# HPCForge/Bubbleformer

Measured on AMD Instinct MI355X. Metric: train samples/sec, FiLMAViT 16x192x192x4ch, bs=8 per GPU, higher is better.
Workload: dtype bf16; 1 GPU; FiLMAViT-small (E=384, 6 heads, 12 blocks, P=16, 9 fluid params) fwd + relative-L2 loss + bwd + AdamW, 4-field 16x192x192 clips, batch 8 per GPU (BASELINE.json configs[1]); global_batch=8, parallelism=dp1

## Files before the change

bubbleformer_amd/_lib.py:

```python
import ctypes as C
import os
import subprocess

_HERE = os.path.dirname(os.path.abspath(__file__))
LIB_PATH = os.path.join(_HERE, "libbubbleformer_hip.so")
CSRC = os.path.join(_HERE, "csrc")

BF_DTYPE_F32, BF_DTYPE_BF16 = 0, 1
BF_LAY_KC, BF_LAY_XC = 0, 1
BF_PRO_NONE, BF_PRO_AFFINE, BF_PRO_AFFINE_GELU, BF_PRO_GELU = 0, 1, 2, 3
BF_AUX_NONE, BF_AUX_ADD, BF_AUX_DGELU = 0, 1, 2
BF_OUT_STORE, BF_OUT_STORE_F32, BF_OUT_ATOMIC_F32 = 0, 1, 2
BF_MAX_STAGES = 5
BF_LOSS_LIMBS = 5
BF_OPT_CHUNK, BF_OPT_MAX_GROUPS = 64, 64

vp, fp, i32, i64, f32 = C.c_void_p, C.c_void_p, C.c_int32, C.c_int64, C.c_float


class Operand(C.Structure):
    _fields_ = [("p", vp), ("ld", i64), ("layout", i32), ("seglen", i32), ("segstride", i64), ("gw", i32), ("gh", i32),
                ("gc", i32), ("pro", i32), ("sc", fp), ("sh", fp), ("rows_per_frame", i32), ("nch", i32)]


# ... 34 lines not shown


class DebedParams(C.Structure):
    _fields_ = [("conv_w", fp * BF_MAX_STAGES), ("in_w", fp * BF_MAX_STAGES), ("in_b", fp * BF_MAX_STAGES)]


class ConvSrc(C.Structure):
    _fields_ = [("p", vp), ("C", i32), ("nchw", i32), ("f32", i32)]


class ConvGeo(C.Structure):
    _fields_ = [(n, i32) for n in ("F", "Hi", "Wi", "Ho", "Wo", "kh", "kw", "stride", "pad")]


BF_CONV_PRO_NONE, BF_CONV_PRO_AFFINE_GELU, BF_CONV_PRO_GELU = 0, 1, 2


class RolloutStep(C.Structure):
    _fields_ = [("pred", fp), ("frames", fp), ("field_stride", i64), ("total_frames", i64), ("first", vp), ("step", vp), ("field", vp), ("diff", fp),
                ("div", fp)] + [(n, i32) for n in ("nfields", "B", "T", "C", "H", "W", "Ho", "Wo", "steps", "reserved")]


class CensusRows(C.Structure):
    _fields_ = [(n, vp) for n in ("count", "cells", "attached", "area")]


class LinkRows(C.Structure):
    _fields_ = [(n, vp) for n in ("successor", "n_successors", "predecessor", "n_predecessors", "departure_area", "events")]


class ErrorRows(C.Structure):
    _fields_ = [(n, vp) for n in ("rmse", "max_error", "boundary_rmse", "interface_rmse", "interface_cells", "spectral_error", "spectrum_error",
                                  "spectrum_pred", "spectrum_target")]


class EnsembleRows(C.Structure):
    _fields_ = [(n, vp) for n in ("mean_rmse", "spread", "crps", "rank_hist", "mean")]


class OptStep(C.Structure):
    _fields_ = [("p", fp), ("g", fp), ("m", fp), ("v", fp), ("coef_dev", fp), ("avg", fp), ("chunk_group", vp), ("group_lr_scale", fp),
                ("group_weight_decay", fp), ("group_frozen", vp), ("live_dev", vp), ("n", i64), ("step", i32), ("n_groups", i32)] + [
        (n, f32) for n in ("lr", "beta1", "beta2", "eps", "wd", "gscale", "clip_value", "avg_weight")]


class ClipGatherJob(C.Structure):
    _fields_ = [("src", fp), ("idx", vp), ("first_tab", vp), ("in_field", vp), ("in_diff", fp), ("in_div", fp), ("in_out", fp), ("out_field", vp),
                ("out_diff", fp), ("out_div", fp), ("out_out", fp), ("fluid_tab", fp), ("file_tab", vp), ("fluid_out", fp), ("field_stride", i64),
                ("nframes", i64), ("nsamples", i64)] + [(n, i32) for n in ("Cin", "Tin", "Cout", "Tout", "unroll", "P", "B", "H", "W", "Ho", "Wo", "reserved")]


class ClipAugment(C.Structure):
    _fields_ = [("in_odd", vp), ("out_odd", vp), ("seed", i64), ("flip_thr", i64)] + [(n, i32) for n in ("draw", "Hc", "Wc", "crop_y", "eval_view", "reserved")]


class ClipGatherQ16Job(C.Structure):
    _fields_ = [("codes", vp), ("frame_seg", vp), ("seg_lo", fp), ("seg_step", fp), ("idx", vp), ("first_tab", vp), ("in_field", vp), ("in_diff", fp),
                ("in_div", fp), ("in_out", fp), ("out_field", vp), ("out_diff", fp), ("out_div", fp), ("out_out", fp), ("fluid_tab", fp), ("file_tab", vp),
                ("fluid_out", fp), ("field_stride", i64), ("nframes", i64), ("nsamples", i64)] + [
        (n, i32) for n in ("nfiles", "Cin", "Tin", "Cout", "Tout", "unroll", "P", "B", "H", "W", "Ho", "Wo")]


class RenderTile(C.Structure):
    _fields_ = [("a", fp), ("b", fp), ("mask", fp), ("frame_stride", i64), ("slot_stride", i64), ("mask_frame_stride", i64), ("mask_slot_stride", i64),
                ("range", vp), ("kind", i32)]


class RenderGeom(C.Structure):
    _fields_ = [(n, i32) for n in ("H", "W", "scale", "rows", "cols", "ox", "oy", "pitch_x", "pitch_y", "bar_dx", "bar_w", "img_h", "img_w", "stride")] + [
        ("stroke", C.c_double)]


BF_RENDER_SDF, BF_RENDER_TEMP, BF_RENDER_SPEED = 0, 1, 2
BF_RENDER_MAX_TILES = 6

STAGE_DONE_FN = C.CFUNCTYPE(None, C.c_int, C.c_void_p)
P = C.POINTER
SIGNATURES = {
    "bf_last_error": (C.c_char_p, []),
    "bf_abi_version": (C.c_int, []),
    "bf_prof_enable": (None, [C.c_int]),
    "bf_debug_force_generic_attn": (None, [C.c_int]),
    "bf_debug_tokred_fold": (None, [C.c_int]),
    "bf_side_defer": (None, [C.c_int]),
    "bf_prep_stages": (C.c_int, [C.POINTER(Dims), C.c_int, C.POINTER(C.c_int32), C.POINTER(vp), C.POINTER(vp), C.POINTER(vp), vp]),
    "bf_stage_prepared": (None, [C.c_int]),
    "bf_trunk_train_fwd": (C.c_int, [C.POINTER(Dims), C.c_int, C.POINTER(C.c_int32), C.POINTER(vp), C.POINTER(vp), C.POINTER(vp), C.POINTER(vp), vp,
                                     C.POINTER(vp), vp, vp]),
    "bf_trunk_train_bwd": (C.c_int, [C.POINTER(Dims), C.c_int, C.POINTER(C.c_int32), C.POINTER(vp), C.POINTER(vp), C.POINTER(vp), C.POINTER(vp),
                                     C.POINTER(vp), vp, C.POINTER(vp), vp, C.POINTER(vp), vp, vp, vp, vp, vp]),
    "bf_field_stats_ws_doubles": (i64, [C.c_int]),
    "bf_field_stats": (C.c_int, [fp, vp, vp, C.c_int, vp, vp, vp]),
    "bf_stage_chain_next": (C.c_int, [C.POINTER(Dims), C.c_int, vp, vp]),
    "bf_stage_next_scale": (C.c_int, [fp, C.c_int]),
    "bf_gemm_fwd_frames": (C.c_int, [C.c_int, C.c_int, C.c_int, C.c_int, vp, i64, vp, i64, fp, fp, fp, fp, C.c_int, vp, vp, C.c_int,
                                     C.POINTER(FrameNorm), C.POINTER(FrameNorm), vp]),
    "bf_trunk_eval_weights_bytes": (i64, [C.POINTER(Dims), C.c_int, C.POINTER(C.c_int32)]),
    "bf_trunk_eval_prepare": (C.c_int, [C.POINTER(Dims), C.c_int, C.POINTER(C.c_int32), C.POINTER(vp), vp, vp]),
    "bf_trunk_eval_fwd": (C.c_int, [C.POINTER(Dims), C.c_int, C.POINTER(C.c_int32), C.POINTER(vp), vp, vp, vp, vp, vp]),
    "bf_frame_linear": (C.c_int, [C.c_int, C.c_int, C.c_int, C.c_int, C.c_int, vp, i64, vp, i64, fp, fp, fp, fp, fp, vp, i64, C.c_int, fp, fp, fp,
                                  vp, i64, fp, fp, vp, i64, vp]),
    "bf_side_join": (C.c_int, [vp]),
    "bf_prof_report": (C.c_int, [C.c_char_p, C.c_int]),
    "bf_gemm": (C.c_int, [C.c_int, C.c_int, C.c_int, C.c_int, P(Operand), P(Operand), P(Epilogue), C.c_int, vp]),
    "bf_gemm_tokred": (C.c_int, [C.c_int, C.c_int, C.c_int, i64, vp, i64, vp, i64, fp, C.c_int, fp, fp, i64, vp]),
    "bf_gemm_tokred_ws_floats": (i64, [C.c_int, C.c_int, i64]),
    "bf_gemm_inbwd_frames": (C.c_int, [C.c_int, C.c_int, C.c_int, C.c_int, vp, i64, vp, i64, vp, vp, vp, C.c_int, fp, fp, fp, fp, fp, C.c_int, vp]),
    "bf_gemm_inbwd_frames_chain": (C.c_int, [C.c_int, C.c_int, C.c_int, C.c_int, vp, i64, vp, i64, vp, vp, vp, C.c_int, fp, fp, fp, fp, fp, C.c_int,
                                             vp, vp, fp, fp, fp, fp, C.c_int, fp, vp]),
    "bf_in_stats": (C.c_int, [C.c_int, vp, C.c_int, C.c_int, C.c_int, fp, fp, fp, C.c_int, fp, fp, fp, fp, fp, fp, vp]),
    "bf_in_ws_floats": (i64, [C.c_int, C.c_int, C.c_int, C.c_int]),
    "bf_affine_apply": (C.c_int, [C.c_int, vp, vp, fp, fp, vp, i64, C.c_int, C.c_int, vp]),
    "bf_in_bwd": (C.c_int, [C.c_int, vp, vp, vp, vp, C.c_int, C.c_int, C.c_int, fp, fp, fp, fp, fp, C.c_int, C.c_int, fp, fp,
                            fp, fp, fp, vp]),
    "bf_colsum": (C.c_int, [C.c_int, vp, i64, C.c_int, fp, fp, vp]),
    "bf_attn_axial_fwd": (C.c_int, [C.c_int, vp, vp, i64, C.c_int, C.c_int, C.c_int, C.c_int, fp, fp, fp, fp, fp, fp, fp, vp]),
    "bf_attn_axial_norm_fwd": (C.c_int, [C.c_int, vp, vp, vp, i64, C.c_int, C.c_int, C.c_int, C.c_int, fp, fp, fp, fp, fp, fp, fp, fp, fp, fp, fp, fp,
                                         fp, vp]),
    "bf_attn_fwd": (C.c_int, [C.c_int, vp, vp, i64, C.c_int, i64, i64, i64, i64, C.c_int, C.c_int, fp, fp, fp, fp, fp, fp, f32,
                              C.c_int, vp]),
    "bf_attn_bwd": (C.c_int, [C.c_int, vp, vp, vp, i64, C.c_int, i64, i64, i64, i64, C.c_int, C.c_int, fp, fp, fp, fp, fp, fp,
                              fp, fp, fp, fp, fp, fp, f32, C.c_int, fp, i64, vp]),
    "bf_im2col_nchw": (C.c_int, [C.c_int, fp, vp, C.c_int, C.c_int, C.c_int, C.c_int, C.c_int, vp]),
    "bf_col2im_nchw": (C.c_int, [C.c_int, vp, fp, C.c_int, C.c_int, C.c_int, C.c_int, C.c_int, vp]),
    "bf_pm2nchw": (C.c_int, [fp, fp, fp, fp, C.c_int, C.c_int, C.c_int, C.c_int, C.c_int, vp]),
    "bf_debed_last_bwd": (C.c_int, [C.c_int, fp, fp, fp, fp, fp, vp, vp, vp, C.c_int, C.c_int, C.c_int, C.c_int, C.c_int, C.c_int, vp]),
    "bf_debed_last_bwd_norm": (C.c_int, [C.c_int, fp, fp, fp, fp, fp, vp, vp, vp, fp, fp, fp, fp, vp, fp, fp, C.c_int, C.c_int, C.c_int, C.c_int, C.c_int,
                                         C.c_int, fp, C.c_int64, vp]),
    "bf_gather_gemm": (C.c_int, [C.c_int, vp, vp, C.c_int, fp, fp, vp, C.c_int, C.c_int, C.c_int, C.c_int, C.c_int, vp]),
    "bf_scatter_gemm": (C.c_int, [C.c_int, vp, vp, C.c_int, fp, fp, vp, fp, C.c_int, C.c_int, C.c_int, C.c_int, C.c_int, vp]),
    "bf_gather_wgrad_ws_floats": (C.c_int64, [C.c_int, C.c_int, C.c_int]),
    "bf_gather_wgrad": (C.c_int, [C.c_int, vp, vp, fp, fp, fp, fp, fp, C.c_int, C.c_int, C.c_int, C.c_int, C.c_int, C.c_int, fp, C.c_int64, vp]),
    "bf_gather_gemm_rebuilt": (C.c_int, [C.c_int, vp, vp, vp, C.c_int, fp, fp, vp, C.c_int, C.c_int, C.c_int, C.c_int, C.c_int, vp]),
    "bf_gather_wgrad_rebuilt": (C.c_int, [C.c_int, vp, vp, vp, fp, fp, fp, C.c_int, C.c_int, C.c_int, C.c_int, C.c_int, C.c_int, fp, C.c_int64, vp]),
    "bf_stage_chain_head": (C.c_int, [vp, vp, vp]),
    "bf_stage_chain_tail": (C.c_int, [vp, vp, C.c_int]),
    "bf_embed_tail_ws_floats": (C.c_int64, [C.c_int, C.c_int, C.c_int, C.c_int, C.c_int]),
    "bf_embed_tail_bwd": (C.c_int, [C.c_int, vp, vp, vp, vp, vp, fp, fp, fp, fp, fp, fp, fp, fp, C.c_int, C.c_int, C.c_int, C.c_int, C.c_int, C.c_int,
                                    fp, C.c_int64, vp]),
    "bf_embed_first": (C.c_int, [C.c_int, fp, vp, vp, vp, C.c_int, C.c_int, C.c_int, C.c_int, C.c_int, C.c_int, fp, vp]),
    "bf_in_stats_merge_slices": (C.c_int, [C.c_int, C.c_int, C.c_int, C.c_int, C.c_int, fp, fp, fp, C.c_int, fp, fp, fp, fp, fp, fp, vp]),
    "bf_debed_last": (C.c_int, [C.c_int, vp, fp, fp, vp, fp, fp, fp, C.c_int, C.c_int, C.c_int, C.c_int, C.c_int, C.c_int, vp]),
    "bf_lploss_finalize": (C.c_int, [fp, C.c_int, C.c_int, fp, fp, vp]),
    "bf_nchw2pm": (C.c_int, [C.c_int, fp, fp, fp, fp, fp, vp, C.c_int, C.c_int, C.c_int, C.c_int, C.c_int, vp]),
    "bf_wprep": (C.c_int, [C.c_int, C.c_int, fp, vp, C.c_int, C.c_int, C.c_int, vp]),
    "bf_wgrad_unprep": (C.c_int, [C.c_int, fp, fp, C.c_int, C.c_int, C.c_int, C.c_int, vp]),
    "bf_film_net_fwd": (C.c_int, [fp, fp, fp, fp, fp, fp, fp, fp, C.c_int, C.c_int, C.c_int, vp]),
    "bf_film_net_bwd": (C.c_int, [fp, fp, fp, fp, fp, fp, fp, fp, fp, C.c_int, C.c_int, C.c_int, vp]),
    "bf_adamw": (C.c_int, [P(OptStep), vp]),
    "bf_adam": (C.c_int, [P(OptStep), vp]),
    "bf_lion": (C.c_int, [P(OptStep), vp]),
    "bf_grad_norm_ws_doubles": (i64, [i64]),
    "bf_grad_norm": (C.c_int, [fp, i64, f32, f32, fp, vp, i64, vp]),
    "bf_weight_average": (C.c_int, [fp, fp, i64, f32, vp]),
    "bf_swap_buffers": (C.c_int, [fp, fp, i64, vp]),
    "bf_group_sumsq_ws_doubles": (i64, [i64]),
    "bf_group_sumsq": (C.c_int, [fp, i64, vp, C.c_int, vp, vp, i64, vp]),
    "bf_group_clip_coef": (C.c_int, [vp, vp, C.c_int, f32, f32, fp, fp, vp]),
    "bf_step_guard": (C.c_int, [fp, i32, vp, vp]),
    "bf_nonfinite_scan_ws_len": (i64, [i64]),
    "bf_nonfinite_scan": (C.c_int, [fp, i64, vp, vp, i64, vp]),
    "bf_eikonal_sum": (C.c_int, [fp, i64, C.c_int, C.c_int, f32, vp, vp]),
    "bf_eikonal_l1_frames": (C.c_int, [fp, i64, C.c_int, C.c_int, f32, fp, vp]),
    "bf_heatflux_rows": (C.c_int, [fp, fp, i64, i64, C.c_int, f32, f32, f32, f32, fp, vp]),
    "bf_clip_gather": (C.c_int, [fp, i64, vp, vp, C.c_int, fp, fp, fp, C.c_int, C.c_int, C.c_int, C.c_int, C.c_int, C.c_int, C.c_int, vp]),
    "bf_clip_gather_batch": (C.c_int, [fp, i64, vp, i64, vp, vp, fp, fp, C.c_int, C.c_int, fp, vp, fp, fp, C.c_int, C.c_int, fp, fp, vp, C.c_int, fp,
                                       C.c_int, C.c_int, C.c_int, C.c_int, C.c_int, vp]),
    "bf_clip_gather_unroll": (C.c_int, [fp, i64, i64, vp, i64, vp, vp, fp, fp, C.c_int, C.c_int, fp, vp, fp, fp, C.c_int, C.c_int, C.c_int, fp, fp, vp, C.c_int,
                                        fp, C.c_int, C.c_int, C.c_int, C.c_int, C.c_int, vp]),
    "bf_clip_gather_augment": (C.c_int, [P(ClipGatherJob), P(ClipAugment), vp]),
    "bf_clip_encode_q16": (C.c_int, [fp, vp, i64, f32, f32, vp]),
    "bf_clip_decode_q16": (C.c_int, [vp, i64, vp, fp, fp, fp, i64, C.c_int, C.c_int, C.c_int, C.c_int, vp]),
    "bf_clip_gather_q16": (C.c_int, [P(ClipGatherQ16Job), P(ClipAugment), vp]),
    "bf_clip_noise": (C.c_int, [fp, fp, fp, vp, C.c_uint64, C.c_uint32, C.c_uint32, C.c_int, C.c_int, C.c_int, C.c_int, C.c_int, vp]),
    "bf_rollout_score_ws_doubles": (i64, [C.c_int, C.c_int, C.c_int, C.c_int, C.c_int]),
    "bf_rollout_score": (C.c_int, [P(RolloutStep), C.c_int, f32, fp, fp, fp, fp, fp, fp, vp, i64, vp]),
    "bf_rollout_heatflux": (C.c_int, [P(RolloutStep), C.c_int, C.c_int, fp, f32, f32, f32, f32, fp, fp, vp]),
    "bf_kde_kl_ws_doubles": (i64, [C.c_int, i64, i64, C.c_int]),
    "bf_kde_kl": (C.c_int, [vp, vp, C.c_int, i64, i64, C.c_int, C.c_double, vp, vp, vp, vp, vp, i64, vp]),
    "bf_bubble_census_lds_cells": (i64, []),
    "bf_bubble_census_ws_bytes": (i64, [i64, C.c_int, C.c_int, C.c_int]),
    "bf_bubble_census": (C.c_int, [fp, i64, C.c_int, C.c_int, C.c_int, C.c_int, vp, vp, vp, vp, fp, vp, vp, vp, i64, vp]),
    "bf_rollout_bubbles": (C.c_int, [P(RolloutStep), C.c_int, C.c_int, C.c_int, P(CensusRows), P(CensusRows), vp, vp, i64, vp]),
    "bf_redistance_lds_cells": (i64, []),
    "bf_redistance_ws_bytes": (i64, [i64, C.c_int, C.c_int]),
    "bf_redistance": (C.c_int, [fp, i64, C.c_int, C.c_int, f32, f32, C.c_int, fp, vp, fp, vp, i64, vp]),
    "bf_rollout_redistance": (C.c_int, [P(RolloutStep), C.c_int, f32, f32, C.c_int, C.c_int, fp, vp, fp, vp, i64, vp]),
    "bf_bubble_links_lds_entries": (i64, []),
    "bf_bubble_links_ws_bytes": (i64, [i64, C.c_int]),
    "bf_bubble_links": (C.c_int, [vp, P(CensusRows), i64, C.c_int, C.c_int, C.c_int, C.c_int, P(LinkRows), vp, i64, vp]),
    "bf_bubble_track_ids": (C.c_int, [vp, vp, vp, i64, C.c_int, C.c_int, vp, vp, vp]),
    "bf_rollout_bubble_links": (C.c_int, [P(RolloutStep), C.c_int, vp, P(CensusRows), P(CensusRows), P(LinkRows), P(LinkRows), vp, i64, vp]),
# ... 97 lines not shown
```

bubbleformer_amd/csrc/gemm_frame.hip:

```cpp
#include "gemm_common.h"
#include <stdlib.h>
#include <string.h>
#include <type_traits>

int bf_gemm_pair_scaled(int M, int N, int K, const bf_operand* A, const bf_operand* B, const bf_epilogue* E, void* out2, const float* rowfac,
                        int rows_per_group, hipStream_t st);

namespace {
using namespace bfgemm;

constexpr int FM = 144, FN = 128, FK = 64, FNT = 384;
constexpr int A_EL = FM * FK, B_EL = FK * FN, BUF_EL = A_EL + B_EL;
constexpr int XLD = 136;
constexpr int TILE_EL = FM * XLD;
constexpr int RED_OFF = 2 * TILE_EL * 2;
constexpr int LDS_BYTES = RED_OFF + 3 * 2 * FN * 4;
static_assert(2 * BUF_EL * 2 <= RED_OFF, "operand buffers must not reach the exchange area");

struct FrameArgs {
    const bf16* A; long lda; const bf16* B; long ldb; int N, nk, nt;
    const bf16* x; const bf16* add; bf16* out; long ldx;
    const float* mean; const float* rstd; const float* w; float* ws;
    const float* fscale; int fdiv;
};

__global__ void __launch_bounds__(FNT, 3) gemm_inbwd_frames_kernel(FrameArgs a) {
    extern __shared__ __attribute__((aligned(16))) unsigned char smem[];
    bf16* lds = reinterpret_cast<bf16*>(smem);
    const int tid = threadIdx.x, lane = tid & 63, wave = tid >> 6;
    const int wm = wave >> 1, wn = wave & 1;
    const int li = lane & 15, lg = lane >> 4;
    const int seq = xcd_remap(blockIdx.x, gridDim.x);
    const int fidx = seq / a.nt;
    const int m0 = fidx * FM, n0 = (seq - fidx * a.nt) * FN;

    const bf16* ga[3]; int la[3];
    const bf16* gb[3]; int lb[3];
#pragma unroll
    for (int i = 0; i < 3; ++i) {
        const int c = tid + FNT * i;
        const int row = c >> 3, c8 = (c & 7) << 3;
        ga[i] = a.A + (long)(m0 + row) * a.lda + c8;
        la[i] = lds_off<bf16, false, FK>(row, c8);
        const int kr = (c >> 4) & 63, d8 = (c & 15) << 3;
        gb[i] = a.B + (long)kr * a.ldb + n0 + d8;
        lb[i] = A_EL + lds_off<bf16, true, FN>(kr, d8);
    }
    const bool b2 = tid < FK * FN / 8 - 2 * FNT;
    Chunk<bf16> ra[3], rb[3];
    auto issue = [&](int kt) {
        const long ka = (long)kt * FK, kb = (long)kt * FK * a.ldb;
#pragma unroll
        for (int i = 0; i < 3; ++i) ra[i].load(ga[i] + ka);
        rb[0].load(gb[0] + kb);
        rb[1].load(gb[1] + kb);
        if (b2) rb[2].load(gb[2] + kb);
    };
    auto commit = [&](int buf) {
        bf16* base = lds + buf * BUF_EL;
#pragma unroll
        for (int i = 0; i < 3; ++i) ra[i].store(base + la[i]);
        rb[0].store(base + lb[0]);
        rb[1].store(base + lb[1]);
        if (b2) rb[2].store(base + lb[2]);
    };
    f32x4 acc[3][4];
#pragma unroll
    for (int i = 0; i < 3; ++i)
#pragma unroll
        for (int j = 0; j < 4; ++j) acc[i][j] = f32x4{0.f, 0.f, 0.f, 0.f};
    auto mma = [&](int buf) {
        const bf16* cA = lds + buf * BUF_EL;
        const bf16* cB = cA + A_EL;
#pragma unroll
        for (int kk = 0; kk < FK; kk += 32) {
            bf16x8 fa[3], fb[4];
#pragma unroll
            for (int i = 0; i < 3; ++i) fa[i] = frag_bf16<false, FK>(cA, wm * 48 + i * 16, kk, lane);
#pragma unroll
            for (int j = 0; j < 4; ++j) fb[j] = frag_bf16<true, FN>(cB, wn * 64 + j * 16, kk, lane);
#pragma unroll
            for (int i = 0; i < 3; ++i)
#pragma unroll
// ... 455 lines not shown
#pragma unroll
        for (int i = 0; i < 9; ++i) {
            const bf16x8 x8 = xr[i];
            const bf16x8 d8 = __builtin_bit_cast(bf16x8, ad[i]);
            bf16x8 o;
#pragma unroll
            for (int q = 0; q < 8; ++q) {
                const float xh = ((float)x8[q] - mu[q]) * rs[q];
                float t = rs[q] * ww[q] * (v[i][q] - (s1[q] + xh * s2[q]) * invS);
                if (a.add) t += (float)d8[q];
                o[q] = (bf16)t;
            }
            *reinterpret_cast<bf16x8*>(a.out + (row0 + 16 * i) * a.ldx + col0) = o;
            if constexpr (MODE == 5) {
                const float m2 = a.fscale_s[fidx / a.fdiv_s];
                bf16x8 o2;
#pragma unroll
                for (int q = 0; q < 8; ++q) o2[q] = (bf16)((float)o[q] * m2);
                *reinterpret_cast<bf16x8*>(a.out_s + (row0 + 16 * i) * a.ldx + col0) = o2;
            }
        }
        if constexpr (chain) {
            __builtin_amdgcn_sched_barrier(0);
            uint4 zr[9];
            bf16x8 ov[9];
#pragma unroll
            for (int i = 0; i < 9; ++i) {
                zr[i] = *reinterpret_cast<const uint4*>(a.cz + (row0 + 16 * i) * a.ldx + col0);
                ov[i] = *reinterpret_cast<const bf16x8*>(a.out + (row0 + 16 * i) * a.ldx + col0);
            }
            const long cb = (long)fidx * a.N + col0;
            float m3[8], r3[8], k3[8];
            {
                const float4 m0 = *reinterpret_cast<const float4*>(a.cmean + cb), m1 = *reinterpret_cast<const float4*>(a.cmean + cb + 4);
                const float4 r0 = *reinterpret_cast<const float4*>(a.crstd + cb), r1 = *reinterpret_cast<const float4*>(a.crstd + cb + 4);
                const float4 w0 = *reinterpret_cast<const float4*>(a.cw + col0), w1 = *reinterpret_cast<const float4*>(a.cw + col0 + 4);
                m3[0] = m0.x; m3[1] = m0.y; m3[2] = m0.z; m3[3] = m0.w; m3[4] = m1.x; m3[5] = m1.y; m3[6] = m1.z; m3[7] = m1.w;
                r3[0] = r0.x; r3[1] = r0.y; r3[2] = r0.z; r3[3] = r0.w; r3[4] = r1.x; r3[5] = r1.y; r3[6] = r1.z; r3[7] = r1.w;
                k3[0] = w0.x; k3[1] = w0.y; k3[2] = w0.z; k3[3] = w0.w; k3[4] = w1.x; k3[5] = w1.y; k3[6] = w1.z; k3[7] = w1.w;
                if (a.cg) {
                    const long gbase = (long)(fidx / a.cgdiv) * a.N + col0;
                    const float4 g0 = *reinterpret_cast<const float4*>(a.cg + gbase), g1 = *reinterpret_cast<const float4*>(a.cg + gbase + 4);
                    k3[0] *= g0.x; k3[1] *= g0.y; k3[2] *= g0.z; k3[3] *= g0.w; k3[4] *= g1.x; k3[5] *= g1.y; k3[6] *= g1.z; k3[7] *= g1.w;
                }
#pragma unroll
                for (int q = 0; q < 8; ++q) k3[q] *= r3[q];
            }
            float c1[8], c2[8];
#pragma unroll
            for (int q = 0; q < 8; ++q) { c1[q] = 0.f; c2[q] = 0.f; }
#pragma unroll
            for (int i = 0; i < 9; ++i) {
                const bf16x8 z8 = __builtin_bit_cast(bf16x8, zr[i]);
#pragma unroll
                for (int q = 0; q < 8; ++q) {
                    const float dd = (float)ov[i][q], xh = ((float)z8[q] - m3[q]) * r3[q];
                    c1[q] += dd;
                    c2[q] += dd * xh;
                }
            }
#pragma unroll
            for (int q = 0; q < 8; ++q) { c1[q] = row16_sum(c1[q]); c2[q] = row16_sum(c2[q]); }
            if (li == 0 && a.cws) {
                float* wp = a.cws + cb * 2;
#pragma unroll
                for (int q = 0; q < 8; q += 2) *reinterpret_cast<float4*>(wp + 2 * q) = make_float4(c1[q], c2[q], c1[q + 1], c2[q + 1]);
            }
#pragma unroll
            for (int i = 0; i < 9; ++i) {
                const bf16x8 z8 = __builtin_bit_cast(bf16x8, zr[i]);
                bf16x8 o;
#pragma unroll
                for (int q = 0; q < 8; ++q) {
                    const float dd = (float)ov[i][q], xh = ((float)z8[q] - m3[q]) * r3[q];
                    o[q] = (bf16)(k3[q] * (dd - (c1[q] + xh * c2[q]) * (1.f / 144.f)));
                }
                *reinterpret_cast<bf16x8*>(a.cdz + (row0 + 16 * i) * a.ldx + col0) = o;
            }
        }
    }
}

template <int MODE>
__global__ void __launch_bounds__(512) gemm_pair_kernel(PairArgs a) {
    extern __shared__ __attribute__((aligned(16))) unsigned char smem[];
    const int tid = threadIdx.x, lane = tid & 63, wave = __builtin_amdgcn_readfirstlane(tid >> 6);
    const int seq = xcd_remap(blockIdx.x, gridDim.x);
    const int fp = seq / a.nt;
    const int m0 = fp * PM, n0 = (seq - fp * a.nt) * PN;
    const int f0 = ((MODE == 0 || MODE == 2 || MODE == 5) && a.whole) ? fp : 2 * fp;
    if (wave < 4) pair_body<MODE, 0>(a, smem, lane, wave, m0, n0, f0);
    else pair_body<MODE, 1>(a, smem, lane, wave - 4, m0, n0, f0);
}

template <int MODE>
int launch_pair(const PairArgs& a, int M, hipStream_t st) {
    static BfPerDeviceOnce attr_once; bool& attr_done = attr_once.flag();
    if (!attr_done) {
        hipError_t e_ = hipFuncSetAttribute(reinterpret_cast<const void*>(gemm_pair_kernel<MODE>), hipFuncAttributeMaxDynamicSharedMemorySize, PNSLOT * PSLOT_BYTES);
        if (e_ != hipSuccess) return bf_fail(e_, __FILE__, __LINE__);
        attr_done = true;
    }
    hipLaunchKernelGGL(gemm_pair_kernel<MODE>, dim3((unsigned)((M / PM) * a.nt)), dim3(512), PNSLOT * PSLOT_BYTES, st, a);
    BF_CHECK_LAUNCH();
    return 0;
}
bool pair_shape_ok(int M, int N, int K, int64_t lda, int64_t ldb) {
    static const bool off = bf_knob("BF_PAIR", 1) == 0;
    if (off) return false;
    return M > 0 && M % PM == 0 && N > 0 && N % PN == 0 && K >= PK && K % PK == 0 && lda % 8 == 0 && ldb % 8 == 0 &&
           (long)PM * lda * 2 < (1L << 31) && (long)PK * ldb * 2 < (1L << 31);
}

}

struct InbwdChain { const void* z; void* dz; const float *mean, *rstd, *w, *g; int gdiv; float* ws; };
struct InbwdScaled { void* out_s; const float* f; int fdiv; };
static int inbwd_frames_impl2(int dtype, int M, int N, int K, const void* A, int64_t lda, const void* B, int64_t ldb, const void* x,
                              const void* add, void* out, int S, const float* mean, const float* rstd, const float* w, float* ws,
                              const float* fscale, int fdiv, const InbwdChain* ch, const InbwdScaled* sc2, bf_stream_t stream);
static int inbwd_frames_impl(int dtype, int M, int N, int K, const void* A, int64_t lda, const void* B, int64_t ldb, const void* x,
                             const void* add, void* out, int S, const float* mean, const float* rstd, const float* w, float* ws,
                             const float* fscale, int fdiv, const InbwdChain* ch, bf_stream_t stream);
extern "C" int bf_gemm_inbwd_frames(int dtype, int M, int N, int K, const void* A, int64_t lda, const void* B, int64_t ldb, const void* x,
                                    const void* add, void* out, int S, const float* mean, const float* rstd, const float* w, float* ws,
                                    const float* fscale, int fdiv, bf_stream_t stream) {
    return inbwd_frames_impl(dtype, M, N, K, A, lda, B, ldb, x, add, out, S, mean, rstd, w, ws, fscale, fdiv, nullptr, stream);
}
extern "C" int bf_gemm_inbwd_frames_chain(int dtype, int M, int N, int K, const void* A, int64_t lda, const void* B, int64_t ldb, const void* x,
                                          const void* add, void* out, int S, const float* mean, const float* rstd, const float* w, float* ws,
                                          const float* fscale, int fdiv, const void* cz, void* cdz, const float* cmean, const float* crstd,
                                          const float* cw, const float* cg, int cgdiv, float* cws, bf_stream_t stream) {
    BF_REQUIRE(cz && cdz && cmean && crstd && cw, "bf_gemm_inbwd_frames_chain: null pointer");
    const InbwdChain ch{cz, cdz, cmean, crstd, cw, cg, cgdiv > 0 ? cgdiv : 1, cws};
    return inbwd_frames_impl(dtype, M, N, K, A, lda, B, ldb, x, add, out, S, mean, rstd, w, ws, fscale, fdiv, &ch, stream);
}
static int inbwd_frames_impl(int dtype, int M, int N, int K, const void* A, int64_t lda, const void* B, int64_t ldb, const void* x,
                             const void* add, void* out, int S, const float* mean, const float* rstd, const float* w, float* ws,
                             const float* fscale, int fdiv, const InbwdChain* ch, bf_stream_t stream) {
    return inbwd_frames_impl2(dtype, M, N, K, A, lda, B, ldb, x, add, out, S, mean, rstd, w, ws, fscale, fdiv, ch, nullptr, stream);
}
int bf_gemm_inbwd_frames_scaled(int dtype, int M, int N, int K, const void* A, int64_t lda, const void* B, int64_t ldb, const void* x,
                                const void* add, void* out, int S, const float* mean, const float* rstd, const float* w, float* ws,
                                const float* fscale, int fdiv, void* out_s, const float* f_s, int fdiv_s, hipStream_t stream) {
    if (!out_s || !f_s || (((uintptr_t)out_s) & 15)) return 1;
    const InbwdScaled sc2{out_s, f_s, fdiv_s > 0 ? fdiv_s : 1};
    return inbwd_frames_impl2(dtype, M, N, K, A, lda, B, ldb, x, add, out, S, mean, rstd, w, ws, fscale, fdiv, nullptr, &sc2, (bf_stream_t)stream);
}
static int inbwd_frames_impl2(int dtype, int M, int N, int K, const void* A, int64_t lda, const void* B, int64_t ldb, const void* x,
                              const void* add, void* out, int S, const float* mean, const float* rstd, const float* w, float* ws,
                              const float* fscale, int fdiv, const InbwdChain* ch, const InbwdScaled* sc2, bf_stream_t stream) {
    BF_REQUIRE(A && B && x && out && mean && rstd && w, "bf_gemm_inbwd_frames: null pointer");
    static const bool off = bf_knob("BF_FUSE_INBWD", 1) == 0;
    if (off || dtype != BF_DTYPE_BF16 || (S != FM && S != PM) || M <= 0 || M % S || N <= 0 || N % FN || K < FK || K % FK || lda % 8 || ldb % 8) return 1;
    if (pair_shape_ok(M, N, K, lda, ldb) && (((uintptr_t)A | (uintptr_t)B | (uintptr_t)x | (uintptr_t)add | (uintptr_t)out) & 15) == 0) {
        PairArgs a;
        a.whole = S == PM;
        a.A = (const bf16*)A; a.lda = lda; a.B = (const bf16*)B; a.ldb = ldb; a.N = N; a.nk = K / PK; a.nt = N / PN;
        a.x = (const bf16*)x; a.add = (const bf16*)add; a.out = (bf16*)out; a.ldx = N;
        a.mean = mean; a.rstd = rstd; a.w = w; a.ws = ws; a.fscale = fscale; a.fdiv = fdiv > 0 ? fdiv : 1; a.out2 = nullptr;
        a.cz = nullptr; a.cdz = nullptr; a.cmean = a.crstd = a.cw = a.cg = nullptr; a.cgdiv = 1; a.cws = nullptr;
        a.bias = a.cs = a.ch = nullptr; memset(&a.n1, 0, sizeof(a.n1)); memset(&a.n2, 0, sizeof(a.n2));
        a.out_s = nullptr; a.fscale_s = nullptr; a.fdiv_s = 1;
        if (sc2) { a.out_s = (bf16*)sc2->out_s; a.fscale_s = sc2->f; a.fdiv_s = sc2->fdiv; }
        if (ch) {
            if (a.whole || (((uintptr_t)ch->z | (uintptr_t)ch->dz) & 15)) return 1;
            a.cz = (const bf16*)ch->z; a.cdz = (bf16*)ch->dz; a.cmean = ch->mean; a.crstd = ch->rstd; a.cw = ch->w; a.cg = ch->g; a.cgdiv = ch->gdiv; a.cws = ch->ws;
        }
        BfProfScope prof((hipStream_t)stream, ch ? "gemm_pair<inbwd,chain>" : sc2 ? "gemm_pair<inbwd,scaled>" : "gemm_pair<inbwd>", 2.0 * M * N * K,
                         2.0 * ((double)M * K + (double)N * K + (double)M * N * ((add ? 3 : 2) + (ch ? 2 : 0) + (sc2 ? 1 : 0))));
        if (sc2) { if (ch) return 1; return launch_pair<5>(a, M, (hipStream_t)stream); }
        return ch ? launch_pair<2>(a, M, (hipStream_t)stream) : launch_pair<0>(a, M, (hipStream_t)stream);
    }
    if (ch || sc2) return 1;
    if (S != FM) return 1;
    static BfPerDeviceOnce attr_once;
    if (bool& done = attr_once.flag(); !done) {
        const hipError_t attr = hipFuncSetAttribute(reinterpret_cast<const void*>(gemm_inbwd_frames_kernel), hipFuncAttributeMaxDynamicSharedMemorySize, LDS_BYTES);
        if (attr != hipSuccess) return bf_fail(attr, __FILE__, __LINE__);
        done = true;
    }
    hipStream_t st = (hipStream_t)stream;
    FrameArgs a;
    a.A = (const bf16*)A; a.lda = lda; a.B = (const bf16*)B; a.ldb = ldb; a.N = N; a.nk = K / FK; a.nt = N / FN;
    a.x = (const bf16*)x; a.add = (const bf16*)add; a.out = (bf16*)out; a.ldx = N;
    a.mean = mean; a.rstd = rstd; a.w = w; a.ws = ws;
    a.fscale = fscale; a.fdiv = fdiv > 0 ? fdiv : 1;
    BfProfScope prof(st, "gemm_inbwd_frames<bf16>", 2.0 * M * N * K, 2.0 * ((double)M * K + (double)N * K + (double)M * N * (add ? 3 : 2)));
    hipLaunchKernelGGL(gemm_inbwd_frames_kernel, dim3((unsigned)((M / FM) * a.nt)), dim3(FNT), LDS_BYTES, st, a);
    BF_CHECK_LAUNCH();
    return 0;
}

int bf_gemm_pair_try(int M, int N, int K, const bf_operand* A, const bf_operand* B, const bf_epilogue* E, hipStream_t st) {
    return bf_gemm_pair_scaled(M, N, K, A, B, E, nullptr, nullptr, 1, st);
}
int bf_gemm_pair_scaled(int M, int N, int K, const bf_operand* A, const bf_operand* B, const bf_epilogue* E, void* out2, const float* rowfac,
                        int rows_per_group, hipStream_t st) {
    if (A->layout != BF_LAY_KC || B->layout != BF_LAY_XC || A->pro != BF_PRO_NONE || B->pro != BF_PRO_NONE) return 1;
    if (A->gw > 0 || A->seglen > 0 || B->gw > 0 || B->seglen > 0 || E->gw > 0 || E->seglen > 0) return 1;
    if (E->out_mode != BF_OUT_STORE || E->colsum || E->bias || E->colscale || E->rowscale || E->gelu_out) return 1;
    if (E->aux_mode != BF_AUX_NONE && E->aux_mode != BF_AUX_ADD) return 1;
    if (!pair_shape_ok(M, N, K, A->ld, B->ld) || K < 2 * PK || E->ldc != N || (E->aux_mode == BF_AUX_ADD && E->ld_aux != N)) return 1;
    if (((uintptr_t)A->p | (uintptr_t)B->p | (uintptr_t)E->c | (uintptr_t)E->aux) & 15) return 1;
    PairArgs a;
    a.A = (const bf16*)A->p; a.lda = A->ld; a.B = (const bf16*)B->p; a.ldb = B->ld; a.N = N; a.nk = K / PK; a.nt = N / PN;
    a.x = nullptr; a.add = E->aux_mode == BF_AUX_ADD ? (const bf16*)E->aux : nullptr; a.out = (bf16*)E->c; a.ldx = N;
    a.mean = nullptr; a.rstd = nullptr; a.w = nullptr; a.ws = nullptr; a.fscale = rowfac; a.fdiv = rows_per_group > 0 ? rows_per_group : 1;
    a.out2 = rowfac ? (bf16*)out2 : nullptr; a.whole = 0;
    a.cz = nullptr; a.cdz = nullptr; a.cmean = a.crstd = a.cw = a.cg = nullptr; a.cgdiv = 1; a.cws = nullptr;
    a.bias = a.cs = a.ch = nullptr; memset(&a.n1, 0, sizeof(a.n1)); memset(&a.n2, 0, sizeof(a.n2));
    a.out_s = nullptr; a.fscale_s = nullptr; a.fdiv_s = 1;
    if (a.out2 && ((uintptr_t)out2 & 15)) return 1;
    BfProfScope prof(st, a.add ? "gemm_pair<add>" : "gemm_pair<plain>", 2.0 * M * N * K, 2.0 * ((double)M * K + (double)N * K + (double)M * N * (a.add ? 2 : 1)));
    return launch_pair<1>(a, M, st);
}

extern "C" int bf_gemm_fwd_frames(int dtype, int M, int N, int K, const void* A, int64_t lda, const void* Bt, int64_t ldb, const float* bias,
                                  const float* colscale, const float* colshift, const float* fscale, int fdiv, const void* add, void* out, int S,
                                  const bf_frame_norm* n1, const bf_frame_norm* n2, bf_stream_t stream) {
    static const bool off = bf_knob("BF_FUSE_FWD_NORM", 1) == 0;
    if (off || dtype != BF_DTYPE_BF16 || S != FM || !pair_shape_ok(M, N, K, lda, ldb) || K < 2 * PK) return 1;
    BF_REQUIRE(A && Bt && out, "bf_gemm_fwd_frames: null pointer");
    BF_REQUIRE(!colscale == !colshift, "bf_gemm_fwd_frames: column scale and shift come together");
    if (fscale && !colscale) return 1;
    if (((uintptr_t)A | (uintptr_t)Bt | (uintptr_t)add | (uintptr_t)out | (uintptr_t)bias | (uintptr_t)colscale | (uintptr_t)colshift) & 15) return 1;
    PairArgs a;
    memset(&a, 0, sizeof(a));
    a.A = (const bf16*)A; a.lda = lda; a.B = (const bf16*)Bt; a.ldb = ldb; a.N = N; a.nk = K / PK; a.nt = N / PN;
    a.add = (const bf16*)add; a.out = (bf16*)out; a.ldx = N;
    a.fscale = fscale; a.fdiv = fdiv > 0 ? fdiv : 1; a.cgdiv = 1;
    a.bias = bias; a.cs = colscale; a.ch = colshift;
    auto take = [&](const bf_frame_norm* n, FwdNorm& o, bool first) -> int {
        if (!n) return 0;
        BF_REQUIRE(n->w && n->b && n->mean && n->rstd && n->sc && n->sh && n->out, "bf_gemm_fwd_frames: incomplete norm record");
        if (((uintptr_t)n->w | (uintptr_t)n->b | (uintptr_t)n->g | (uintptr_t)n->mean | (uintptr_t)n->rstd | (uintptr_t)n->sc | (uintptr_t)n->sh |
             (uintptr_t)n->resid | (uintptr_t)n->out) & 15) return 1;
        if (!first && (n->g || n->resid)) return 1;
        o.w = n->w; o.b = n->b; o.g = n->g; o.gdiv = n->gdiv > 0 ? n->gdiv : 1; o.mean = n->mean; o.rstd = n->rstd; o.sc = n->sc; o.sh = n->sh;
        o.resid = (const bf16*)n->resid; o.out = (bf16*)n->out;
        return 0;
    };
    if (int rc = take(n1, a.n1, true)) return rc;
    if (int rc = take(n2, a.n2, false)) return rc;
    BfProfScope prof((hipStream_t)stream, n1 ? (n2 ? "gemm_pair<fwd,norm,chain>" : "gemm_pair<fwd,norm>") : (n2 ? "gemm_pair<fwd,chain>" : "gemm_pair<fwd>"),
                     2.0 * M * N * K, 2.0 * ((double)M * K + (double)N * K + (double)M * N * (1 + (add ? 1 : 0) + (n1 ? (n1->resid ? 2 : 1) : 0) + (n2 ? 1 : 0))));
    return n1 ? launch_pair<4>(a, M, (hipStream_t)stream) : launch_pair<3>(a, M, (hipStream_t)stream);
}
```

bubbleformer_amd/csrc/gemm_tokred.hip:

```cpp
#include "gemm_common.h"
#include <stdio.h>
#include <stdlib.h>
#include <algorithm>

namespace {
using namespace bfgemm;

constexpr int PTN = 192;
constexpr int HR = 32;
constexpr int NSB = PTN / 64;
constexpr int SUBB = HR * 64 * 2;
constexpr int NBUF = 4;
template <int NI> struct PPGeom {
    static constexpr int TM = 64 * NI, HALFB = (NI + NSB) * SUBB, TILES = NI * 6, TILE_FLOATS = TM * PTN;
};

__device__ __forceinline__ bf16x8 tr_frag(unsigned addr) {
    return cat(__builtin_amdgcn_ds_read_tr16_b64_v4i16((lds_s16x4)(uintptr_t)addr),
               __builtin_amdgcn_ds_read_tr16_b64_v4i16((lds_s16x4)(uintptr_t)(addr + 512u)));
}

template <int NI, int GRP>
__device__ __forceinline__ void tokred_pp_body(const bf16* __restrict__ A, long lda, const bf16* __restrict__ B, long ldb,
                                               float* __restrict__ slab_tile, float* __restrict__ cslab_row, int nh, bool do_cs,
                                               unsigned ring_lds, int lane, int w4) {
    using Gm = PPGeom<NI>;
    constexpr int HALFB = Gm::HALFB;
    constexpr int PG = NI == 6 ? (GRP == 0 ? 5 : 4) : 3;
    constexpr int NCS = 3;
    const int wm = w4, wn = GRP;
    const int dr = 8 * w4 + (lane >> 3);
    const int dkey = ((dr >> 1) & 1) | (((dr >> 3) & 1) << 1);
    const int dch = (lane & 7) ^ (dkey << 1);
    const bf16* pA = A + (long)dr * lda + 8 * dch;
    const bf16* pB = B + (long)dr * ldb + 8 * dch;
    const long stepA = (long)HR * lda, stepB = (long)HR * ldb;
    auto issue = [&](int buf) {
        const unsigned base = __builtin_amdgcn_readfirstlane(ring_lds + (unsigned)buf * (unsigned)HALFB + (unsigned)w4 * 1024u);
        if constexpr (NI == 6 && GRP == 0) {
            glds16_off<0>(pA, base + 0 * SUBB); glds16_off<128>(pA, base + 1 * SUBB); glds16_off<256>(pA, base + 2 * SUBB);
            glds16_off<384>(pA, base + 3 * SUBB); glds16_off<512>(pA, base + 4 * SUBB);
            pA += stepA;
        } else if constexpr (NI == 6) {
            glds16_off<640>(pA, base + 5 * SUBB);
            glds16_off<0>(pB, base + 6 * SUBB); glds16_off<128>(pB, base + 7 * SUBB); glds16_off<256>(pB, base + 8 * SUBB);
            pA += stepA; pB += stepB;
        } else if constexpr (GRP == 0) {
            glds16_off<0>(pA, base + 0 * SUBB); glds16_off<128>(pA, base + 1 * SUBB); glds16_off<256>(pA, base + 2 * SUBB);
            pA += stepA;
        } else {
            glds16_off<0>(pB, base + 3 * SUBB); glds16_off<128>(pB, base + 4 * SUBB); glds16_off<256>(pB, base + 5 * SUBB);
            pB += stepB;
        }
    };
    const int g = lane >> 4, q = (lane >> 2) & 3, p = lane & 3;
    const int fkey = ((q >> 1) & 1) | ((g & 1) << 1);
    const unsigned rowb = (unsigned)(8 * g + q) * 128u + (unsigned)(p & 1) * 8u;
    const unsigned offA = rowb + (unsigned)(((2 * wm + (p >> 1)) ^ (fkey << 1)) * 16);
    const unsigned offB0 = rowb + (unsigned)(((2 * wn + (p >> 1)) ^ (fkey << 1)) * 16) + (unsigned)(NI * SUBB);
    const unsigned offB1 = rowb + (unsigned)(((2 * wn + 4 + (p >> 1)) ^ (fkey << 1)) * 16) + (unsigned)(NI * SUBB);

    f32x4 acc[NI][6];
#pragma unroll
    for (int i = 0; i < NI; ++i)
#pragma unroll
        for (int j = 0; j < 6; ++j) acc[i][j] = f32x4{0.f, 0.f, 0.f, 0.f};
    f32x4 cs[NCS];
#pragma unroll
    for (int c = 0; c < NCS; ++c) cs[c] = f32x4{0.f, 0.f, 0.f, 0.f};
    bf16x8 ones;
#pragma unroll
    for (int c = 0; c < 8; ++c) ones[c] = (bf16)1.0f;

    issue(0);
    if (nh > 1) issue(1);
    if (nh > 2) issue(2);
    if (nh > 2) wait_vm<2 * PG>(); else if (nh > 1) wait_vm<PG>(); else wait_vm<0>();
    __builtin_amdgcn_s_barrier();
    if constexpr (GRP == 1) __builtin_amdgcn_s_barrier();

    int buf = 0;
    for (int h = 0; h < nh; ++h) {
        const unsigned hb = ring_lds + (unsigned)buf * (unsigned)HALFB;
        bf16x8 fa[NI], fb[6];
#pragma unroll
        for (int i = 0; i < NI; ++i) fa[i] = tr_frag(hb + offA + (unsigned)(i * SUBB));
#pragma unroll
        for (int j = 0; j < 6; ++j) fb[j] = tr_frag(hb + ((j & 1) ? offB1 : offB0) + (unsigned)((j >> 1) * SUBB));
        if (h + 3 < nh) issue((buf + 3) & 3);
        const int younger = min(h + 3, nh - 1) - (h + 1);
        if (younger >= 2) wait_vm<2 * PG>(); else if (younger == 1) wait_vm<PG>(); else wait_vm<0>();
        asm volatile("s_waitcnt lgkmcnt(0)" ::: "memory");
        __builtin_amdgcn_sched_barrier(0);
        __builtin_amdgcn_s_barrier();
#pragma unroll
        for (int i = 0; i < NI; ++i)
#pragma unroll
            for (int j = 0; j < 6; ++j) acc[i][j] = __builtin_amdgcn_mfma_f32_16x16x32_bf16(fb[j], fa[i], acc[i][j], 0, 0, 0);
        if (do_cs) {
#pragma unroll
            for (int c = 0; c < NCS; ++c) {
                if constexpr (NI == 6) cs[c] = __builtin_amdgcn_mfma_f32_16x16x32_bf16(ones, fa[NCS * GRP + c], cs[c], 0, 0, 0);
                else if constexpr (GRP == 0) cs[c] = __builtin_amdgcn_mfma_f32_16x16x32_bf16(ones, fa[c], cs[c], 0, 0, 0);
            }
        }
        __builtin_amdgcn_sched_barrier(0);
        __builtin_amdgcn_s_barrier();
        buf = (buf + 1) & 3;
    }
    if constexpr (GRP == 0) __builtin_amdgcn_s_barrier();

    const int wave = GRP * 4 + w4;
    float* so = slab_tile + ((size_t)wave * Gm::TILES * 64 + lane) * 4;
#pragma unroll
    for (int i = 0; i < NI; ++i)
#pragma unroll
        for (int j = 0; j < 6; ++j)
            *reinterpret_cast<float4*>(so + (size_t)(i * 6 + j) * 256) = make_float4(acc[i][j][0], acc[i][j][1], acc[i][j][2], acc[i][j][3]);
    if (do_cs && lane < 16) {
        if constexpr (NI == 6) {
#pragma unroll
            for (int c = 0; c < NCS; ++c) cslab_row[16 * (wm + 4 * (NCS * GRP + c)) + lane] = cs[c][0];
        } else if constexpr (GRP == 0) {
#pragma unroll
            for (int c = 0; c < NCS; ++c) cslab_row[16 * (wm + 4 * c) + lane] = cs[c][0];
        }
    }
}

struct FoldRed { const float* slab; const float* cslab; int nslice, ntiles, tiles_k, Nout, Kin; float* out; float* colsum; int accumulate; int nwg; };
template <int NI>
__device__ __forceinline__ void fold_reduce(const FoldRed& r, int b) {
    using Gm = PPGeom<NI>;
    constexpr int T4 = Gm::TILE_FLOATS / 4;
    const long total = (long)r.ntiles * T4;
    const size_t sstride = (size_t)r.ntiles * Gm::TILE_FLOATS;
    for (long e = (long)b * 512 + threadIdx.x; e < total; e += (long)r.nwg * 512) {
        const int tile = (int)(e / T4), q = (int)(e - (long)tile * T4);
        const int lane = q & 63, t = q >> 6, wave = t / Gm::TILES, ij = t - wave * Gm::TILES, i = ij / 6, j = ij - i * 6;
        const int wm = wave & 3, wn = wave >> 2;
        const int nout = (tile / r.tiles_k) * Gm::TM + 16 * (wm + 4 * i) + (lane & 15);
        const int kin = (tile % r.tiles_k) * PTN + 16 * (wn + 2 * j) + 4 * (lane >> 4);
        const float* src = r.slab + (size_t)tile * Gm::TILE_FLOATS + (size_t)q * 4;
        float4* dst = reinterpret_cast<float4*>(r.out + (size_t)nout * r.Kin + kin);
        float4 a = r.accumulate ? *dst : make_float4(0.f, 0.f, 0.f, 0.f);
        for (int s0 = 0; s0 < r.nslice; s0 += 8) {
            float4 v[8];
#pragma unroll
            for (int u = 0; u < 8; ++u) v[u] = s0 + u < r.nslice ? *reinterpret_cast<const float4*>(src + (size_t)(s0 + u) * sstride) : make_float4(0.f, 0.f, 0.f, 0.f);
#pragma unroll
            for (int u = 0; u < 8; ++u)
                if (s0 + u < r.nslice) { a.x += v[u].x; a.y += v[u].y; a.z += v[u].z; a.w += v[u].w; }
        }
        *dst = a;
    }
    if (r.colsum)
        for (long m = (long)b * 512 + threadIdx.x; m < r.Nout; m += (long)r.nwg * 512) {
            float a = r.accumulate ? r.colsum[m] : 0.f;
            for (int s2 = 0; s2 < r.nslice; ++s2) a += r.cslab[(size_t)s2 * r.Nout + m];
            r.colsum[m] = a;
        }
}

template <int NI>
__global__ void __launch_bounds__(512) tokred_pp_kernel(const bf16* __restrict__ A, long lda, const bf16* __restrict__ B, long ldb,
                                                      float* __restrict__ slab, float* __restrict__ cslab, int Nout, int halves_total,
                                                      int halves_per, int tiles_k, int ntiles, int main_wgs, FoldRed red) {
    using Gm = PPGeom<NI>;
    extern __shared__ __attribute__((aligned(16))) char smem[];
    if ((int)blockIdx.x >= main_wgs) { fold_reduce<NI>(red, (int)blockIdx.x - main_wgs); return; }
    const int tid = threadIdx.x, lane = tid & 63, wave = __builtin_amdgcn_readfirstlane(tid >> 6);
    const int seq = xcd_remap(blockIdx.x, main_wgs);
    const int slice = seq / ntiles, tile = seq - slice * ntiles;
    const int n0 = (tile / tiles_k) * Gm::TM, c0 = (tile % tiles_k) * PTN;
    const int h_beg = slice * halves_per;
    const int nh = min(halves_per, halves_total - h_beg);
    const bf16* a0 = A + (long)h_beg * HR * lda + n0;
    const bf16* b0 = B + (long)h_beg * HR * ldb + c0;
    float* slab_tile = slab + ((size_t)slice * ntiles + tile) * Gm::TILE_FLOATS;
    const bool do_cs = cslab != nullptr && c0 == 0;
    float* cslab_row = do_cs ? cslab + (size_t)slice * Nout + n0 : nullptr;
    const unsigned ring_lds = lds_addr(smem);
    if (wave < 4) tokred_pp_body<NI, 0>(a0, lda, b0, ldb, slab_tile, cslab_row, nh, do_cs, ring_lds, lane, wave);
    else tokred_pp_body<NI, 1>(a0, lda, b0, ldb, slab_tile, cslab_row, nh, do_cs, ring_lds, lane, wave - 4);
}

template <int NI, int MAXS>
__global__ void __launch_bounds__(256) tokred_pp_reduce_kernel(const float* __restrict__ slab, const float* __restrict__ cslab, int nslice,
                                                               int ntiles, int tiles_k, int Nout, int Kin, float* __restrict__ out,
                                                               float* __restrict__ colsum, int accumulate) {
    using Gm = PPGeom<NI>;
    constexpr int T4 = Gm::TILE_FLOATS / 4;
    const long e = (long)blockIdx.x * 256 + threadIdx.x;
    if (e < (long)ntiles * T4) {
        const int tile = (int)(e / T4), r = (int)(e - (long)tile * T4);
        const int lane = r & 63, t = r >> 6, wave = t / Gm::TILES, ij = t - wave * Gm::TILES, i = ij / 6, j = ij - i * 6;
        const int wm = wave & 3, wn = wave >> 2;
        const int nout = (tile / tiles_k) * Gm::TM + 16 * (wm + 4 * i) + (lane & 15);
        const int kin = (tile % tiles_k) * PTN + 16 * (wn + 2 * j) + 4 * (lane >> 4);
        const size_t sstride = (size_t)ntiles * Gm::TILE_FLOATS;
        const float* src = slab + (size_t)tile * Gm::TILE_FLOATS + (size_t)r * 4;
        float4 v[MAXS];
#pragma unroll
        for (int s = 0; s < MAXS; ++s) v[s] = s < nslice ? *reinterpret_cast<const float4*>(src + s * sstride) : make_float4(0.f, 0.f, 0.f, 0.f);
        float4* dst = reinterpret_cast<float4*>(out + (size_t)nout * Kin + kin);
        float4 a = accumulate ? *dst : make_float4(0.f, 0.f, 0.f, 0.f);
#pragma unroll
        for (int s = 0; s < MAXS; ++s)
            if (s < nslice) { a.x += v[s].x; a.y += v[s].y; a.z += v[s].z; a.w += v[s].w; }
        *dst = a;
    }
    if (colsum && e < Nout) {
        float v[MAXS];
#pragma unroll
        for (int s = 0; s < MAXS; ++s) v[s] = s < nslice ? cslab[(size_t)s * Nout + e] : 0.f;
        float a = accumulate ? colsum[e] : 0.f;
#pragma unroll
        for (int s = 0; s < MAXS; ++s)
            if (s < nslice) a += v[s];
        colsum[e] = a;
    }
}

constexpr int NW_TILE = 32;
template <int CT, bool PRO>
__global__ void __launch_bounds__(256) tokred_narrow_kernel(const bf16* __restrict__ dy, const bf16* __restrict__ x, long tiles_total, float* __restrict__ slab,
                                                          const float* __restrict__ psc, const float* __restrict__ psh, int tiles_per_frame) {
    constexpr int C = 16 * CT, DYB = NW_TILE * C * 2, XB = NW_TILE * 16 * 2, TB_ = DYB + XB;
    extern __shared__ __attribute__((aligned(16))) char smem[];
    const int tid = threadIdx.x, lane = tid & 63, wave = __builtin_amdgcn_readfirstlane(tid >> 6);
    const long nwaves = (long)gridDim.x * 4, w = (long)blockIdx.x * 4 + wave;
    const long t_beg = tiles_total * w / nwaves, t_end = tiles_total * (w + 1) / nwaves;
    char* mine = smem + (size_t)wave * 2 * TB_;
    const unsigned lds0 = lds_addr(mine);
    auto issue = [&](long t, int slot) {
        const char* gd = reinterpret_cast<const char*>(dy) + t * DYB + lane * 16;
        const unsigned dst = __builtin_amdgcn_readfirstlane(lds0 + (unsigned)slot * (unsigned)TB_);
#pragma unroll
        for (int pce = 0; pce < DYB / 1024; ++pce) glds16(gd + pce * 1024, dst + (unsigned)pce * 1024u);
        glds16(reinterpret_cast<const char*>(x) + t * XB + lane * 16, dst + (unsigned)DYB);
    };
    constexpr int PCS = DYB / 1024 + 1;
    f32x4 acc[CT];
#pragma unroll
    for (int i = 0; i < CT; ++i) acc[i] = f32x4{0.f, 0.f, 0.f, 0.f};
    const int g = lane >> 4, q = (lane >> 2) & 3, pp = lane & 3;
    const unsigned offD = (unsigned)((8 * g + q) * (C * 2) + 8 * pp), offX = (unsigned)(DYB + (8 * g + q) * 32 + 8 * pp);
    auto trf = [&](unsigned addr, unsigned hi_off) {
        return cat(__builtin_amdgcn_ds_read_tr16_b64_v4i16((lds_s16x4)(uintptr_t)addr),
                   __builtin_amdgcn_ds_read_tr16_b64_v4i16((lds_s16x4)(uintptr_t)(addr + hi_off)));
    };
    float scv[CT], shv[CT];
    for (long s_beg = t_beg; s_beg < t_end;) {
        long s_end = t_end;
        if constexpr (PRO) {
            const long f = s_beg / tiles_per_frame;
            s_end = min(t_end, (f + 1) * (long)tiles_per_frame);
            wait_vm<0>();
#pragma unroll
            for (int i = 0; i < CT; ++i) { scv[i] = psc[f * C + 16 * i + (lane & 15)]; shv[i] = psh ? psh[f * C + 16 * i + (lane & 15)] : 0.f; }
#pragma unroll
            for (int i = 0; i < CT; ++i) asm volatile("s_waitcnt vmcnt(0)" : "+v"(scv[i]), "+v"(shv[i]) :: "memory");
        }
        issue(s_beg, 0);
        int slot = 0;
        for (long t = s_beg; t < s_end; ++t) {
            if (t + 1 < s_end) { issue(t + 1, slot ^ 1); wait_vm<PCS>(); } else wait_vm<0>();
// ... 103 lines not shown
    bf16x8 ones;
#pragma unroll
    for (int q = 0; q < 8; ++q) ones[q] = (bf16)1.0f;

#pragma unroll
    for (int s = 0; s < NSLOT - 1; ++s)
        if (s < steps) issue(s);

    int cur = 0, nxt = NSLOT - 1;
    for (int s = 0; s < steps; ++s) {
        const int younger = min(NSLOT - 2, steps - 1 - s);
        if (younger == NSLOT - 2) wait_vm<(NSLOT - 2) * G>();
        else wait_vm<0>();
        asm volatile("s_waitcnt lgkmcnt(0)" ::: "memory");
        __builtin_amdgcn_s_barrier();
        if (s + NSLOT - 1 < steps) issue(nxt);
        const bf16* cA = ring + (size_t)cur * SLOT;
        const bf16* cB = cA + CHUNK;
#pragma unroll
        for (int kk = 0; kk < BK; kk += 32) {
            bf16x8 fa[TMI], fb[TNI];
#pragma unroll
            for (int i = 0; i < TMI; ++i) fa[i] = frag_bf16<true, TB>(cA, wm * (16 * TMI) + i * 16, kk, lane);
#pragma unroll
            for (int j = 0; j < TNI; ++j) fb[j] = frag_bf16<true, TB>(cB, wn * (16 * TNI) + j * 16, kk, lane);
#pragma unroll
            for (int i = 0; i < TMI; ++i)
#pragma unroll
                for (int j = 0; j < TNI; ++j) acc[i][j] = __builtin_amdgcn_mfma_f32_16x16x32_bf16(fb[j], fa[i], acc[i][j], 0, 0, 0);
            if (do_cs) {
#pragma unroll
                for (int i = 0; i < TMI; ++i)
                    if (wn == i) cs = __builtin_amdgcn_mfma_f32_16x16x32_bf16(ones, fa[i], cs, 0, 0, 0);
            }
        }
        cur = cur + 1 == NSLOT ? 0 : cur + 1;
        nxt = nxt + 1 == NSLOT ? 0 : nxt + 1;
    }

    const int li = lane & 15, lg = lane >> 4;
    float* so = slab + ((size_t)slice * Nout + n0 + wm * (16 * TMI) + li) * Kin + c0 + wn * (16 * TNI) + 4 * lg;
#pragma unroll
    for (int i = 0; i < TMI; ++i)
#pragma unroll
        for (int j = 0; j < TNI; ++j)
            *reinterpret_cast<float4*>(so + (size_t)(i * 16) * Kin + j * 16) = make_float4(acc[i][j][0], acc[i][j][1], acc[i][j][2], acc[i][j][3]);
    if (do_cs && lg == 0) cslab[(size_t)slice * Nout + n0 + wm * (16 * TMI) + wn * 16 + li] = cs[0];
}

__global__ void __launch_bounds__(256) tokred_reduce_kernel(const float* __restrict__ slab, const float* __restrict__ cslab, int nslice, long n,
                                                            int Nout, float* __restrict__ out, float* __restrict__ colsum, int accumulate) {
    const long n4 = n / 4;
    for (long i = (long)blockIdx.x * 256 + threadIdx.x; i < n4; i += (long)gridDim.x * 256) {
        float4 a = accumulate ? reinterpret_cast<const float4*>(out)[i] : make_float4(0.f, 0.f, 0.f, 0.f);
        for (int s0 = 0; s0 < nslice; s0 += 8) {
            float4 v[8];
#pragma unroll
            for (int q = 0; q < 8; ++q) v[q] = s0 + q < nslice ? reinterpret_cast<const float4*>(slab + (size_t)(s0 + q) * n)[i] : make_float4(0.f, 0.f, 0.f, 0.f);
#pragma unroll
            for (int q = 0; q < 8; ++q)
                if (s0 + q < nslice) { a.x += v[q].x; a.y += v[q].y; a.z += v[q].z; a.w += v[q].w; }
        }
        reinterpret_cast<float4*>(out)[i] = a;
    }
    if (colsum) {
        for (long m = (long)blockIdx.x * 256 + threadIdx.x; m < Nout; m += (long)gridDim.x * 256) {
            float a = accumulate ? colsum[m] : 0.f;
            for (int s = 0; s < nslice; ++s) a += cslab[(size_t)s * Nout + m];
            colsum[m] = a;
        }
    }
}

constexpr int MAX_SLICES = 16;

}

extern "C" int64_t bf_gemm_tokred_ws_floats(int Nout, int Kin, int64_t M) {
    if (Nout <= 0 || Kin <= 0 || M <= 0) return 0;
    return (int64_t)MAX_SLICES * ((int64_t)Nout * Kin + Nout);
}

namespace {
struct PendingRed { bool on = false; FoldRed r{}; int NI = 0; hipStream_t st = nullptr; bool half = false; hipEvent_t handoff = nullptr; };
PendingRed g_pending[64];
PendingRed& pending_slot() { int dev = 0; (void)hipGetDevice(&dev); return g_pending[(dev >= 0 && dev < 64) ? dev : 0]; }
constexpr int FOLD_WGS = 40;
}
static int tokred_impl(int dtype, int Nout, int Kin, int64_t M, const void* dy, int64_t ldy, const void* x, int64_t ldx, float* out,
                       int accumulate, float* colsum, float* ws, int64_t ws_floats, bool defer, bf_stream_t stream);
static int flush_pending(PendingRed& p, hipStream_t caller) {
    if (!p.on) return 0;
    p.on = false;
    hipStream_t st = p.st;
    const FoldRed& r = p.r;
    const long n = (long)r.Nout * r.Kin;
    const unsigned rblocks = (unsigned)bf_cdiv(std::max<long>(n / 4, r.Nout), 256);
    BfProfScope prof(st, "tokred_reduce_kernel", 0.0, (double)(r.nslice + 1 + (r.accumulate ? 1 : 0)) * n * 4.0);
    if (p.NI == 6) {
        if (r.nslice <= 8) hipLaunchKernelGGL((tokred_pp_reduce_kernel<6, 8>), dim3(rblocks), dim3(256), 0, st, r.slab, r.cslab, r.nslice, r.ntiles, r.tiles_k, r.Nout, r.Kin, r.out, r.colsum, r.accumulate);
        else hipLaunchKernelGGL((tokred_pp_reduce_kernel<6, MAX_SLICES>), dim3(rblocks), dim3(256), 0, st, r.slab, r.cslab, r.nslice, r.ntiles, r.tiles_k, r.Nout, r.Kin, r.out, r.colsum, r.accumulate);
    } else {
        if (r.nslice <= 8) hipLaunchKernelGGL((tokred_pp_reduce_kernel<3, 8>), dim3(rblocks), dim3(256), 0, st, r.slab, r.cslab, r.nslice, r.ntiles, r.tiles_k, r.Nout, r.Kin, r.out, r.colsum, r.accumulate);
        else hipLaunchKernelGGL((tokred_pp_reduce_kernel<3, MAX_SLICES>), dim3(rblocks), dim3(256), 0, st, r.slab, r.cslab, r.nslice, r.ntiles, r.tiles_k, r.Nout, r.Kin, r.out, r.colsum, r.accumulate);
    }
    BF_CHECK_LAUNCH();
    if (caller == st) return 0;
    hipError_t e = p.handoff ? hipSuccess : hipEventCreateWithFlags(&p.handoff, hipEventDisableTiming);
    if (e == hipSuccess) e = hipEventRecord(p.handoff, st);
    if (e == hipSuccess) e = hipStreamWaitEvent(caller, p.handoff, 0);
    return e == hipSuccess ? 0 : bf_fail(e, __FILE__, __LINE__);
}
int bf_gemm_tokred_flush(hipStream_t st) { return flush_pending(pending_slot(), st); }
namespace { bool g_fold_off = false; }
extern "C" void bf_debug_tokred_fold(int on) { g_fold_off = on == 0; }
bool bf_gemm_tokred_pending() { return pending_slot().on; }
const float* bf_gemm_tokred_pending_out() { const PendingRed& p = pending_slot(); return p.on ? p.r.out : nullptr; }
int bf_gemm_tokred_deferred(int dtype, int Nout, int Kin, int64_t M, const void* dy, int64_t ldy, const void* x, int64_t ldx, float* out,
                            int accumulate, float* colsum, float* ws, int64_t ws_floats, hipStream_t stream) {
    return tokred_impl(dtype, Nout, Kin, M, dy, ldy, x, ldx, out, accumulate, colsum, ws, ws_floats, true, (bf_stream_t)stream);
}
extern "C" int bf_gemm_tokred(int dtype, int Nout, int Kin, int64_t M, const void* dy, int64_t ldy, const void* x, int64_t ldx, float* out,
                              int accumulate, float* colsum, float* ws, int64_t ws_floats, bf_stream_t stream) {
    return tokred_impl(dtype, Nout, Kin, M, dy, ldy, x, ldx, out, accumulate, colsum, ws, ws_floats, false, stream);
}
static int tokred_impl(int dtype, int Nout, int Kin, int64_t M, const void* dy, int64_t ldy, const void* x, int64_t ldx, float* out,
                       int accumulate, float* colsum, float* ws, int64_t ws_floats, bool defer, bf_stream_t stream) {
    if (dtype != BF_DTYPE_BF16) return 1;
    static const int skip_env = bf_knob("BF_TOKRED_SKIP", 0);
    if (skip_env) return 0;
    const bool pp = Nout % 192 == 0 && Kin % PTN == 0 && M % HR == 0 && M >= 4 * HR;
    if (!pp && (Nout % TB || Kin % TB || M % BK || M < BK)) return 1;
    if (ldy % 8 || ldx % 8) return 1;
    BF_REQUIRE(dy && x && out && ws, "bf_gemm_tokred: null pointer");
    BF_REQUIRE(((uintptr_t)dy & 15) == 0 && ((uintptr_t)x & 15) == 0 && ((uintptr_t)out & 15) == 0 && ((uintptr_t)ws & 15) == 0,
               "bf_gemm_tokred: operands must be 16-byte aligned");
    BF_REQUIRE(ldy >= Nout && ldx >= Kin, "bf_gemm_tokred: leading dimensions smaller than the row length");
    hipStream_t st = (hipStream_t)stream;
    const long n = (long)Nout * Kin;
    static const int slices_env = bf_knob("BF_TOKRED_SLICES", 0);
    static const int tile_env = bf_knob("BF_TOKRED_TILE", 0);
    static const int wgs_env = bf_knob("BF_TOKRED_WGS", 128);
    if (pp) {
        const long halves = M / HR;
        const int tiles_k0 = Kin / PTN;
        const bool big = Nout % 384 == 0 && tile_env == 384;
        const int tm = big ? 384 : 192;
        int nslice = slices_env > 0 ? slices_env : std::max(1, wgs_env / ((Nout / tm) * tiles_k0));
        nslice = (int)std::max<long>(1, std::min<long>({(long)nslice, (long)MAX_SLICES, halves / 4}));
        const int halves_per = bf_cdiv(halves, nslice);
        const int ns = bf_cdiv(halves, halves_per);
        BF_REQUIRE(ws_floats >= (int64_t)ns * (n + Nout), "bf_gemm_tokred: workspace too small (bf_gemm_tokred_ws_floats)");
        const int tiles_k = Kin / PTN, ntiles = (Nout / tm) * tiles_k;
        static const bool fold_on = bf_knob("BF_TOKRED_FOLD", 1) != 0;
        const int64_t half_floats = (ws_floats / 2) & ~(int64_t)3;
        const bool fold = defer && fold_on && !g_fold_off && (int64_t)ns * (n + Nout) <= half_floats;
        PendingRed& pend = pending_slot();
        if (pend.on && (!fold || pend.NI != (big ? 6 : 3) || pend.st != st)) { const int frc = flush_pending(pend, st); if (frc) return frc; }
        float* region = ws;
        if (fold) { region = ws + (pend.half ? half_floats : 0); pend.half = !pend.half; }
        float* slab = region;
        float* cslab = colsum ? region + (size_t)ns * n : nullptr;
        const unsigned rblocks = (unsigned)bf_cdiv(std::max<long>(n / 4, Nout), 256);
        FoldRed red{};
        static const int fold_wgs = bf_knob("BF_TOKRED_FOLD_WGS", FOLD_WGS);
        if (fold && pend.on) { red = pend.r; red.nwg = fold_wgs; }
        const unsigned extra = red.nwg > 0 ? (unsigned)red.nwg : 0u;
#define BF_PP_GO(NIV)                                                                                                                     \
        do {                                                                                                                              \
            {                                                                                                                             \
                BfProfScope prof(st, NIV == 6 ? "tokred_pp_kernel<384x192,h32,ring4>" : "tokred_pp_kernel<192x192,h32,ring4>",           \
                                 2.0 * Nout * Kin * (double)M, (double)M * (Nout + Kin) * 2.0 + (double)n * 4.0);                         \
                static BfPerDeviceOnce attr_once; bool& attr_done = attr_once.flag();                                                                                            \
                constexpr int lds_bytes = NBUF * PPGeom<NIV>::HALFB;                                                                      \
                if (!attr_done) {                                                                                                         \
                    hipError_t e_ = hipFuncSetAttribute((const void*)tokred_pp_kernel<NIV>, hipFuncAttributeMaxDynamicSharedMemorySize, lds_bytes); \
                    if (e_ != hipSuccess) return bf_fail(e_, __FILE__, __LINE__);                                                         \
                    attr_done = true;                                                                                                     \
                }                                                                                                                         \
                hipLaunchKernelGGL(tokred_pp_kernel<NIV>, dim3((unsigned)(ns * ntiles) + extra), dim3(512), lds_bytes, st, (const bf16*)dy, (long)ldy, \
                                   (const bf16*)x, (long)ldx, slab, cslab, Nout, (int)halves, halves_per, tiles_k, ntiles, ns * ntiles, red); \
                BF_CHECK_LAUNCH();                                                                                                        \
            }                                                                                                                             \
            if (fold) {                                                                                                                   \
                pend.on = true; pend.NI = NIV; pend.st = st;                                                                              \
                pend.r = FoldRed{slab, cslab, ns, ntiles, tiles_k, Nout, Kin, out, colsum, accumulate, 0};                                \
                break;                                                                                                                    \
            }                                                                                                                             \
            BfProfScope prof(st, "tokred_reduce_kernel", 0.0, (double)(ns + 1 + (accumulate ? 1 : 0)) * n * 4.0);                         \
            if (ns <= 8) hipLaunchKernelGGL((tokred_pp_reduce_kernel<NIV, 8>), dim3(rblocks), dim3(256), 0, st, slab, cslab, ns, ntiles, tiles_k, Nout, Kin, out, colsum, accumulate); \
            else hipLaunchKernelGGL((tokred_pp_reduce_kernel<NIV, MAX_SLICES>), dim3(rblocks), dim3(256), 0, st, slab, cslab, ns, ntiles, tiles_k, Nout, Kin, out, colsum, accumulate); \
            BF_CHECK_LAUNCH();                                                                                                            \
        } while (0)
        if (big) BF_PP_GO(6); else BF_PP_GO(3);
#undef BF_PP_GO
        return 0;
    }
    { const int frc = flush_pending(pending_slot(), st); if (frc) return frc; }
    const long steps = M / BK;
    int nslice = slices_env > 0 ? slices_env : 8;
    nslice = (int)std::max<long>(1, std::min<long>({(long)nslice, (long)MAX_SLICES, steps}));
    BF_REQUIRE(ws_floats >= (int64_t)nslice * (n + Nout), "bf_gemm_tokred: workspace too small (bf_gemm_tokred_ws_floats)");
    const int steps_per = bf_cdiv(steps, nslice);
    const int ns = bf_cdiv(steps, steps_per);
    const int tiles_k = Kin / TB, ntiles = (Nout / TB) * tiles_k;
    float* slab = ws;
    float* cslab = colsum ? ws + (size_t)ns * n : nullptr;
    {
        BfProfScope prof(st, "tokred_kernel<128x128,bk64,slots3>", 2.0 * Nout * Kin * (double)M, (double)M * (Nout + Kin) * 2.0 + (double)n * 4.0);
        static BfPerDeviceOnce attr_once; bool& attr_done = attr_once.flag();
        constexpr int lds_bytes = NSLOT * 2 * BK * TB * 2;
        if (!attr_done) {
            hipError_t e_ = hipFuncSetAttribute((const void*)tokred_kernel, hipFuncAttributeMaxDynamicSharedMemorySize, lds_bytes);
            if (e_ != hipSuccess) return bf_fail(e_, __FILE__, __LINE__);
            attr_done = true;
        }
        hipLaunchKernelGGL(tokred_kernel, dim3((unsigned)(ns * ntiles)), dim3(512), lds_bytes, st, (const bf16*)dy, (long)ldy, (const bf16*)x,
                           (long)ldx, slab, cslab, Nout, Kin, (int)steps, steps_per, tiles_k, ntiles);
        BF_CHECK_LAUNCH();
    }
    {
        BfProfScope prof(st, "tokred_reduce_kernel", 0.0, (double)(ns + 1 + (accumulate ? 1 : 0)) * n * 4.0);
        const int blocks = (int)std::min<long>(512, (n / 4 + 255) / 256);
        hipLaunchKernelGGL(tokred_reduce_kernel, dim3(blocks), dim3(256), 0, st, slab, cslab, ns, n, Nout, out, colsum, accumulate);
        BF_CHECK_LAUNCH();
    }
    return 0;
}

int bf_tokred_narrow(int dtype, int C, int64_t P, const void* wide, const void* narrow, float* out, int ldo, int accumulate, int transposed,
                     const float* sc, const float* sh, int64_t rows_per_frame, float* ws, int64_t ws_floats, hipStream_t st) {
    static const bool off = bf_knob("BF_TOKRED_NARROW", 1) == 0;
    if (off || dtype != BF_DTYPE_BF16 || (C != 96 && C != 64 && C != 32) || P <= 0 || P % NW_TILE || ldo < (transposed ? C : 16)) return 1;
    if (((uintptr_t)wide | (uintptr_t)narrow | (uintptr_t)ws) & 15) return 1;
    if (sc && (rows_per_frame <= 0 || rows_per_frame % NW_TILE)) return 1;
    const int wgs = sc ? 512 : 256;
    if (ws_floats < (int64_t)wgs * C * 16) return 1;
    const long tiles = P / NW_TILE;
    const int tpf = sc ? (int)(rows_per_frame / NW_TILE) : 1;
    BfProfScope prof(st, sc ? "tokred_narrow_kernel<gelu>" : "tokred_narrow_kernel", 2.0 * C * 16 * (double)P, (double)P * (C + 16) * 2.0);
#define BF_NARROW_GO(CTV)                                                                                                               \
    do {                                                                                                                                \
        constexpr int lds_bytes = 4 * 2 * (NW_TILE * 16 * CTV * 2 + NW_TILE * 16 * 2);                                                  \
        static_assert(lds_bytes >= 4 * 16 * CTV * 16 * 4, "the reduction buffer aliases the tile rings");                               \
        if (sc) hipLaunchKernelGGL((tokred_narrow_kernel<CTV, true>), dim3(wgs), dim3(256), lds_bytes, st, (const bf16*)wide, (const bf16*)narrow, tiles, ws, sc, sh, tpf); \
        else hipLaunchKernelGGL((tokred_narrow_kernel<CTV, false>), dim3(wgs), dim3(256), lds_bytes, st, (const bf16*)wide, (const bf16*)narrow, tiles, ws, sc, sh, tpf); \
    } while (0)
    if (C == 96) BF_NARROW_GO(6); else if (C == 64) BF_NARROW_GO(4); else BF_NARROW_GO(2);
#undef BF_NARROW_GO
    BF_CHECK_LAUNCH();
    hipLaunchKernelGGL(tokred_narrow_reduce_kernel, dim3(bf_cdiv(C * 16, 256)), dim3(256), 0, st, ws, wgs, C, out, ldo, accumulate, transposed);
    BF_CHECK_LAUNCH();
    return 0;
}
```

bubbleformer_amd/csrc/model.hip:

```cpp
#include "model_common.h"

bool bf_attn_raw_modes(int dtype, int d);
int bf_gemm_tokred_deferred(int dtype, int Nout, int Kin, int64_t M, const void* dy, int64_t ldy, const void* x, int64_t ldx, float* out,
                            int accumulate, float* colsum, float* ws, int64_t ws_floats, hipStream_t stream);
const float* bf_gemm_tokred_pending_out();
int bf_gemm_inbwd_frames_scaled(int dtype, int M, int N, int K, const void* A, int64_t lda, const void* B, int64_t ldb, const void* x,
                                const void* add, void* out, int S, const float* mean, const float* rstd, const float* w, float* ws,
                                const float* fscale, int fdiv, void* out_s, const float* f_s, int fdiv_s, hipStream_t stream);

using namespace bfm;

namespace {

bool g_side_defer = false;

BfPerDevice<TrunkLinks> g_links;

int launch_reduce_jobs(ReduceJobs& J, hipStream_t st);
__global__ void __launch_bounds__(256) stage_prep_multi_kernel(PrepBatch b);

}

bool bfm::side_defer() { return g_side_defer; }
TrunkLinks& bfm::links() { return g_links.get(); }
int bfm::flush_pending_reduce(TrunkLinks& L, hipStream_t st) {
    if (!L.reduce.on) return 0;
    L.reduce.on = false;
    TRY(launch_reduce_jobs(L.reduce.jobs, L.reduce.st));
    return L.hand_over(L.reduce.st, st);
}
int bfm::side_join_pending(TrunkLinks& L, hipStream_t main, int set) {
    if (set < 0) TRY(flush_pending_reduce(L, main));
    SideStream* s = L.side_stream();
    if (set < 0 && bf_gemm_tokred_pending()) {
        hipStream_t ws_st = s ? s->st : main;
        TRY(bf_gemm_tokred_flush(ws_st));
        if (s) { HIP_TRY(hipEventRecord(s->join, s->st)); HIP_TRY(hipStreamWaitEvent(main, s->join, 0)); }
    }
    if (!s) return 0;
    for (int i = 0; i < 2; ++i)
        if ((set < 0 || set == i) && s->pending[i]) {
            HIP_TRY(hipStreamWaitEvent(main, s->tail[i], 0));
            s->pending[i] = false;
        }
    return 0;
}
int bfm::launch_stage_prep(const D& d, const PrepBatch& b, int m, int planes, hipStream_t st) {
    hipLaunchKernelGGL(stage_prep_multi_kernel, dim3(std::max(64, d.E), planes, m), dim3(256), 0, st, b);
    BF_CHECK_LAUNCH();
    return 0;
}

namespace {

int launch_with_pending(TrunkLinks& L, ReduceJobs& J, hipStream_t st) {
    if (L.reduce.on && L.reduce.st == st && J.fits(L.reduce.jobs)) {
        L.reduce.on = false;
        const ReduceJobs& P = L.reduce.jobs;
        for (int i = 0; i < P.n_in; ++i) TRY(J.push(P.in[i]));
        for (int i = 0; i < P.n_attn; ++i) TRY(J.push(P.at[i]));
    }
    TRY(flush_pending_reduce(L, st));
    return launch_reduce_jobs(J, st);
}

__device__ __forceinline__ void outproj_prep_row(const float* __restrict__ W, const float* __restrict__ bias, const float* __restrict__ nb,
                                                 const float* __restrict__ gamma, const float* __restrict__ lo, const float* __restrict__ hi,
                                                 float* __restrict__ alpha, float* __restrict__ beta, float* __restrict__ mc, int E, int n,
                                                 void* __restrict__ wscaled, int dtype) {
    __shared__ float red[4];
    __shared__ float s_alpha;
    float acc = 0.f;
    if (lo) for (int k = threadIdx.x; k < E; k += blockDim.x) acc += W[(long)n * E + k] * nb[k];
    acc = wave_sum(acc);
    if ((threadIdx.x & 63) == 0) red[threadIdx.x >> 6] = acc;
    __syncthreads();
    if (threadIdx.x == 0) {
        float m = bias[n];
        for (int i = 0; i < (int)(blockDim.x >> 6); ++i) m += red[i];
        const float l = lo ? lo[n] : 0.f, h = hi ? hi[n] : 0.f, g = gamma[n];
        alpha[n] = g * (1.f + h);
        beta[n] = g * (bias[n] * (1.f + h) + (lo ? m * (l - h) : 0.f));
        mc[n] = m;
        s_alpha = g * (1.f + h);
    }
    if (wscaled) {
        __syncthreads();
        const float al = s_alpha;
// ... 216 lines not shown
        const InReduceJob& j = J.in[z];
        if ((int)blockIdx.x < (j.C + 63) / 64 && (int)blockIdx.y < (j.frames + j.rdiv() - 1) / j.rdiv()) in_reduce_block(j, blockIdx.x, blockIdx.y, red);
    } else {
        int a = z - J.n_in;
        if (J.at_follows[a]) return;
        for (;; ++a) {
            const AttnReduceJob& j = J.at[a];
            const int nvals = 4 * j.D + 32 * j.heads + j.heads;
            if ((int)blockIdx.x < (nvals + 63) / 64 && blockIdx.y == 0) attn_reduce_block(j, blockIdx.x, 0, 1, red);
            if (a + 1 >= J.n_attn || !J.at_follows[a + 1]) break;
            __syncthreads();
        }
    }
}
int launch_reduce_jobs(ReduceJobs& J, hipStream_t st) {
    int k = 0;
    for (int i = 0; i < J.n_attn; ++i) if (J.at[i].rows > 0) J.at[k++] = J.at[i];
    J.n_attn = k;
    for (int i = 0; i < J.n_attn; ++i)
        J.at_follows[i] = i > 0 && J.at[i].D == J.at[i - 1].D && J.at[i].heads == J.at[i - 1].heads &&
                          ((J.at[i].dqw && J.at[i].dqw == J.at[i - 1].dqw) || (J.at[i].demb && J.at[i].demb == J.at[i - 1].demb));
    if (J.n_in + J.n_attn == 0) return 0;
    int gx = 1, gy = 1;
    for (int i = 0; i < J.n_in; ++i) { gx = std::max(gx, bf_cdiv(J.in[i].C, 64)); gy = std::max(gy, bf_cdiv(J.in[i].frames, J.in[i].rdiv())); }
    for (int i = 0; i < J.n_attn; ++i) { gx = std::max(gx, bf_cdiv(4 * J.at[i].D + 33 * J.at[i].heads, 64)); }
    hipLaunchKernelGGL(stage_param_reduce_kernel, dim3(gx, gy, J.n_in + J.n_attn), dim3(64 * BF_RED_FL), 0, st, J);
    BF_CHECK_LAUNCH();
    return 0;
}

int qkv_gemm(const D& d, const void* xn, const void* w_c, const float* bias, void* qkv, hipStream_t st) {
    bf_operand A = op_plain(xn, d.E, BF_LAY_KC);
    bf_operand Bo = op_plain(w_c, d.E, BF_LAY_KC);
    bf_epilogue e = epi_store(qkv, 3L * d.E);
    e.bias = bias;
    return bf_gemm(d.dtype, (int)d.N, 3 * d.E, d.E, &A, &Bo, &e, 1, st);
}
int outproj_gemm(const D& d, const void* on, const void* w_c, const float* alpha, const float* beta,
                 const void* resid, void* out, const float* drop, long rows_per_group, hipStream_t st) {
    bf_operand A = op_plain(on, d.E, BF_LAY_KC);
    bf_operand Bo = op_plain(w_c, d.E, BF_LAY_KC);
    bf_epilogue e = epi_store(out, d.E);
    e.colscale = alpha; e.colshift = beta; e.aux_mode = BF_AUX_ADD; e.aux = resid; e.ld_aux = d.E;
    e.rowscale = drop; e.rows_per_group = (int)rows_per_group;
    return bf_gemm(d.dtype, (int)d.N, d.E, d.E, &A, &Bo, &e, 1, st);
}
void* bwd_scratch(TrunkLinks& L, const D& d, void* scratch) {
    if (!g_side_defer || !L.side_stream()) return scratch;
    L.scratch_parity ^= 1;
    return (char*)scratch + (size_t)L.scratch_parity * Scratch(d, nullptr).bytes;
}
struct TailNorm { const void* z; void* dz; const float *mean, *rstd, *w, *g; int gdiv; float* ws; bool* done; };
struct InFuse { const void* x; const void* add; void* dx; const float* mean; const float* rstd; const float* w; const float* b; float* ws;
                const float* fscale = nullptr; int fdiv = 1;
                const TailNorm* tail = nullptr;
                void* scaled_out = nullptr; const float* scaled_f = nullptr; int scaled_fdiv = 1; bool* scaled_done = nullptr; };
int dgrad_inbwd(const D& d, const void* dy, int Kdim, const void* w_xc, int Nout, void* tmp, const InFuse& f, hipStream_t st) {
    if (f.tail) {
        const TailNorm& t = *f.tail;
        const int crc = bf_gemm_inbwd_frames_chain(d.dtype, (int)d.N, Nout, Kdim, dy, Kdim, w_xc, Nout, f.x, f.add, f.dx, (int)d.S, f.mean, f.rstd, f.w, f.ws,
                                                   f.fscale, f.fdiv, t.z, t.dz, t.mean, t.rstd, t.w, t.g, t.gdiv, t.ws, st);
        if (crc < 0) return crc;
        if (crc == 0) { *t.done = true; return 0; }
    }
    if (f.scaled_out) {
        const int src = bf_gemm_inbwd_frames_scaled(d.dtype, (int)d.N, Nout, Kdim, dy, Kdim, w_xc, Nout, f.x, f.add, f.dx, (int)d.S, f.mean, f.rstd, f.w, f.ws,
                                                    f.fscale, f.fdiv, f.scaled_out, f.scaled_f, f.scaled_fdiv, st);
        if (src < 0) return src;
        if (src == 0) { *f.scaled_done = true; return 0; }
    }
    const int rc = bf_gemm_inbwd_frames(d.dtype, (int)d.N, Nout, Kdim, dy, Kdim, w_xc, Nout, f.x, f.add, f.dx, (int)d.S, f.mean, f.rstd, f.w, f.ws,
                                        f.fscale, f.fdiv, st);
    if (rc <= 0) return rc;
    bf_operand A = op_plain(dy, Kdim, BF_LAY_KC);
    bf_operand Bo = op_plain(w_xc, Nout, BF_LAY_XC);
    bf_epilogue e = epi_store(tmp, Nout);
    if (f.fscale) { e.rowscale = f.fscale; e.rows_per_group = (int)(d.S * f.fdiv); }
    TRY(bf_gemm(d.dtype, (int)d.N, Nout, Kdim, &A, &Bo, &e, 1, st));
    return bf_in_bwd_partials(d.dtype, tmp, f.x, f.add, f.dx, (int)d.F, (int)d.S, Nout, f.mean, f.rstd, f.w, f.b, nullptr, 1, 0, f.ws, st);
}
int outproj_bwd(const D& d, const Scratch& sc, const void* dout, const void* on, const void* w_s,
                const float* W, const float* bias, const float* nb, const float* gamma, const float* lo, const float* hi,
                const float* alpha, const float* mc, float* dW, float* dbias, float* dnb, float* dgamma, float* dlo, float* dhi,
                void* don, hipStream_t st, Fork& fk, const InFuse* fu = nullptr) {
    TRY(fk.run([=](hipStream_t ss) -> int {
        const void* dsrc = dout;
        const int trc = bf_gemm_tokred_deferred(d.dtype, d.E, d.E, d.N, dsrc, d.E, on, d.E, sc.G, 0, sc.csum, sc.tokred_ws, sc.tokred_floats, ss);
        if (trc < 0) return trc;
        if (trc == 1) {
            ZERO_ON(ss, sc.G, (size_t)((char*)sc.csum - (char*)sc.G) + (size_t)d.E * 4);
            bf_operand A = op_plain(dsrc, d.E, BF_LAY_XC);
            bf_operand Bo = op_plain(on, d.E, BF_LAY_XC);
            bf_epilogue e = epi_atomic(sc.G, d.E);
            e.colsum = sc.csum;
            TRY(bf_gemm(d.dtype, d.E, d.E, (int)d.N, &A, &Bo, &e, splitk_for(d.E, d.E, d.N), ss));
        }
        return 0;
    }));
    fk.run_late([=](hipStream_t ss) -> int {
        if (bf_gemm_tokred_pending_out() == sc.G) TRY(bf_gemm_tokred_flush(ss));
        hipLaunchKernelGGL(outproj_finalize_kernel, dim3(d.E + (lo ? bf_cdiv(d.E, 16) : 0)), dim3(256), 0, ss, sc.G, sc.csum, W, bias, nb, gamma, lo, hi, mc,
                           dW, dbias, dnb, dgamma, dlo, dhi, d.E);
        BF_CHECK_LAUNCH();
        return 0;
    });
    if (fu) return dgrad_inbwd(d, dout, d.E, w_s, d.E, don, *fu, st);
    {
        bf_operand A = op_plain(dout, d.E, BF_LAY_KC);
        bf_operand Bo = op_plain(w_s, d.E, BF_LAY_XC);
        bf_epilogue e = epi_store(don, d.E);
        TRY(bf_gemm(d.dtype, (int)d.N, d.E, d.E, &A, &Bo, &e, 1, st));
    }
    return 0;
}
int linear_bwd(const D& d, const Scratch& sc, const void* dy, int Nout, const void* x, int Kin, int xpro, const float* xsc, const float* xsh,
               const void* w_c, float* dW, float* db, void* dxn, const bf_epilogue* dx_epi, hipStream_t st, Fork& fk, const InFuse* fu = nullptr,
               bool last = false, const void* w_t = nullptr, void* scaled_out = nullptr, const float* rowfac = nullptr, int rpg = 1,
               bool* scaled_done = nullptr) {
    TRY(fk.run([=](hipStream_t ss) -> int {
        const void* xo = x;
        int pro = xpro;
        bf_operand A = op_plain(dy, Nout, BF_LAY_XC);
        if (pro == BF_PRO_AFFINE) {
            TRY(bf_affine_apply(d.dtype, x, nullptr, xsc, xsh, sc.s1, d.N, (int)d.S, Kin, ss));
            xo = sc.s1;
            pro = BF_PRO_NONE;
        }
        bf_operand Bo = op_plain(xo, Kin, BF_LAY_XC);
        if (pro == BF_PRO_NONE) {
            const int trc = bf_gemm_tokred_deferred(d.dtype, Nout, Kin, d.N, dy, Nout, xo, Kin, dW, 1, db, sc.tokred_ws, sc.tokred_floats, ss);
            if (trc <= 0) return trc;
        }
        if (pro != BF_PRO_NONE) op_affine(Bo, pro, xsc, xsh, d.S, Kin);
        bf_epilogue e = epi_atomic(dW, Kin);
        e.colsum = db;
        return bf_gemm(d.dtype, Nout, Kin, (int)d.N, &A, &Bo, &e, splitk_for(Nout, Kin, d.N), ss);
    }));
    if (last) TRY(fk.flush());
    if (fu) return dgrad_inbwd(d, dy, Nout, w_c, Kin, dxn, *fu, st);
    {
        bf_operand A = op_plain(dy, Nout, BF_LAY_KC);
        bf_operand Bo = w_t ? op_plain(w_t, Nout, BF_LAY_KC) : op_plain(w_c, Kin, BF_LAY_XC);
        bf_epilogue e = dx_epi ? *dx_epi : epi_store(dxn, Kin);
        e.c = dxn; e.ldc = Kin;
        if (scaled_out && rowfac && d.dtype == BF_DTYPE_BF16) {
            const int rc = bf_gemm_pair_scaled((int)d.N, Kin, Nout, &A, &Bo, &e, scaled_out, rowfac, rpg, st);
            if (rc < 0) return rc;
            if (rc == 0) { if (scaled_done) *scaled_done = true; return 0; }
        }
        TRY(bf_gemm(d.dtype, (int)d.N, Kin, Nout, &A, &Bo, &e, 1, st));
    }
    return 0;
}

}

extern "C" int64_t bf_temporal_saved_bytes(const bf_dims* s) { D d; if (get_dims(s, &d)) return -1; return (int64_t)TemporalSaved(d, nullptr).bytes; }
extern "C" int64_t bf_spatial_saved_bytes(const bf_dims* s) { D d; if (get_dims(s, &d)) return -1; return (int64_t)SpatialSaved(d, nullptr).bytes; }
static size_t dbr_bytes(const D& d) { return (((size_t)d.N * d.E * d.es) + 255) & ~(size_t)255; }
extern "C" int64_t bf_scratch_bytes(const bf_dims* s) { D d; if (get_dims(s, &d)) return -1; return 2 * (int64_t)Scratch(d, nullptr).bytes + 2 * (int64_t)dbr_bytes(d); }

extern "C" void bf_side_defer(int on) { g_side_defer = on != 0; }
extern "C" int bf_side_join(bf_stream_t s) { return side_join_pending(g_links.get(), (hipStream_t)s); }

extern "C" void bf_stage_prepared(int on) { g_links.get().hints.prepared = on != 0; }
extern "C" int bf_stage_chain_tail(const bf_spatial_params* prev_p, const void* prev_saved, int has_drop_mlp) {
    g_links.get().hints.tail = NextTail{prev_p && prev_saved, prev_p, prev_saved, has_drop_mlp != 0};
    return 0;
}
extern "C" int bf_stage_next_scale(const float* factors, int fdiv) { g_links.get().hints.scale = NextScale{factors, fdiv > 0 ? fdiv : 1}; return 0; }
static NextHead next_head(const D& d, int kind, const void* params, void* saved) {
    auto of = [&](auto* np, const auto& sv) { return NextHead{true, np->norm1_w, np->norm1_b, sv.mean1, sv.rstd1, sv.sc1, sv.sh1, sv.xn, saved}; };
    return kind == 0 ? of((const bf_temporal_params*)params, TemporalSaved(d, saved)) : of((const bf_spatial_params*)params, SpatialSaved(d, saved));
}
extern "C" int bf_stage_chain_next(const bf_dims* dims, int next_kind, const void* next_params, void* next_saved) {
    NextHead& h = g_links.get().hints.head;
    h = NextHead{};
    if (!dims || !next_params || !next_saved) return 0;
    BF_REQUIRE(next_kind == 0 || next_kind == 1, "bf_stage_chain_next: kind must be 0 (temporal) or 1 (spatial)");
    D d; TRY(get_dims(dims, &d));
    h = next_head(d, next_kind, next_params, next_saved);
    return 0;
}
extern "C" int bf_stage_chain_head(const bf_dims* dims, const bf_temporal_params* next_p, void* next_saved) {
    return bf_stage_chain_next(dims, 0, next_p, next_saved);
}

static int temporal_fwd(TrunkLinks& L, const StageHints& H, const bf_dims* dims, const bf_temporal_params* p, const void* x, void* out, void* saved,
                        void* scratch, const float* drop, bf_stream_t s) {
    D d; TRY(get_dims(dims, &d));
    BF_REQUIRE(p && x && out && saved && scratch, "bf_temporal_fwd: null pointer");
    hipStream_t st = (hipStream_t)s;
    const bool head_done = L.take_head_done(saved, st);
    TRY(side_join_pending(L, st));
    TemporalSaved sv(d, saved);
    Scratch sc(d, scratch);
    const void* wv[4];
    TRY(wviews(d, stage_prep(d, 0, p, sv.prep_dst(), nullptr), H.prepared, wv, st));
    const void *win_c = wv[0], *wout_c = wv[1];
    if (!head_done)
        TRY(bf_in_stats_apply(d.dtype, x, (int)d.F, (int)d.S, d.E, p->norm1_w, p->norm1_b, nullptr, 1, nullptr, sv.mean1, sv.rstd1, sv.sc1, sv.sh1, sc.in_ws,
                              nullptr, sv.xn, st));
    TRY(qkv_gemm(d, sv.xn, win_c, p->input_head_b, sv.qkv, st));
    TRY(bf_attn_fwd(d.dtype, sv.qkv, sv.o, (long)d.B * d.S, d.T, d.S, (long)d.T * d.S, 1, d.S, d.heads, d.d, p->qnorm_w, p->qnorm_b,
                    p->knorm_w, p->knorm_b, p->rel_pos_emb, d.attn_scale ? p->attn_scale_factor : nullptr, 1.f, 0, st));
    TRY(bf_in_stats_apply(d.dtype, sv.o, (int)d.F, (int)d.S, d.E, p->norm2_w, p->norm2_b, nullptr, 1, nullptr, sv.mean2, sv.rstd2, sv.sc2, sv.sh2, sc.in_ws,
                          nullptr, sv.on, st));
    if (H.head.armed) {
        const NextHead& h = H.head;
        const bf_frame_norm n2{h.w, h.b, nullptr, 1, h.mean, h.rstd, h.sc, h.sh, nullptr, h.xn};
        const int rc = bf_gemm_fwd_frames(d.dtype, (int)d.N, d.E, d.E, sv.on, d.E, sv.wout_t, d.E, nullptr, sv.alpha, sv.beta, drop, d.T, x, out, (int)d.S,
                                          nullptr, &n2, s);
        if (rc < 0) return rc;
        if (rc == 0) { L.head_done = {h.saved, st}; return 0; }
    }
    TRY(outproj_gemm(d, sv.on, wout_c, sv.alpha, sv.beta, x, out, drop, (long)d.T * d.S, st));
    return 0;
}

static int temporal_bwd(TrunkLinks& L, const StageHints& H, const bf_dims* dims, const bf_temporal_params* p, const bf_temporal_params* g, const void* x,
                        const void* dout, void* dx, void* saved, void* scratch, const float* drop, bf_stream_t s) {
    D d; TRY(get_dims(dims, &d));
    BF_REQUIRE(p && g && x && dout && dx && saved && scratch, "bf_temporal_bwd: null pointer");
    hipStream_t st = (hipStream_t)s;
    TemporalSaved sv(d, saved);
    Scratch sc(d, bwd_scratch(L, d, scratch));
    const void* win_c = d.dtype == BF_DTYPE_F32 ? (const void*)p->input_head_w : sv.win_c;
    Fork fk(L, st, true, L.scratch_parity);
    if (fk.deferred) TRY(side_join_pending(L, st, fk.set));
    void* don = sc.t1;
    void* dO = sc.t1b;
    void* dqkv = sc.t3;
    const void* dbr = dout;
    if (drop) {
        const TrunkLinks::DbrReady& r = L.dbr_ready;
        if (r.dx == dout && r.f == drop && r.buf && r.st == st) dbr = r.buf;
        else {
            TRY(bf_frame_scale(d.dtype, dout, drop, d.T, sc.t4, d.N, (int)d.S, d.E, st));
            dbr = sc.t4;
        }
    }
    L.dbr_ready = TrunkLinks::DbrReady{};
    const InFuse fu2{sv.o, nullptr, dO, sv.mean2, sv.rstd2, p->norm2_w, p->norm2_b, sc.in_ws2};
    TRY(outproj_bwd(d, sc, dbr, sv.on, sv.wout_s, p->output_head_w, p->output_head_b, p->norm2_b, p->gamma, nullptr, nullptr,
                    sv.alpha, sv.mc, g->output_head_w, g->output_head_b, nullptr, g->gamma, nullptr, nullptr, don, st, fk, &fu2));
    ReduceJobs jobs;
    TRY(jobs.push(InReduceJob{sc.in_ws2, (int)d.F, d.E, p->norm2_w, p->norm2_b, nullptr, 1, g->norm2_w, g->norm2_b, nullptr, nullptr, nullptr, nullptr}));
    {
        int rows = 0;
        TRY(bf_attn_bwd_partials(d.dtype, sv.qkv, dO, dqkv, (long)d.B * d.S, d.T, d.S, (long)d.T * d.S, 1, d.S, d.heads, d.d, p->qnorm_w, p->qnorm_b,
                                 p->knorm_w, p->knorm_b, p->rel_pos_emb, d.attn_scale ? p->attn_scale_factor : nullptr, g->qnorm_w, g->qnorm_b,
                                 g->knorm_w, g->knorm_b, g->rel_pos_emb, d.attn_scale ? g->attn_scale_factor : nullptr, 1.f, 0, sc.attn_ws,
                                 Scratch::ATTN_WS_FLOATS, &rows, st));
        TRY(jobs.push(AttnReduceJob{sc.attn_ws, rows, d.d, d.heads, g->qnorm_w, g->qnorm_b, g->knorm_w, g->knorm_b, g->rel_pos_emb,
                                    d.attn_scale ? g->attn_scale_factor : nullptr}));
    }
    void* dxn = sc.t1;
    InFuse fu1{x, dout, dx, sv.mean1, sv.rstd1, p->norm1_w, p->norm1_b, sc.in_ws};
    TailNorm tn;
    bool tail_done = false;
    static const bool chain_on = bf_knob("BF_BWD_CHAIN", 1) != 0;
    if (H.tail.armed && chain_on && fk.deferred && d.dtype == BF_DTYPE_BF16 && d.S == 144 && d.F % 2 == 0) {
        const NextTail& h = H.tail;
        const int oset = L.scratch_parity ^ 1;
        TRY(side_join_pending(L, st, oset));
        Scratch so(d, (char*)scratch + (size_t)oset * Scratch(d, nullptr).bytes);
        SpatialSaved ps(d, const_cast<void*>(h.saved));
        tn = TailNorm{ps.z, so.t1, ps.mean3, ps.rstd3, h.p->mlp_norm_w, h.drop ? ps.gtab : h.p->gamma_mlp, h.drop ? 1 : (int)d.F, L.tail_ws_flip ? so.in_ws5 : so.in_ws4, &tail_done};
        L.tail_ws_flip = !L.tail_ws_flip;
        fu1.tail = &tn;
    }
    if (H.tail.armed) L.tail_done = TrunkLinks::TailDone{};
    TRY(linear_bwd(d, sc, dqkv, 3 * d.E, sv.xn, d.E, BF_PRO_NONE, nullptr, nullptr, win_c, g->input_head_w, g->input_head_b, dxn, nullptr, st, fk, &fu1, true));
    if (tail_done) L.tail_done = {H.tail.saved, dx, tn.ws, st};
    TRY(jobs.push(InReduceJob{sc.in_ws, (int)d.F, d.E, p->norm1_w, p->norm1_b, nullptr, 1, g->norm1_w, g->norm1_b, nullptr, nullptr, nullptr, nullptr}));
    TRY(launch_with_pending(L, jobs, st));
    return fk.join();
}
extern "C" int bf_temporal_fwd(const bf_dims* dims, const bf_temporal_params* p, const void* x, void* out, void* saved, void* scratch,
                               const float* drop, bf_stream_t s) {
    TrunkLinks& L = g_links.get();
    return temporal_fwd(L, L.take_hints(), dims, p, x, out, saved, scratch, drop, s);
}
extern "C" int bf_temporal_bwd(const bf_dims* dims, const bf_temporal_params* p, const bf_temporal_params* g, const void* x, const void* dout,
                               void* dx, void* saved, void* scratch, const float* drop, bf_stream_t s) {
    TrunkLinks& L = g_links.get();
    return temporal_bwd(L, L.take_hints(), dims, p, g, x, dout, dx, saved, scratch, drop, s);
}

static int prep_stages(TrunkLinks& L, const bf_dims* dims, int n, const int32_t* kinds, const void* const* params, void* const* saved,
                       const float* const* drop_mlp, bf_stream_t s) {
    D d; TRY(get_dims(dims, &d));
    BF_REQUIRE(n >= 1 && kinds && params && saved, "bf_prep_stages: bad arguments");
    if (d.dtype != BF_DTYPE_BF16) return 1;
    hipStream_t st = (hipStream_t)s;
    TRY(side_join_pending(L, st));
    for (int i0 = 0; i0 < n; i0 += PREP_BATCH) {
        PrepBatch b;
        memset(&b, 0, sizeof(b));
        const int m = std::min(PREP_BATCH, n - i0);
        for (int i = 0; i < m; ++i) {
            const int k = i0 + i;
            BF_REQUIRE(params[k] && saved[k] && (kinds[k] == 0 || kinds[k] == 1), "bf_prep_stages: bad stage entry");
            b.s[i] = kinds[k] == 0 ? stage_prep(d, 0, params[k], TemporalSaved(d, saved[k]).prep_dst(), nullptr)
                                   : stage_prep(d, 1, params[k], SpatialSaved(d, saved[k]).prep_dst(), drop_mlp ? drop_mlp[k] : nullptr);
        }
        TRY(launch_stage_prep(d, b, m, 7, st));
    }
    return 0;
}
extern "C" int bf_prep_stages(const bf_dims* dims, int n, const int32_t* kinds, const void* const* params, void* const* saved,
                              const float* const* drop_mlp, bf_stream_t s) {
    return prep_stages(g_links.get(), dims, n, kinds, params, saved, drop_mlp, s);
}

static int spatial_fwd(TrunkLinks& L, const StageHints& H, const bf_dims* dims, const bf_spatial_params* p, const void* x, void* out, void* saved,
                       void* scratch, const float* drop_att, const float* drop_mlp, bf_stream_t s) {
    D d; TRY(get_dims(dims, &d));
    BF_REQUIRE(p && x && out && saved && scratch, "bf_spatial_fwd: null pointer");
    hipStream_t st = (hipStream_t)s;
    const bool head_done = L.take_head_done(saved, st);
    TRY(side_join_pending(L, st));
    SpatialSaved sv(d, saved);
    Scratch sc(d, scratch);
    const void* wv[4];
    TRY(wviews(d, stage_prep(d, 1, p, sv.prep_dst(), drop_mlp), H.prepared, wv, st));
    const void *win_c = wv[0], *wout_c = wv[1], *w1_c = wv[2], *w2_c = wv[3];
    if (!head_done)
// ... 38 lines not shown
        const int rc = bf_gemm_fwd_frames(d.dtype, (int)d.N, d.E, 4 * d.E, sv.hid, 4L * d.E, sv.w2t_c, d.E, p->fc2_b, nullptr, nullptr, nullptr, 1, nullptr, sv.z,
                                          (int)d.S, &n1, h.armed ? &n2 : nullptr, s);
        if (rc < 0) return rc;
        if (rc == 0) {
            if (h.armed) L.head_done = {h.saved, st};
            return 0;
        }
    }
    {
        bf_operand A = op_plain(sv.hid, 4L * d.E, BF_LAY_KC);
        bf_operand Bo = op_plain(w2_c, 4L * d.E, BF_LAY_KC);
        bf_epilogue e = epi_store(sv.z, d.E);
        e.bias = p->fc2_b;
        TRY(bf_gemm(d.dtype, (int)d.N, d.E, 4 * d.E, &A, &Bo, &e, 1, st));
    }
    if (H.head.armed) {
        const NextHead& h = H.head;
        bool chained = false;
        TRY(bf_in_stats_apply_chain(d.dtype, sv.z, (int)d.F, (int)d.S, d.E, p->mlp_norm_w, p->mlp_norm_b, g3, g3div, nullptr, sv.mean3, sv.rstd3, sv.sc3, sv.sh3,
                                    sc.in_ws, sv.x1, out, h.w, h.b, h.mean, h.rstd, h.sc, h.sh, h.xn, &chained, st));
        if (chained) L.head_done = {h.saved, st};
        return 0;
    }
    TRY(bf_in_stats_apply(d.dtype, sv.z, (int)d.F, (int)d.S, d.E, p->mlp_norm_w, p->mlp_norm_b, g3, g3div, nullptr, sv.mean3, sv.rstd3,
                          sv.sc3, sv.sh3, sc.in_ws, sv.x1, out, st));
    return 0;
}

static int spatial_bwd(TrunkLinks& L, const StageHints& H, const bf_dims* dims, const bf_spatial_params* p, const bf_spatial_params* g, const void* x,
                       const void* dout, void* dx, void* saved, void* scratch, const float* drop_att, const float* drop_mlp, bf_stream_t s) {
    D d; TRY(get_dims(dims, &d));
    BF_REQUIRE(p && g && x && dout && dx && saved && scratch, "bf_spatial_bwd: null pointer");
    hipStream_t st = (hipStream_t)s;
    SpatialSaved sv(d, saved);
    Scratch sc(d, bwd_scratch(L, d, scratch));
    const bool f32 = d.dtype == BF_DTYPE_F32;
    const void* win_c = f32 ? (const void*)p->input_head_w : sv.win_c;
    const void* w1_c = f32 ? (const void*)p->fc1_w : sv.w1_c;
    const void* w2_c = f32 ? (const void*)p->fc2_w : sv.w2_c;
    TRY(flush_pending_reduce(L, st));
    Fork fk(L, st, true, L.scratch_parity);
    if (fk.deferred) TRY(side_join_pending(L, st, fk.set));
    void* dz = sc.t1;
    ReduceJobs jobs;
    const TrunkLinks::TailDone td = L.tail_done;
    L.tail_done = TrunkLinks::TailDone{};
    const bool tail_done = td.saved == saved && td.dx == dout && td.st == st;
    {
        const float* gsc = drop_mlp ? sv.gtab : p->gamma_mlp;
        const int gdiv = drop_mlp ? 1 : (int)d.F;
        if (!tail_done)
            TRY(bf_in_bwd_partials(d.dtype, dout, sv.z, nullptr, dz, (int)d.F, (int)d.S, d.E, sv.mean3, sv.rstd3, p->mlp_norm_w, p->mlp_norm_b, gsc, gdiv, 0, sc.in_ws3, st));
        TRY(jobs.push(InReduceJob{tail_done ? td.ws : sc.in_ws3, (int)d.F, d.E, p->mlp_norm_w, p->mlp_norm_b, gsc, gdiv, g->mlp_norm_w, g->mlp_norm_b,
                                  drop_mlp ? nullptr : g->gamma_mlp, nullptr, drop_mlp, drop_mlp ? g->gamma_mlp : nullptr}));
    }
    void* dpre = sc.t4;
    {
        bf_epilogue e; memset(&e, 0, sizeof(e));
        e.aux_mode = BF_AUX_DGELU; e.aux = sv.pre; e.ld_aux = 4L * d.E; e.out_mode = BF_OUT_STORE;
        static const bool use_t = bf_knob("BF_FC2_DGRAD_T", 1) != 0;
        TRY(linear_bwd(d, sc, dz, d.E, sv.hid, 4 * d.E, BF_PRO_NONE, nullptr, nullptr, w2_c, g->fc2_w, g->fc2_b, dpre, &e, st, fk, nullptr, false,
                       (!f32 && use_t) ? sv.w2t_c : nullptr));
    }
    void* dx1 = sc.t1b;
    bool dbr_done = false;
    {
        bf_epilogue e; memset(&e, 0, sizeof(e));
        e.aux_mode = BF_AUX_ADD; e.aux = dout; e.ld_aux = d.E; e.out_mode = BF_OUT_STORE;
        TRY(linear_bwd(d, sc, dpre, 4 * d.E, sv.x1, d.E, BF_PRO_NONE, nullptr, nullptr, w1_c, g->fc1_w, g->fc1_b, dx1, &e, st, fk, nullptr, false, nullptr,
                       drop_att ? sc.e5 : nullptr, drop_att, (int)d.S, &dbr_done));
    }
    void* don = sc.e6;
    const void* dbr = dx1;
    if (dbr_done) dbr = sc.e5;
    else if (drop_att) {
        TRY(bf_frame_scale(d.dtype, dx1, drop_att, 1, sc.e5, d.N, (int)d.S, d.E, st));
        dbr = sc.e5;
    }
    void* dO = sc.e7;
    const InFuse fu2{sv.o, nullptr, dO, sv.mean2, sv.rstd2, p->norm2_w, p->norm2_b, sc.in_ws2};
    TRY(outproj_bwd(d, sc, dbr, sv.on, sv.wout_s, p->output_head_w, p->output_head_b, p->norm2_b, p->gamma_att,
                    d.feat_scale ? p->low_freq_scalar : nullptr, d.feat_scale ? p->high_freq_scalar : nullptr, sv.alpha, sv.mc,
                    g->output_head_w, g->output_head_b, g->norm2_b, g->gamma_att, d.feat_scale ? g->low_freq_scalar : nullptr,
                    d.feat_scale ? g->high_freq_scalar : nullptr, don, st, fk, &fu2));
    TRY(jobs.push(InReduceJob{sc.in_ws2, (int)d.F, d.E, p->norm2_w, p->norm2_b, nullptr, 1, g->norm2_w, g->norm2_b, nullptr, nullptr, nullptr, nullptr}));
    void* dqkv = sc.t3;
    {
        int rows = 0;
        static const bool raw_on = bf_knob("BF_ATTN_RAW", 1) != 0;
        const bool rawm = raw_on && bf_attn_raw_modes(d.dtype, d.d);
        TRY(bf_attn_bwd_partials(d.dtype, sv.qkv, dO, dqkv, d.F * d.h, d.w, 1, d.w, 0, 1, d.heads, d.d, p->qnorm_w, p->qnorm_b, p->knorm_w, p->knorm_b,
                                 p->rel_pos_emb, d.attn_scale ? p->attn_scale_factor_x : nullptr, g->qnorm_w, g->qnorm_b, g->knorm_w, g->knorm_b,
                                 g->rel_pos_emb, d.attn_scale ? g->attn_scale_factor_x : nullptr, 0.5f, rawm ? 2 : 0, sc.attn_ws, Scratch::ATTN_WS_FLOATS, &rows, st));
        TRY(jobs.push(AttnReduceJob{sc.attn_ws, rows, d.d, d.heads, g->qnorm_w, g->qnorm_b, g->knorm_w, g->knorm_b, g->rel_pos_emb,
                                    d.attn_scale ? g->attn_scale_factor_x : nullptr}));
        TRY(bf_attn_bwd_partials(d.dtype, sv.qkv, dO, dqkv, d.F * d.w, d.h, d.w, d.S, 1, d.w, d.heads, d.d, p->qnorm_w, p->qnorm_b, p->knorm_w, p->knorm_b,
                                 p->rel_pos_emb, d.attn_scale ? p->attn_scale_factor_y : nullptr, g->qnorm_w, g->qnorm_b, g->knorm_w, g->knorm_b,
                                 g->rel_pos_emb, d.attn_scale ? g->attn_scale_factor_y : nullptr, 0.5f, rawm ? 5 : 1, sc.attn_ws2, Scratch::ATTN_WS_FLOATS, &rows, st));
        TRY(jobs.push(AttnReduceJob{sc.attn_ws2, rows, d.d, d.heads, g->qnorm_w, g->qnorm_b, g->knorm_w, g->knorm_b, g->rel_pos_emb,
                                    d.attn_scale ? g->attn_scale_factor_y : nullptr}));
    }
    void* dxn = sc.e6;
    InFuse fu1{x, dx1, dx, sv.mean1, sv.rstd1, p->norm1_w, p->norm1_b, sc.in_ws};
    bool scaled_done = false;
    const NextScale& ns = H.scale;
    L.dbr_ready = TrunkLinks::DbrReady{};
    static const bool scaled_on = bf_knob("BF_BWD_SCALED_COPY", 1) != 0;
    if (ns.f && scaled_on && fk.deferred && d.dtype == BF_DTYPE_BF16) {
        fu1.scaled_out = (char*)scratch + 2 * Scratch(d, nullptr).bytes + (L.dbr_flip ? dbr_bytes(d) : 0);
        fu1.scaled_f = ns.f; fu1.scaled_fdiv = ns.fdiv; fu1.scaled_done = &scaled_done;
    }
    TRY(linear_bwd(d, sc, dqkv, 3 * d.E, sv.xn, d.E, BF_PRO_NONE, nullptr, nullptr, win_c, g->input_head_w, g->input_head_b, dxn, nullptr, st, fk, &fu1, true));
    if (scaled_done) { L.dbr_ready = {dx, ns.f, fu1.scaled_out, st}; L.dbr_flip = !L.dbr_flip; }
    TRY(jobs.push(InReduceJob{sc.in_ws, (int)d.F, d.E, p->norm1_w, p->norm1_b, nullptr, 1, g->norm1_w, g->norm1_b, nullptr, nullptr, nullptr, nullptr}));
    static const bool merge_on = bf_knob("BF_REDUCE_MERGE", 1) != 0;
    if (fk.deferred && merge_on) { L.reduce.jobs = jobs; L.reduce.on = true; L.reduce.st = st; }
    else TRY(launch_reduce_jobs(jobs, st));
    return fk.join();
}
extern "C" int bf_spatial_fwd(const bf_dims* dims, const bf_spatial_params* p, const void* x, void* out, void* saved, void* scratch,
                              const float* drop_att, const float* drop_mlp, bf_stream_t s) {
    TrunkLinks& L = g_links.get();
    return spatial_fwd(L, L.take_hints(), dims, p, x, out, saved, scratch, drop_att, drop_mlp, s);
}
extern "C" int bf_spatial_bwd(const bf_dims* dims, const bf_spatial_params* p, const bf_spatial_params* g, const void* x, const void* dout,
                              void* dx, void* saved, void* scratch, const float* drop_att, const float* drop_mlp, bf_stream_t s) {
    TrunkLinks& L = g_links.get();
    return spatial_bwd(L, L.take_hints(), dims, p, g, x, dout, dx, saved, scratch, drop_att, drop_mlp, s);
}

extern "C" int bf_trunk_train_fwd(const bf_dims* dims, int n, const int32_t* kinds, const void* const* params, void* const* saved,
                                  const float* const* drop_a, const float* const* drop_b, const void* x, void* const* acts, void* scratch,
                                  bf_stream_t s) {
    D d; TRY(get_dims(dims, &d));
    BF_REQUIRE(n >= 1 && kinds && params && saved && x && acts && scratch, "bf_trunk_train_fwd: bad arguments");
    for (int i = 0; i < n; ++i)
        BF_REQUIRE(params[i] && saved[i] && acts[i] && (kinds[i] == 0 || kinds[i] == 1), "bf_trunk_train_fwd: bad stage entry");
    TrunkLinks& L = g_links.get();
    (void)L.take_hints();
    const bool b16 = d.dtype == BF_DTYPE_BF16;
    if (b16) {
        const int rc = prep_stages(L, dims, n, kinds, params, saved, drop_b, s);
        if (rc < 0) return rc;
    }
    for (int i = 0; i < n; ++i) {
        const void* in = i ? acts[i - 1] : x;
        StageHints H;
        H.prepared = b16;
        if (b16 && i + 1 < n && kinds[i + 1] != kinds[i]) H.head = next_head(d, kinds[i + 1], params[i + 1], saved[i + 1]);
        TRY(kinds[i] == 0
            ? temporal_fwd(L, H, dims, (const bf_temporal_params*)params[i], in, acts[i], saved[i], scratch, drop_a ? drop_a[i] : nullptr, s)
            : spatial_fwd(L, H, dims, (const bf_spatial_params*)params[i], in, acts[i], saved[i], scratch, drop_a ? drop_a[i] : nullptr,
                          drop_b ? drop_b[i] : nullptr, s));
    }
    return 0;
}

extern "C" int bf_trunk_train_bwd(const bf_dims* dims, int n, const int32_t* kinds, const void* const* params, const void* const* grads,
                                  void* const* saved, const float* const* drop_a, const float* const* drop_b, const void* x, void* const* acts,
                                  const void* dout, void* const* gbuf3, void* dx, void* scratch, bf_stage_done_fn stage_done, void* user,
                                  bf_stream_t s) {
    D d; TRY(get_dims(dims, &d));
    BF_REQUIRE(n >= 1 && kinds && params && grads && saved && x && acts && dout && gbuf3 && dx && scratch, "bf_trunk_train_bwd: bad arguments");
    BF_REQUIRE(gbuf3[0] && gbuf3[1] && gbuf3[2], "bf_trunk_train_bwd: three gradient buffers are needed");
    TrunkLinks& L = g_links.get();
    (void)L.take_hints();
    const void* cur = dout;
    int rot = 0;
    for (int i = n - 1; i >= 0; --i) {
        BF_REQUIRE(params[i] && grads[i] && saved[i] && (kinds[i] == 0 || kinds[i] == 1), "bf_trunk_train_bwd: bad stage entry");
        const void* in = i ? acts[i - 1] : x;
        void* gout = i ? gbuf3[rot] : dx;
        rot = (rot + 1) % 3;
        StageHints H;
        if (kinds[i] == 0) {
            if (i > 0 && kinds[i - 1] == 1) H.tail = NextTail{true, (const bf_spatial_params*)params[i - 1], saved[i - 1], drop_b && drop_b[i - 1]};
            TRY(temporal_bwd(L, H, dims, (const bf_temporal_params*)params[i], (const bf_temporal_params*)grads[i], in, cur, gout, saved[i], scratch,
                             drop_a ? drop_a[i] : nullptr, s));
        } else {
            if (i > 0 && kinds[i - 1] == 0 && drop_a && drop_a[i - 1]) H.scale = NextScale{drop_a[i - 1], d.T};
            TRY(spatial_bwd(L, H, dims, (const bf_spatial_params*)params[i], (const bf_spatial_params*)grads[i], in, cur, gout, saved[i], scratch,
                            drop_a ? drop_a[i] : nullptr, drop_b ? drop_b[i] : nullptr, s));
        }
        if (stage_done) stage_done(i, user);
        cur = gout;
    }
    return 0;
}
```

bubbleformer_amd/csrc/model_common.h:

```cpp
#pragma once
#include <algorithm>
#include <functional>
#include <vector>
#include "bf_common.h"
#include "param_reduce.h"
#include <stdlib.h>
#include <string.h>

int bf_gemm_tokred_flush(hipStream_t st);
bool bf_gemm_tokred_pending();

namespace bfm __attribute__((visibility("hidden"))) {

struct D {
    int dtype, B, T, h, w, E, heads, attn_scale, feat_scale, patch, cin, cout, nfluid;
    long N, F, S;
    int d, nst;
    size_t es;
};
inline int get_dims(const bf_dims* s, D* o) {
    if (!s) return bf_fail_msg("dims: null", __FILE__, __LINE__);
    o->dtype = s->dtype; o->B = s->B; o->T = s->T; o->h = s->h; o->w = s->w; o->E = s->E; o->heads = s->heads;
    o->attn_scale = s->attn_scale; o->feat_scale = s->feat_scale; o->patch = s->patch; o->cin = s->cin; o->cout = s->cout;
    o->nfluid = s->nfluid;
    if (o->B < 1 || o->T < 1 || o->h < 1 || o->w < 1 || o->E < 8 || o->E > 1024 || o->heads < 1 || o->E % o->heads)
        return bf_fail_msg("dims: bad sizes", __FILE__, __LINE__);
    if (o->dtype != BF_DTYPE_F32 && o->dtype != BF_DTYPE_BF16) return bf_fail_msg("dims: bad dtype", __FILE__, __LINE__);
    o->F = (long)o->B * o->T; o->S = (long)o->h * o->w; o->N = o->F * o->S; o->d = o->E / o->heads;
    o->es = bf_esize(o->dtype);
    const int ch = o->dtype == BF_DTYPE_BF16 ? 8 : 4;
    if (o->E % ch || o->d % ch) return bf_fail_msg("dims: E and head dim must be multiples of the 16-byte chunk", __FILE__, __LINE__);
    if (o->T > 128 || o->h > 128 || o->w > 128) return bf_fail_msg("dims: attention axes are limited to 128 tokens", __FILE__, __LINE__);
    o->nst = 0;
    if (o->patch > 0) {
        int p = o->patch;
        while (p > 1) { if (p & 1) return bf_fail_msg("dims: patch must be a power of two", __FILE__, __LINE__); p >>= 1; o->nst++; }
        if (o->nst < 1 || o->nst > BF_MAX_STAGES) return bf_fail_msg("dims: patch size out of range", __FILE__, __LINE__);
        if (o->nst > 1 && (o->E / 4) % ch) return bf_fail_msg("dims: E/4 must be a multiple of the 16-byte chunk", __FILE__, __LINE__);
    }
    return 0;
}

struct Arena {
    char* base; size_t off;
    explicit Arena(void* p) : base((char*)p), off(0) {}
    void* take(size_t bytes) { void* r = base ? base + off : nullptr; off += (bytes + 255) & ~(size_t)255; return r; }
    float* f32(size_t n) { return (float*)take(n * 4); }
};

inline bf_operand op_plain(const void* p, long ld, int layout) {
    bf_operand o; memset(&o, 0, sizeof(o)); o.p = p; o.ld = ld; o.layout = layout; return o;
}
inline void op_affine(bf_operand& o, int pro, const float* sc, const float* sh, long rpf, int nch) {
    o.pro = pro; o.sc = sc; o.sh = sh; o.rows_per_frame = (int)rpf; o.nch = nch;
}
inline void op_gather(bf_operand& o, int gw, int gh, int C) { o.gw = gw; o.gh = gh; o.gc = C; o.seglen = 2 * C; o.segstride = 2L * gw * C; }
inline bf_epilogue epi_store(void* c, long ldc) { bf_epilogue e; memset(&e, 0, sizeof(e)); e.c = c; e.ldc = ldc; e.out_mode = BF_OUT_STORE; return e; }
inline bf_epilogue epi_atomic(float* c, long ldc) { bf_epilogue e = epi_store(c, ldc); e.out_mode = BF_OUT_ATOMIC_F32; return e; }
inline void epi_scatter(bf_epilogue& e, int gw, int gh, int C) { e.gw = gw; e.gh = gh; e.gc = C; e.seglen = 2 * C; e.segstride = 2L * gw * C; }

inline int splitk_for(int M, int N, long K) {
    const long tiles = (long)bf_cdiv(M, 128) * bf_cdiv(N, 128);
    static const long target = bf_knob("BF_SPLITK_TARGET", 256);
    long s = (target + tiles / 2) / tiles;
    const long kt = (K + 63) / 64;
    if (s > kt / 4) s = kt / 4;
    if (s < 1) s = 1;
    return (int)s;
}

#define TRY(x) do { int rc__ = (x); if (rc__) return rc__; } while (0)
#define ZERO(ptr, bytes) do { hipError_t e__ = hipMemsetAsync((ptr), 0, (bytes), st); if (e__ != hipSuccess) return bf_fail(e__, __FILE__, __LINE__); } while (0)
#define ZERO_ON(stream, ptr, bytes) do { hipError_t e__ = hipMemsetAsync((ptr), 0, (bytes), (stream)); if (e__ != hipSuccess) return bf_fail(e__, __FILE__, __LINE__); } while (0)
#define HIP_TRY(x) do { hipError_t e__ = (x); if (e__ != hipSuccess) return bf_fail(e__, __FILE__, __LINE__); } while (0)

struct SideStream { hipStream_t st = nullptr; hipEvent_t fork = nullptr, join = nullptr, tail[2] = {nullptr, nullptr}; bool failed = false; bool pending[2] = {false, false}; };
bool side_defer();

struct NextHead { bool armed = false; const float *w = nullptr, *b = nullptr; float *mean = nullptr, *rstd = nullptr, *sc = nullptr, *sh = nullptr; void* xn = nullptr; const void* saved = nullptr; };
struct NextTail { bool armed = false; const bf_spatial_params* p = nullptr; const void* saved = nullptr; bool drop = false; };
struct NextScale { const float* f = nullptr; int fdiv = 1; };
struct StageHints { bool prepared = false; NextHead head; NextTail tail; NextScale scale; };

struct ReduceJobs {
    static constexpr int IN_CAP = 6, ATTN_CAP = 4;
    int n_in = 0, n_attn = 0; InReduceJob in[IN_CAP]; AttnReduceJob at[ATTN_CAP];
    bool at_follows[ATTN_CAP] = {};
    bool fits(const ReduceJobs& o) const { return n_in + o.n_in <= IN_CAP && n_attn + o.n_attn <= ATTN_CAP; }
    int push(const InReduceJob& j) { BF_REQUIRE(n_in < IN_CAP, "ReduceJobs: more InstanceNorm reductions than one launch holds"); in[n_in++] = j; return 0; }
    int push(const AttnReduceJob& j) { BF_REQUIRE(n_attn < ATTN_CAP, "ReduceJobs: more attention reductions than one launch holds"); at[n_attn++] = j; return 0; }
};

struct TrunkLinks {
    StageHints hints;
    StageHints take_hints() { const StageHints h = hints; hints = StageHints{}; return h; }
    struct HeadDone { const void* saved = nullptr; hipStream_t st = nullptr; } head_done;
    struct TailDone { const void* saved = nullptr; const void* dx = nullptr; float* ws = nullptr; hipStream_t st = nullptr; } tail_done;
    struct DbrReady { const void* dx = nullptr; const float* f = nullptr; void* buf = nullptr; hipStream_t st = nullptr; } dbr_ready;
    int scratch_parity = 0; bool tail_ws_flip = false, dbr_flip = false;
    bool take_head_done(const void* saved, hipStream_t st) { const bool hit = head_done.saved == saved && head_done.st == st; head_done = HeadDone{}; return hit; }
    struct { ReduceJobs jobs; bool on = false; hipStream_t st = nullptr; } reduce;
    hipEvent_t handoff = nullptr;
    SideStream side;
    std::vector<const void*> embed_lean;

    SideStream* side_stream() {
        static const bool enabled = bf_knob("BF_SIDE_STREAM", 1) != 0;
        if (!enabled) return nullptr;
        SideStream& s = side;
        if (!s.st && !s.failed) {
            int lo = 0, hi = 0;
            (void)hipDeviceGetStreamPriorityRange(&lo, &hi);
            const unsigned ef = hipEventDisableTiming | hipEventDisableSystemFence;
            if (hipStreamCreateWithPriority(&s.st, hipStreamNonBlocking, lo) != hipSuccess || hipEventCreateWithFlags(&s.fork, ef) != hipSuccess ||
                hipEventCreateWithFlags(&s.join, ef) != hipSuccess || hipEventCreateWithFlags(&s.tail[0], ef) != hipSuccess ||
                hipEventCreateWithFlags(&s.tail[1], ef) != hipSuccess) { s.failed = true; s.st = nullptr; }
        }
        return s.st ? &s : nullptr;
    }
    int hand_over(hipStream_t from, hipStream_t to) {
        if (from == to) return 0;
        if (!handoff) HIP_TRY(hipEventCreateWithFlags(&handoff, hipEventDisableTiming));
        HIP_TRY(hipEventRecord(handoff, from));
        HIP_TRY(hipStreamWaitEvent(to, handoff, 0));
        return 0;
    }
    void clear(bool forward_side) {
        if (forward_side) { hints.prepared = false; hints.head = NextHead{}; head_done = HeadDone{}; }
        hints.tail = NextTail{}; hints.scale = NextScale{}; tail_done = TailDone{}; dbr_ready = DbrReady{};
    }
    bool embed_lean_get(const void* saved) const { return std::find(embed_lean.begin(), embed_lean.end(), saved) != embed_lean.end(); }
    void embed_lean_set(const void* saved, bool lean) {
        const auto it = std::find(embed_lean.begin(), embed_lean.end(), saved);
        if (it == embed_lean.end()) { if (lean) embed_lean.push_back(saved); }
        else if (!lean) { *it = embed_lean.back(); embed_lean.pop_back(); }
    }
};
TrunkLinks& links();
int flush_pending_reduce(TrunkLinks& L, hipStream_t st);
int side_join_pending(TrunkLinks& L, hipStream_t main, int set = -1);

struct Fork {
    hipStream_t main; SideStream* s; bool used = false; bool deferred; int set;
    std::vector<std::function<int(hipStream_t)>> jobs;
    std::vector<std::function<int(hipStream_t)>> late;
    hipStream_t last_side = nullptr;
    explicit Fork(TrunkLinks& L, hipStream_t m, bool may_defer = false, int scratch_set = 0) : main(m), s(L.side_stream()), set(scratch_set) {
        deferred = may_defer && side_defer() && s != nullptr;
    }
    int begin(hipStream_t* out) {
        *out = main;
        if (!s) return 0;
        HIP_TRY(hipEventRecord(s->fork, main));
        HIP_TRY(hipStreamWaitEvent(s->st, s->fork, 0));
        used = true;
        *out = s->st;
        return 0;
    }
    template <class F> int run(F&& job) {
        hipStream_t ss;
        const int rc = begin(&ss);
        last_side = ss;
        return rc ? rc : job(ss);
    }
    template <class F> void run_late(F&& job) { late.push_back(job); }
    int drain_late() {
        if (late.empty()) return 0;
        hipStream_t ss = last_side ? last_side : main;
        for (auto& j : late) TRY(j(ss));
        late.clear();
        return 0;
    }
    int flush() {
        if (!deferred || jobs.empty()) return 0;
        hipStream_t ss;
        TRY(begin(&ss));
        for (auto& j : jobs) TRY(j(ss));
        jobs.clear();
        return 0;
    }
    int join() {
        if (deferred) {
            TRY(flush());
            TRY(drain_late());
            if (used) { HIP_TRY(hipEventRecord(s->tail[set], s->st)); s->pending[set] = true; used = false; }
            return 0;
        }
        TRY(drain_late());
        if (bf_gemm_tokred_pending()) TRY(bf_gemm_tokred_flush(last_side ? last_side : main));
        if (!s || !used) return 0;
        HIP_TRY(hipEventRecord(s->join, s->st));
        HIP_TRY(hipStreamWaitEvent(main, s->join, 0));
        used = false;
        return 0;
    }
};

struct Scratch {
    float *G, *csum, *zeros, *ones, *wg, *attn_ws, *attn_ws2, *in_ws, *in_ws2, *in_ws3, *in_ws4, *in_ws5;
    float* tokred_ws; int64_t tokred_floats;
    static constexpr long ATTN_WS_FLOATS = 1024L * (4 * 128 + 32 * 16 + 16);
    void *t1, *t3, *t4, *t1b; int64_t t1b_floats;
    void *s1, *e5, *e6, *e7;
    size_t bytes;
    Scratch(const D& d, void* base) {
        Arena a(base);
        const int cm = d.nst > 1 ? d.E / 4 : d.E;
        size_t wgn = (size_t)d.E * d.E;
        wgn = std::max(wgn, (size_t)4 * cm * d.E);
        wgn = std::max(wgn, (size_t)d.E * 64);
        G = a.f32((size_t)d.E * d.E);
        csum = a.f32((size_t)4 * d.E);
        zeros = a.f32((size_t)4 * d.E);
        ones = a.f32((size_t)4 * d.E);
        wg = a.f32(wgn);
        tokred_floats = bf_gemm_tokred_ws_floats(4 * d.E, d.E, d.N);
        tokred_ws = a.f32((size_t)tokred_floats);
        attn_ws = a.f32(ATTN_WS_FLOATS);
        attn_ws2 = a.f32(ATTN_WS_FLOATS);
        {
            int64_t n = bf_in_ws_floats(d.dtype, (int)d.F, (int)d.S, d.E);
            long Si = d.S;
            for (int i = 1; i < d.nst; ++i) { Si *= 4; n = std::max(n, bf_in_ws_floats(d.dtype, (int)d.F, (int)Si, cm)); }
            in_ws = a.f32((size_t)n);
            const size_t nt = (size_t)bf_in_ws_floats(d.dtype, (int)d.F, (int)d.S, d.E);
            in_ws2 = a.f32(nt); in_ws3 = a.f32(nt); in_ws4 = a.f32(nt); in_ws5 = a.f32(nt);
        }
        size_t tok = (size_t)d.N * d.E;
        size_t big = tok * 4;
        if (d.patch > 1) {
            const size_t P0 = (size_t)d.N * (d.patch / 2) * (d.patch / 2);
            const int kp = ((4 * std::max(d.cin, d.cout) + 7) / 8) * 8;
            big = std::max(big, P0 * (size_t)std::max(cm, kp) * 2);
        }
        t4 = a.take(big * d.es);
        t3 = a.take(std::max(tok * 3, big / 2) * d.es);
        t1 = a.take(std::max(tok, big / 2) * d.es);
        t1b = a.take(std::max(tok, big / 2) * d.es);
        t1b_floats = (int64_t)(std::max(tok, big / 2) * d.es / 4);
        s1 = a.take(tok * d.es); e5 = a.take(tok * d.es); e6 = a.take(tok * d.es); e7 = a.take(tok * d.es);
        bytes = a.off;
    }
};

struct PrepArgs { const float *W, *bias, *nb, *gamma, *lo, *hi; float *alpha, *beta, *mc; int E;
                  void* wscaled; int dtype;
                  const float *tab_m, *tab_v; float* tab_out; int tab_F;
                  const float* tr_src; void* tr_dst; int tr_R, tr_C; };
struct Cast4 { const float* src[4]; bf16* dst[4]; long n[4]; };
struct StagePrep { Cast4 j; int cnt; PrepArgs a; };
constexpr int PREP_BATCH = 12;
struct PrepBatch { StagePrep s[PREP_BATCH]; };
struct PrepDst { void *win_c, *wout_c, *w1_c, *w2_c; float *alpha, *beta, *mc; void *wout_s, *wt; float* gtab; };

inline StagePrep stage_prep(const D& d, int kind, const void* params, const PrepDst& o, const float* drop_mlp) {
    const long EE = (long)d.E * d.E;
    StagePrep r;
    memset(&r, 0, sizeof(r));
    auto cast = [&r](const float* src, void* dst, long n) { r.j.src[r.cnt] = src; r.j.dst[r.cnt] = (bf16*)dst; r.j.n[r.cnt] = n; ++r.cnt; };
    const float *W, *bias, *nb, *gamma, *lo = nullptr, *hi = nullptr, *tab_v = nullptr, *tr_src;
    int tr_C;
    if (kind == 0) {
        const bf_temporal_params* p = (const bf_temporal_params*)params;
        cast(p->input_head_w, o.win_c, 3 * EE); cast(p->output_head_w, o.wout_c, EE);
        for (int q = 2; q < 4; ++q) { r.j.src[q] = r.j.src[0]; r.j.dst[q] = r.j.dst[0]; }
        W = p->output_head_w; bias = p->output_head_b; nb = p->norm2_b; gamma = p->gamma;
        tr_src = p->output_head_w; tr_C = d.E;
    } else {
        const bf_spatial_params* p = (const bf_spatial_params*)params;
        cast(p->input_head_w, o.win_c, 3 * EE); cast(p->output_head_w, o.wout_c, EE); cast(p->fc1_w, o.w1_c, 4 * EE); cast(p->fc2_w, o.w2_c, 4 * EE);
        W = p->output_head_w; bias = p->output_head_b; nb = p->norm2_b; gamma = p->gamma_att;
        if (d.feat_scale) { lo = p->low_freq_scalar; hi = p->high_freq_scalar; }
        tab_v = p->gamma_mlp;
        tr_src = p->fc2_w; tr_C = 4 * d.E;
    }
    const bool tab = drop_mlp && tab_v && o.gtab && d.dtype != BF_DTYPE_F32;
    const bool tr = o.wt && d.dtype == BF_DTYPE_BF16;
    r.a = PrepArgs{W, bias, nb, gamma, lo, hi, o.alpha, o.beta, o.mc, d.E, o.wout_s, d.dtype,
                   tab ? drop_mlp : nullptr, tab ? tab_v : nullptr, tab ? o.gtab : nullptr, tab ? (int)d.F : 0,
                   tr ? tr_src : nullptr, tr ? o.wt : nullptr, tr ? d.E : 0, tr ? tr_C : 0};
    return r;
}
int launch_stage_prep(const D& d, const PrepBatch& b, int m, int planes, hipStream_t st);

}
```

include/bubbleformer_hip.h:

```cpp
#ifndef BUBBLEFORMER_HIP_H
#define BUBBLEFORMER_HIP_H

#include <stdint.h>

#ifdef __cplusplus
extern "C" {
#endif

typedef void* bf_stream_t;

enum { BF_DTYPE_F32 = 0, BF_DTYPE_BF16 = 1 };

enum { BF_LAY_KC = 0,
       BF_LAY_XC = 1   };
enum { BF_PRO_NONE = 0, BF_PRO_AFFINE = 1, BF_PRO_AFFINE_GELU = 2, BF_PRO_GELU = 3 };
enum { BF_AUX_NONE = 0, BF_AUX_ADD = 1 , BF_AUX_DGELU = 2  };
enum { BF_OUT_STORE = 0 , BF_OUT_ATOMIC_F32 = 2 ,
       BF_OUT_STORE_F32 = 1  };

typedef struct bf_operand {
    const void* p;
    int64_t ld;
    int32_t layout;
    int32_t seglen;
    int64_t segstride;
    int32_t gw, gh, gc;
    int32_t pro;
    const float* sc;
    const float* sh;
    int32_t rows_per_frame;
    int32_t nch;
} bf_operand;

typedef struct bf_epilogue {
    const float* bias;
    const float* colscale;
    const float* colshift;
    int32_t aux_mode;
    const void* aux;
    int64_t ld_aux;
    int32_t out_mode;
    void* c;
    int64_t ldc;
    int32_t seglen;
    int64_t segstride;
    int32_t gw, gh, gc;
    void* gelu_out;
    float* colsum;
    const float* rowscale;
    int32_t rows_per_group;
} bf_epilogue;

int bf_gemm(int dtype, int M, int N, int K, const bf_operand* A, const bf_operand* B, const bf_epilogue* E,
            int splitk, bf_stream_t stream);

int bf_gemm_inbwd_frames(int dtype, int M, int N, int K, const void* A, int64_t lda, const void* B, int64_t ldb, const void* x,
                         const void* add, void* out, int S, const float* mean, const float* rstd, const float* w, float* ws,
                         const float* fscale , int fdiv,
                         bf_stream_t stream);
int bf_gemm_inbwd_frames_chain(int dtype, int M, int N, int K, const void* A, int64_t lda, const void* B, int64_t ldb, const void* x,
                               const void* add, void* out, int S, const float* mean, const float* rstd, const float* w, float* ws,
                               const float* fscale, int fdiv, const void* cz, void* cdz, const float* cmean, const float* crstd,
                               const float* cw, const float* cg, int cgdiv, float* cws, bf_stream_t stream);

typedef struct bf_frame_norm {
    const float *w, *b;
    const float* g; int32_t gdiv;
    float *mean, *rstd, *sc, *sh;
    const void* resid;
    void* out;
} bf_frame_norm;
int bf_gemm_fwd_frames(int dtype, int M, int N, int K, const void* A, int64_t lda, const void* Bt, int64_t ldb, const float* bias,
                       const float* colscale, const float* colshift, const float* fscale, int fdiv, const void* add, void* out, int S,
                       const bf_frame_norm* n1, const bf_frame_norm* n2, bf_stream_t stream);

int bf_gemm_tokred(int dtype, int Nout, int Kin, int64_t M, const void* dy, int64_t ldy, const void* x, int64_t ldx, float* out,
                   int accumulate, float* colsum, float* ws, int64_t ws_floats, bf_stream_t stream);
int64_t bf_gemm_tokred_ws_floats(int Nout, int Kin, int64_t M);

int bf_frame_linear(int dtype, int frames, int S, int K, int N, const void* A, int64_t lda, const void* W, int64_t ldw,
                    const float* norm_w, const float* norm_b, const float* bias, const float* colscale, const float* colshift,
                    const void* resid, int64_t ldr, int gelu, const float* en_w, const float* en_b, const float* en_g,
                    void* out, int64_t ldo,
                    const float* next_w, const float* next_b, void* out_n, int64_t ldn,
                    bf_stream_t stream);


int bf_in_stats(int dtype, const void* x, int frames, int S, int C, const float* w, const float* b, const float* g, int gdiv,
                const float* gb, float* mean, float* rstd, float* sc, float* sh,
                float* ws ,
                bf_stream_t stream);
int64_t bf_in_ws_floats(int dtype, int frames, int S, int C);
int bf_affine_apply(int dtype, const void* z, const void* resid, const float* sc, const float* sh, void* out, int64_t nrows,
                    int S, int C, bf_stream_t stream);
int bf_in_bwd(int dtype, const void* dy, const void* x, const void* add, void* dx, int frames, int S, int C, const float* mean,
              const float* rstd, const float* w, const float* b, const float* g, int gdiv, int gelu, float* dw, float* db,
              float* dg, float* dgb, float* ws ,
              bf_stream_t stream);
int bf_colsum(int dtype, const void* x, int64_t nrows, int C, const float* scale, float* out, bf_stream_t stream);

int bf_attn_fwd(int dtype, const void* qkv, void* out, int64_t nseq, int L, int64_t inner, int64_t outer_stride,
                int64_t inner_stride, int64_t tok_stride, int heads, int d, const float* qw, const float* qb, const float* kw,
                const float* kb, const float* emb, const float* hscale, float out_scale, int accumulate, bf_stream_t stream);
int bf_attn_axial_fwd(int dtype, const void* qkv, void* out, int64_t frames, int h, int w, int heads, int d, const float* qw,
                      const float* qb, const float* kw, const float* kb, const float* emb, const float* hscale_x,
                      const float* hscale_y, bf_stream_t stream);
int bf_attn_axial_norm_fwd(int dtype, const void* qkv, void* out, void* out_n, int64_t frames, int h, int w, int heads, int d,
                           const float* qw, const float* qb, const float* kw, const float* kb, const float* emb, const float* hscale_x,
                           const float* hscale_y, const float* norm_w, const float* norm_b, float* mean, float* rstd, float* sc,
                           float* sh, bf_stream_t stream);
int bf_attn_bwd(int dtype, const void* qkv, const void* dout, void* dqkv, int64_t nseq, int L, int64_t inner,
                int64_t outer_stride, int64_t inner_stride, int64_t tok_stride, int heads, int d, const float* qw,
                const float* qb, const float* kw, const float* kb, const float* emb, const float* hscale, float* dqw,
                float* dqb, float* dkw, float* dkb, float* demb, float* dhscale, float out_scale, int accumulate,
                float* ws, int64_t ws_floats,
                bf_stream_t stream);

void bf_side_defer(int on);
int bf_side_join(bf_stream_t stream);
void bf_debug_force_generic_attn(int on);
void bf_debug_tokred_fold(int on);

int bf_im2col_nchw(int dtype, const float* x, void* out, int frames, int C, int H, int W, int Kp, bf_stream_t stream);
int bf_col2im_nchw(int dtype, const void* g, float* dx, int frames, int C, int H, int W, int Kp, bf_stream_t stream);
#define BF_LOSS_LIMBS 5
int bf_pm2nchw(const float* pm, float* pred, const float* y, float* lossbuf, int frames, int Co, int h, int w, int Np,
               bf_stream_t stream);
int bf_debed_last(int dtype, const void* act, const float* sc, const float* sh, const void* wc, float* pred, const float* y,
                  float* lossbuf, int frames, int Ci, int Co, int h, int w, int Np, bf_stream_t stream);
int bf_debed_last_bwd(int dtype, const float* dpred, const float* pred, const float* y, const float* coef, const float* gscale,
                      const void* wc, void* dpm, void* dact, int frames, int Ci, int Co, int h, int w, int Np, bf_stream_t stream);
int bf_debed_last_bwd_norm(int dtype, const float* dpred, const float* pred, const float* y, const float* coef, const float* gscale,
                           const void* wc, void* dpm, const void* ymap, const float* mean, const float* rstd, const float* in_w,
                           const float* in_b, void* dx, float* d_in_w, float* d_in_b, int frames, int Ci, int Co, int h, int w, int Np,
                           float* ws, int64_t ws_floats, bf_stream_t stream);
int bf_embed_first(int dtype, const float* x, const void* wc, void* patches, void* y0, int frames, int C0, int cin, int h2, int w2,
                   int Kp, float* stat_part, bf_stream_t stream);
int bf_in_stats_merge_slices(int dtype, int frames, int S, int C, int rows, const float* w, const float* b, const float* g, int gdiv,
                             const float* gb, float* mean, float* rstd, float* sc, float* sh, float* ws, bf_stream_t stream);
int bf_gather_gemm(int dtype, const void* map, const void* w, int w_kn, const float* sc, const float* sh, void* out, int frames, int gh,
                   int gw, int C0, int N, bf_stream_t stream);
int bf_scatter_gemm(int dtype, const void* a, const void* w, int w_kn, const float* sc, const float* sh, void* map, float* stat_part, int frames,
                    int gh, int gw, int K, int C0, bf_stream_t stream);
int64_t bf_gather_wgrad_ws_floats(int frames, int gh, int gw);
int bf_gather_wgrad(int dtype, const void* fine, const void* coarse, const float* fsc, const float* fsh, const float* csc, const float* csh,
                    float* out, int transposed, int frames, int gh, int gw, int C0, int Kc, float* ws, int64_t ws_floats, bf_stream_t stream);
int bf_gather_gemm_rebuilt(int dtype, const void* patches, const void* w0c, const void* w, int w_kn, const float* sc, const float* sh, void* out,
                           int frames, int gh, int gw, int C0, int N, bf_stream_t stream);
int bf_gather_wgrad_rebuilt(int dtype, const void* patches, const void* w0c, const void* coarse, const float* fsc, const float* fsh, float* out,
                            int transposed, int frames, int gh, int gw, int C0, int Kc, float* ws, int64_t ws_floats, bf_stream_t stream);
int64_t bf_embed_tail_ws_floats(int frames, int gh1, int gw1, int C0, int Kp);
int bf_embed_tail_bwd(int dtype, const void* dy1, const void* w1c, const void* y0, const void* patches, const void* w0c, const float* sc,
                      const float* sh, const float* mean, const float* rstd, const float* in_w, float* dwprep, float* d_in_w, float* d_in_b,
                      int frames, int gh1, int gw1, int C1, int C0, int Kp, float* ws, int64_t ws_floats, bf_stream_t stream);
int bf_lploss_finalize(const float* lossbuf, int frames, int Co, float* loss, float* coef, bf_stream_t stream);
int bf_nchw2pm(int dtype, const float* dpred, const float* pred, const float* y, const float* coef, const float* gscale,
               void* dpm, int frames, int Co, int h, int w, int Np, bf_stream_t stream);
int bf_wprep(int dtype, int mode, const float* src, void* dst, int R, int K, int Kp, bf_stream_t stream);
int bf_wgrad_unprep(int mode, const float* gsrc, float* gdst, int R, int K, int Kp, int transposed, bf_stream_t stream);
int bf_film_net_fwd(const float* cond, const float* lnw, const float* lnb, const float* W, const float* bias, float* gb,
                    float* chat, float* crstd, int B, int P, int E2, bf_stream_t stream);
int bf_film_net_bwd(const float* dgb, const float* chat, const float* lnw, const float* lnb, const float* W, float* dW,
                    float* dbias, float* dlnw, float* dlnb, int B, int P, int E2, bf_stream_t stream);
int bf_clip_gather(const float* src, int64_t field_stride, const int32_t* field, const int64_t* first, int t0, const float* diff,
                   const float* div, float* out, int B, int T, int C, int H, int W, int Ho, int Wo, bf_stream_t stream);
int bf_clip_gather_batch(const float* src, int64_t field_stride, const int64_t* idx, int64_t nsamples, const int64_t* first_tab, const int32_t* in_field,
                         const float* in_diff, const float* in_div, int Cin, int Tin, float* in_out, const int32_t* out_field,
                         const float* out_diff, const float* out_div, int Cout, int Tout, float* out_out, const float* fluid_tab,
                         const int64_t* file_tab, int P, float* fluid_out, int B, int H, int W, int Ho, int Wo, bf_stream_t stream);
int bf_clip_gather_unroll(const float* src, int64_t field_stride, int64_t nframes, const int64_t* idx, int64_t nsamples, const int64_t* first_tab,
                          const int32_t* in_field, const float* in_diff, const float* in_div, int Cin, int Tin, float* in_out,
                          const int32_t* out_field, const float* out_diff, const float* out_div, int Cout, int Tout, int unroll, float* out_out,
                          const float* fluid_tab, const int64_t* file_tab, int P, float* fluid_out, int B, int H, int W, int Ho, int Wo,
                          bf_stream_t stream);
typedef struct bf_clip_gather_job {
    const float* src; const int64_t *idx, *first_tab;
    const int32_t* in_field; const float *in_diff, *in_div; float* in_out;
    const int32_t* out_field; const float *out_diff, *out_div; float* out_out;
    const float* fluid_tab; const int64_t* file_tab; float* fluid_out;
    int64_t field_stride, nframes, nsamples;
    int32_t Cin, Tin, Cout, Tout, unroll, P, B, H, W, Ho, Wo, reserved;
} bf_clip_gather_job;
typedef struct bf_clip_augment {
    const int32_t *in_odd, *out_odd;
    int64_t seed, flip_thr;
    int32_t draw, Hc, Wc, crop_y, eval_view, reserved;
} bf_clip_augment;
int bf_clip_gather_augment(const bf_clip_gather_job* job, const bf_clip_augment* augment, bf_stream_t stream);
typedef struct bf_clip_gather_q16_job {
    const uint16_t* codes; const int32_t* frame_seg; const float *seg_lo, *seg_step;
    const int64_t *idx, *first_tab;
    const int32_t* in_field; const float *in_diff, *in_div; float* in_out;
    const int32_t* out_field; const float *out_diff, *out_div; float* out_out;
    const float* fluid_tab; const int64_t* file_tab; float* fluid_out;
    int64_t field_stride, nframes, nsamples;
    int32_t nfiles, Cin, Tin, Cout, Tout, unroll, P, B, H, W, Ho, Wo;
} bf_clip_gather_q16_job;
int bf_clip_encode_q16(const float* src, uint16_t* dst, int64_t n, float lo, float inv, bf_stream_t stream);
int bf_clip_decode_q16(const uint16_t* codes, int64_t field_stride, const int32_t* frame_seg, const float* seg_lo, const float* seg_step, float* dst,
                       int64_t nframes, int nfields, int nfiles, int H, int W, bf_stream_t stream);
int bf_clip_gather_q16(const bf_clip_gather_q16_job* job, const bf_clip_augment* augment, bf_stream_t stream);
int bf_clip_noise(const float* src, float* dst, const float* sigma, const int64_t* sample_ids, uint64_t seed, uint32_t draw, uint32_t pass,
                  int B, int T, int C, int H, int W, bf_stream_t stream);
int64_t bf_field_stats_ws_doubles(int nseg);
// ... 247 lines not shown
```

Before: 816.1 samples/s.

## Co-schedule weight-gradient tokred cells as riders inside the inbwd pair GEMM launch

Moves the token-reduction ping-pong body into a shared header. It adds a ride kernel variant of the pair GEMM that launches extra workgroups to compute weight-gradient token-reduction cells alongside the input-backward GEMM, followed by a commit step. The aim is to fill idle CUs during the input-backward GEMM and drop a separate wgrad launch. It raises dynamic LDS to the larger of the two footprints and adds a planning and commit path. Whether it runs depends on callers and a debug toggle, and the Python caller is not shown.

Result: slower. 803.9 samples/s (-1.5%).

```diff
diff --git a/bubbleformer_amd/_lib.py b/bubbleformer_amd/_lib.py
--- a/bubbleformer_amd/_lib.py
+++ b/bubbleformer_amd/_lib.py
@@ -140,6 +140,7 @@
     "bf_prof_enable": (None, [C.c_int]),
     "bf_debug_force_generic_attn": (None, [C.c_int]),
     "bf_debug_tokred_fold": (None, [C.c_int]),
+    "bf_debug_wgrad_ride": (None, [C.c_int]),
     "bf_side_defer": (None, [C.c_int]),
     "bf_prep_stages": (C.c_int, [C.POINTER(Dims), C.c_int, C.POINTER(C.c_int32), C.POINTER(vp), C.POINTER(vp), C.POINTER(vp), vp]),
     "bf_stage_prepared": (None, [C.c_int]),
@@ -166,6 +167,8 @@
     "bf_gemm_inbwd_frames": (C.c_int, [C.c_int, C.c_int, C.c_int, C.c_int, vp, i64, vp, i64, vp, vp, vp, C.c_int, fp, fp, fp, fp, fp, C.c_int, vp]),
     "bf_gemm_inbwd_frames_chain": (C.c_int, [C.c_int, C.c_int, C.c_int, C.c_int, vp, i64, vp, i64, vp, vp, vp, C.c_int, fp, fp, fp, fp, fp, C.c_int,
                                              vp, vp, fp, fp, fp, fp, C.c_int, fp, vp]),
+    "bf_gemm_inbwd_frames_ride_wgrad": (C.c_int, [C.c_int, C.c_int, C.c_int, C.c_int, vp, i64, vp, i64, vp, vp, vp, C.c_int, fp, fp, fp, fp, fp, C.c_int,
+                                                  C.c_int, C.c_int, vp, i64, vp, i64, fp, C.c_int, fp, fp, i64, C.c_int, vp]),
     "bf_in_stats": (C.c_int, [C.c_int, vp, C.c_int, C.c_int, C.c_int, fp, fp, fp, C.c_int, fp, fp, fp, fp, fp, fp, vp]),
     "bf_in_ws_floats": (i64, [C.c_int, C.c_int, C.c_int, C.c_int]),
     "bf_affine_apply": (C.c_int, [C.c_int, vp, vp, fp, fp, vp, i64, C.c_int, C.c_int, vp]),
diff --git a/bubbleformer_amd/csrc/gemm_frame.hip b/bubbleformer_amd/csrc/gemm_frame.hip
--- a/bubbleformer_amd/csrc/gemm_frame.hip
+++ b/bubbleformer_amd/csrc/gemm_frame.hip
@@ -1,4 +1,5 @@
 #include "gemm_common.h"
+#include "tokred_pp.h"
 #include <stdlib.h>
 #include <string.h>
 #include <type_traits>
@@ -620,15 +621,29 @@
 }
 
 template <int MODE>
-__global__ void __launch_bounds__(512) gemm_pair_kernel(PairArgs a) {
-    extern __shared__ __attribute__((aligned(16))) unsigned char smem[];
+__device__ __forceinline__ void pair_wg(const PairArgs& a, unsigned char* smem, int bid, int nwg) {
     const int tid = threadIdx.x, lane = tid & 63, wave = __builtin_amdgcn_readfirstlane(tid >> 6);
-    const int seq = xcd_remap(blockIdx.x, gridDim.x);
+    const int seq = xcd_remap(bid, nwg);
     const int fp = seq / a.nt;
     const int m0 = fp * PM, n0 = (seq - fp * a.nt) * PN;
     const int f0 = ((MODE == 0 || MODE == 2 || MODE == 5) && a.whole) ? fp : 2 * fp;
     if (wave < 4) pair_body<MODE, 0>(a, smem, lane, wave, m0, n0, f0);
     else pair_body<MODE, 1>(a, smem, lane, wave - 4, m0, n0, f0);
+}
+template <int MODE>
+__global__ void __launch_bounds__(512) gemm_pair_kernel(PairArgs a) {
+    extern __shared__ __attribute__((aligned(16))) unsigned char smem[];
+    pair_wg<MODE>(a, smem, blockIdx.x, gridDim.x);
+}
+template <int MODE>
+__global__ void __launch_bounds__(512) gemm_pair_ride_kernel(PairArgs a, int host_wgs, tokpp::Riders r) {
+    extern __shared__ __attribute__((aligned(16))) unsigned char smem[];
+    if ((int)blockIdx.x >= host_wgs) {
+        const int tid = threadIdx.x, wave = __builtin_amdgcn_readfirstlane(tid >> 6);
+        tokpp::tokred_pp_cell<3>(r.c, xcd_remap((int)blockIdx.x - host_wgs, r.n), reinterpret_cast<char*>(smem), tid & 63, wave);
+        __builtin_amdgcn_endpgm();
+    }
+    pair_wg<MODE>(a, smem, blockIdx.x, host_wgs);
 }
 
 template <int MODE>
@@ -643,6 +658,20 @@
     BF_CHECK_LAUNCH();
     return 0;
 }
+template <int MODE>
+int launch_pair_ride(const PairArgs& a, int M, const tokpp::Riders& r, hipStream_t st) {
+    constexpr int lds_bytes = PNSLOT * PSLOT_BYTES > tokpp::RIDER_LDS_BYTES ? PNSLOT * PSLOT_BYTES : tokpp::RIDER_LDS_BYTES;
+    static BfPerDeviceOnce attr_once; bool& attr_done = attr_once.flag();
+    if (!attr_done) {
+        hipError_t e_ = hipFuncSetAttribute(reinterpret_cast<const void*>(gemm_pair_ride_kernel<MODE>), hipFuncAttributeMaxDynamicSharedMemorySize, lds_bytes);
+        if (e_ != hipSuccess) return bf_fail(e_, __FILE__, __LINE__);
+        attr_done = true;
+    }
+    const int host_wgs = (M / PM) * a.nt;
+    hipLaunchKernelGGL(gemm_pair_ride_kernel<MODE>, dim3((unsigned)(host_wgs + r.n)), dim3(512), lds_bytes, st, a, host_wgs, r);
+    BF_CHECK_LAUNCH();
+    return 0;
+}
 bool pair_shape_ok(int M, int N, int K, int64_t lda, int64_t ldb) {
     static const bool off = bf_knob("BF_PAIR", 1) == 0;
     if (off) return false;
@@ -656,7 +685,7 @@
 struct InbwdScaled { void* out_s; const float* f; int fdiv; };
 static int inbwd_frames_impl2(int dtype, int M, int N, int K, const void* A, int64_t lda, const void* B, int64_t ldb, const void* x,
                               const void* add, void* out, int S, const float* mean, const float* rstd, const float* w, float* ws,
-                              const float* fscale, int fdiv, const InbwdChain* ch, const InbwdScaled* sc2, bf_stream_t stream);
+                              const float* fscale, int fdiv, const InbwdChain* ch, const InbwdScaled* sc2, const bfgemm::tokpp::Riders* ride, bf_stream_t stream);
 static int inbwd_frames_impl(int dtype, int M, int N, int K, const void* A, int64_t lda, const void* B, int64_t ldb, const void* x,
                              const void* add, void* out, int S, const float* mean, const float* rstd, const float* w, float* ws,
                              const float* fscale, int fdiv, const InbwdChain* ch, bf_stream_t stream);
@@ -676,18 +705,40 @@
 static int inbwd_frames_impl(int dtype, int M, int N, int K, const void* A, int64_t lda, const void* B, int64_t ldb, const void* x,
                              const void* add, void* out, int S, const float* mean, const float* rstd, const float* w, float* ws,
                              const float* fscale, int fdiv, const InbwdChain* ch, bf_stream_t stream) {
-    return inbwd_frames_impl2(dtype, M, N, K, A, lda, B, ldb, x, add, out, S, mean, rstd, w, ws, fscale, fdiv, ch, nullptr, stream);
+    return inbwd_frames_impl2(dtype, M, N, K, A, lda, B, ldb, x, add, out, S, mean, rstd, w, ws, fscale, fdiv, ch, nullptr, nullptr, stream);
 }
 int bf_gemm_inbwd_frames_scaled(int dtype, int M, int N, int K, const void* A, int64_t lda, const void* B, int64_t ldb, const void* x,
                                 const void* add, void* out, int S, const float* mean, const float* rstd, const float* w, float* ws,
                                 const float* fscale, int fdiv, void* out_s, const float* f_s, int fdiv_s, hipStream_t stream) {
     if (!out_s || !f_s || (((uintptr_t)out_s) & 15)) return 1;
     const InbwdScaled sc2{out_s, f_s, fdiv_s > 0 ? fdiv_s : 1};
-    return inbwd_frames_impl2(dtype, M, N, K, A, lda, B, ldb, x, add, out, S, mean, rstd, w, ws, fscale, fdiv, nullptr, &sc2, (bf_stream_t)stream);
+    return inbwd_frames_impl2(dtype, M, N, K, A, lda, B, ldb, x, add, out, S, mean, rstd, w, ws, fscale, fdiv, nullptr, &sc2, nullptr, (bf_stream_t)stream);
+}
+int bf_gemm_inbwd_frames_ride(int dtype, int M, int N, int K, const void* A, int64_t lda, const void* B, int64_t ldb, const void* x,
+                              const void* add, void* out, int S, const float* mean, const float* rstd, const float* w, float* ws,
+                              const float* fscale, int fdiv, const TokredRidePlan& plan, hipStream_t stream) {
+    if (plan.ride.n <= 0) return 1;
+    return inbwd_frames_impl2(dtype, M, N, K, A, lda, B, ldb, x, add, out, S, mean, rstd, w, ws, fscale, fdiv, nullptr, nullptr, &plan.ride, (bf_stream_t)stream);
+}
+extern "C" int bf_gemm_inbwd_frames_ride_wgrad(int dtype, int M, int N, int K, const void* A, int64_t lda, const void* B, int64_t ldb, const void* x,
+                                               const void* add, void* out, int S, const float* mean, const float* rstd, const float* w, float* ws,
+                                               const float* fscale, int fdiv, int Nout, int Kin, const void* dy, int64_t ldy, const void* tx,
+                                               int64_t ldtx, float* dW, int accumulate, float* colsum, float* tws, int64_t tws_floats, int riders,
+                                               bf_stream_t stream) {
+    BF_REQUIRE(A && B && x && out && mean && rstd && w && dy && tx && dW && tws, "bf_gemm_inbwd_frames_ride_wgrad: null pointer");
+    if (dtype != BF_DTYPE_BF16 || S != FM || !pair_shape_ok(M, N, K, lda, ldb) || K < FK) return 1;
+    if (((uintptr_t)A | (uintptr_t)B | (uintptr_t)x | (uintptr_t)add | (uintptr_t)out | (uintptr_t)dW) & 15) return 1;
+    TokredRidePlan plan;
+    if (const int rc = bf_tokred_ride_plan(dtype, Nout, Kin, M, dy, ldy, tx, ldtx, colsum, tws, tws_floats, riders, &plan)) return rc;
+    const int rc = plan.ride.n > 0
+        ? bf_gemm_inbwd_frames_ride(dtype, M, N, K, A, lda, B, ldb, x, add, out, S, mean, rstd, w, ws, fscale, fdiv, plan, (hipStream_t)stream)
+        : bf_gemm_inbwd_frames(dtype, M, N, K, A, lda, B, ldb, x, add, out, S, mean, rstd, w, ws, fscale, fdiv, stream);
+    if (rc) return rc;
+    return bf_tokred_ride_commit(plan, dW, accumulate, false, (hipStream_t)stream);
 }
 static int inbwd_frames_impl2(int dtype, int M, int N, int K, const void* A, int64_t lda, const void* B, int64_t ldb, const void* x,
                               const void* add, void* out, int S, const float* mean, const float* rstd, const float* w, float* ws,
-                              const float* fscale, int fdiv, const InbwdChain* ch, const InbwdScaled* sc2, bf_stream_t stream) {
+                              const float* fscale, int fdiv, const InbwdChain* ch, const InbwdScaled* sc2, const bfgemm::tokpp::Riders* ride, bf_stream_t stream) {
     BF_REQUIRE(A && B && x && out && mean && rstd && w, "bf_gemm_inbwd_frames: null pointer");
     static const bool off = bf_knob("BF_FUSE_INBWD", 1) == 0;
     if (off || dtype != BF_DTYPE_BF16 || (S != FM && S != PM) || M <= 0 || M % S || N <= 0 || N % FN || K < FK || K % FK || lda % 8 || ldb % 8) return 1;
@@ -705,12 +756,14 @@
             if (a.whole || (((uintptr_t)ch->z | (uintptr_t)ch->dz) & 15)) return 1;
             a.cz = (const bf16*)ch->z; a.cdz = (bf16*)ch->dz; a.cmean = ch->mean; a.crstd = ch->rstd; a.cw = ch->w; a.cg = ch->g; a.cgdiv = ch->gdiv; a.cws = ch->ws;
         }
-        BfProfScope prof((hipStream_t)stream, ch ? "gemm_pair<inbwd,chain>" : sc2 ? "gemm_pair<inbwd,scaled>" : "gemm_pair<inbwd>", 2.0 * M * N * K,
+        if (ride && (ch || sc2)) return 1;
+        BfProfScope prof((hipStream_t)stream, ch ? "gemm_pair<inbwd,chain>" : sc2 ? "gemm_pair<inbwd,scaled>" : ride ? "gemm_pair<inbwd,ride>" : "gemm_pair<inbwd>", 2.0 * M * N * K,
                          2.0 * ((double)M * K + (double)N * K + (double)M * N * ((add ? 3 : 2) + (ch ? 2 : 0) + (sc2 ? 1 : 0))));
         if (sc2) { if (ch) return 1; return launch_pair<5>(a, M, (hipStream_t)stream); }
+        if (ride && ride->n > 0) return launch_pair_ride<0>(a, M, *ride, (hipStream_t)stream);
         return ch ? launch_pair<2>(a, M, (hipStream_t)stream) : launch_pair<0>(a, M, (hipStream_t)stream);
     }
-    if (ch || sc2) return 1;
+    if (ch || sc2 || ride) return 1;
     if (S != FM) return 1;
     static BfPerDeviceOnce attr_once;
     if (bool& done = attr_once.flag(); !done) {
diff --git a/bubbleformer_amd/csrc/gemm_tokred.hip b/bubbleformer_amd/csrc/gemm_tokred.hip
--- a/bubbleformer_amd/csrc/gemm_tokred.hip
+++ b/bubbleformer_amd/csrc/gemm_tokred.hip
@@ -1,132 +1,12 @@
 #include "gemm_common.h"
+#include "tokred_pp.h"
 #include <stdio.h>
 #include <stdlib.h>
 #include <algorithm>
 
 namespace {
 using namespace bfgemm;
-
-constexpr int PTN = 192;
-constexpr int HR = 32;
-constexpr int NSB = PTN / 64;
-constexpr int SUBB = HR * 64 * 2;
-constexpr int NBUF = 4;
-template <int NI> struct PPGeom {
-    static constexpr int TM = 64 * NI, HALFB = (NI + NSB) * SUBB, TILES = NI * 6, TILE_FLOATS = TM * PTN;
-};
-
-__device__ __forceinline__ bf16x8 tr_frag(unsigned addr) {
-    return cat(__builtin_amdgcn_ds_read_tr16_b64_v4i16((lds_s16x4)(uintptr_t)addr),
-               __builtin_amdgcn_ds_read_tr16_b64_v4i16((lds_s16x4)(uintptr_t)(addr + 512u)));
-}
-
-template <int NI, int GRP>
-__device__ __forceinline__ void tokred_pp_body(const bf16* __restrict__ A, long lda, const bf16* __restrict__ B, long ldb,
-                                               float* __restrict__ slab_tile, float* __restrict__ cslab_row, int nh, bool do_cs,
-                                               unsigned ring_lds, int lane, int w4) {
-    using Gm = PPGeom<NI>;
-    constexpr int HALFB = Gm::HALFB;
-    constexpr int PG = NI == 6 ? (GRP == 0 ? 5 : 4) : 3;
-    constexpr int NCS = 3;
-    const int wm = w4, wn = GRP;
-    const int dr = 8 * w4 + (lane >> 3);
-    const int dkey = ((dr >> 1) & 1) | (((dr >> 3) & 1) << 1);
-    const int dch = (lane & 7) ^ (dkey << 1);
-    const bf16* pA = A + (long)dr * lda + 8 * dch;
-    const bf16* pB = B + (long)dr * ldb + 8 * dch;
-    const long stepA = (long)HR * lda, stepB = (long)HR * ldb;
-    auto issue = [&](int buf) {
-        const unsigned base = __builtin_amdgcn_readfirstlane(ring_lds + (unsigned)buf * (unsigned)HALFB + (unsigned)w4 * 1024u);
-        if constexpr (NI == 6 && GRP == 0) {
-            glds16_off<0>(pA, base + 0 * SUBB); glds16_off<128>(pA, base + 1 * SUBB); glds16_off<256>(pA, base + 2 * SUBB);
-            glds16_off<384>(pA, base + 3 * SUBB); glds16_off<512>(pA, base + 4 * SUBB);
-            pA += stepA;
-        } else if constexpr (NI == 6) {
-            glds16_off<640>(pA, base + 5 * SUBB);
-            glds16_off<0>(pB, base + 6 * SUBB); glds16_off<128>(pB, base + 7 * SUBB); glds16_off<256>(pB, base + 8 * SUBB);
-            pA += stepA; pB += stepB;
-        } else if constexpr (GRP == 0) {
-            glds16_off<0>(pA, base + 0 * SUBB); glds16_off<128>(pA, base + 1 * SUBB); glds16_off<256>(pA, base + 2 * SUBB);
-            pA += stepA;
-        } else {
-            glds16_off<0>(pB, base + 3 * SUBB); glds16_off<128>(pB, base + 4 * SUBB); glds16_off<256>(pB, base + 5 * SUBB);
-            pB += stepB;
-        }
-    };
-    const int g = lane >> 4, q = (lane >> 2) & 3, p = lane & 3;
-    const int fkey = ((q >> 1) & 1) | ((g & 1) << 1);
-    const unsigned rowb = (unsigned)(8 * g + q) * 128u + (unsigned)(p & 1) * 8u;
-    const unsigned offA = rowb + (unsigned)(((2 * wm + (p >> 1)) ^ (fkey << 1)) * 16);
-    const unsigned offB0 = rowb + (unsigned)(((2 * wn + (p >> 1)) ^ (fkey << 1)) * 16) + (unsigned)(NI * SUBB);
-    const unsigned offB1 = rowb + (unsigned)(((2 * wn + 4 + (p >> 1)) ^ (fkey << 1)) * 16) + (unsigned)(NI * SUBB);
-
-    f32x4 acc[NI][6];
-#pragma unroll
-    for (int i = 0; i < NI; ++i)
-#pragma unroll
-        for (int j = 0; j < 6; ++j) acc[i][j] = f32x4{0.f, 0.f, 0.f, 0.f};
-    f32x4 cs[NCS];
-#pragma unroll
-    for (int c = 0; c < NCS; ++c) cs[c] = f32x4{0.f, 0.f, 0.f, 0.f};
-    bf16x8 ones;
-#pragma unroll
-    for (int c = 0; c < 8; ++c) ones[c] = (bf16)1.0f;
-
-    issue(0);
-    if (nh > 1) issue(1);
-    if (nh > 2) issue(2);
-    if (nh > 2) wait_vm<2 * PG>(); else if (nh > 1) wait_vm<PG>(); else wait_vm<0>();
-    __builtin_amdgcn_s_barrier();
-    if constexpr (GRP == 1) __builtin_amdgcn_s_barrier();
-
-    int buf = 0;
-    for (int h = 0; h < nh; ++h) {
-        const unsigned hb = ring_lds + (unsigned)buf * (unsigned)HALFB;
-        bf16x8 fa[NI], fb[6];
-#pragma unroll
-        for (int i = 0; i < NI; ++i) fa[i] = tr_frag(hb + offA + (unsigned)(i * SUBB));
-#pragma unroll
-        for (int j = 0; j < 6; ++j) fb[j] = tr_frag(hb + ((j & 1) ? offB1 : offB0) + (unsigned)((j >> 1) * SUBB));
-        if (h + 3 < nh) issue((buf + 3) & 3);
-        const int younger = min(h + 3, nh - 1) - (h + 1);
-        if (younger >= 2) wait_vm<2 * PG>(); else if (younger == 1) wait_vm<PG>(); else wait_vm<0>();
-        asm volatile("s_waitcnt lgkmcnt(0)" ::: "memory");
-        __builtin_amdgcn_sched_barrier(0);
-        __builtin_amdgcn_s_barrier();
-#pragma unroll
-        for (int i = 0; i < NI; ++i)
-#pragma unroll
-            for (int j = 0; j < 6; ++j) acc[i][j] = __builtin_amdgcn_mfma_f32_16x16x32_bf16(fb[j], fa[i], acc[i][j], 0, 0, 0);
-        if (do_cs) {
-#pragma unroll
-            for (int c = 0; c < NCS; ++c) {
-                if constexpr (NI == 6) cs[c] = __builtin_amdgcn_mfma_f32_16x16x32_bf16(ones, fa[NCS * GRP + c], cs[c], 0, 0, 0);
-                else if constexpr (GRP == 0) cs[c] = __builtin_amdgcn_mfma_f32_16x16x32_bf16(ones, fa[c], cs[c], 0, 0, 0);
-            }
-        }
-        __builtin_amdgcn_sched_barrier(0);
-        __builtin_amdgcn_s_barrier();
-        buf = (buf + 1) & 3;
-    }
-    if constexpr (GRP == 0) __builtin_amdgcn_s_barrier();
-
-    const int wave = GRP * 4 + w4;
-    float* so = slab_tile + ((size_t)wave * Gm::TILES * 64 + lane) * 4;
-#pragma unroll
-    for (int i = 0; i < NI; ++i)
-#pragma unroll
-        for (int j = 0; j < 6; ++j)
-            *reinterpret_cast<float4*>(so + (size_t)(i * 6 + j) * 256) = make_float4(acc[i][j][0], acc[i][j][1], acc[i][j][2], acc[i][j][3]);
-    if (do_cs && lane < 16) {
-        if constexpr (NI == 6) {
-#pragma unroll
-            for (int c = 0; c < NCS; ++c) cslab_row[16 * (wm + 4 * (NCS * GRP + c)) + lane] = cs[c][0];
-        } else if constexpr (GRP == 0) {
-#pragma unroll
-            for (int c = 0; c < NCS; ++c) cslab_row[16 * (wm + 4 * c) + lane] = cs[c][0];
-        }
-    }
-}
+using namespace bfgemm::tokpp;
 
 struct FoldRed { const float* slab; const float* cslab; int nslice, ntiles, tiles_k, Nout, Kin; float* out; float* colsum; int accumulate; int nwg; };
 template <int NI>
@@ -163,26 +43,15 @@
 }
 
 template <int NI>
-__global__ void __launch_bounds__(512) tokred_pp_kernel(const bf16* __restrict__ A, long lda, const bf16* __restrict__ B, long ldb,
-                                                      float* __restrict__ slab, float* __restrict__ cslab, int Nout, int halves_total,
-                                                      int halves_per, int tiles_k, int ntiles, int main_wgs, FoldRed red) {
-    using Gm = PPGeom<NI>;
+__global__ void __launch_bounds__(512) tokred_pp_kernel(Cells c, int cell0, int main_wgs, FoldRed red, FoldRed red2) {
     extern __shared__ __attribute__((aligned(16))) char smem[];
-    if ((int)blockIdx.x >= main_wgs) { fold_reduce<NI>(red, (int)blockIdx.x - main_wgs); return; }
+    if ((int)blockIdx.x >= main_wgs) {
+        const int fb = (int)blockIdx.x - main_wgs;
+        if (fb < red.nwg) fold_reduce<NI>(red, fb); else fold_reduce<NI>(red2, fb - red.nwg);
+        return;
+    }
     const int tid = threadIdx.x, lane = tid & 63, wave = __builtin_amdgcn_readfirstlane(tid >> 6);
-    const int seq = xcd_remap(blockIdx.x, main_wgs);
-    const int slice = seq / ntiles, tile = seq - slice * ntiles;
-    const int n0 = (tile / tiles_k) * Gm::TM, c0 = (tile % tiles_k) * PTN;
-    const int h_beg = slice * halves_per;
-    const int nh = min(halves_per, halves_total - h_beg);
-    const bf16* a0 = A + (long)h_beg * HR * lda + n0;
-    const bf16* b0 = B + (long)h_beg * HR * ldb + c0;
-    float* slab_tile = slab + ((size_t)slice * ntiles + tile) * Gm::TILE_FLOATS;
-    const bool do_cs = cslab != nullptr && c0 == 0;
-    float* cslab_row = do_cs ? cslab + (size_t)slice * Nout + n0 : nullptr;
-    const unsigned ring_lds = lds_addr(smem);
-    if (wave < 4) tokred_pp_body<NI, 0>(a0, lda, b0, ldb, slab_tile, cslab_row, nh, do_cs, ring_lds, lane, wave);
-    else tokred_pp_body<NI, 1>(a0, lda, b0, ldb, slab_tile, cslab_row, nh, do_cs, ring_lds, lane, wave - 4);
+    tokred_pp_cell<NI>(c, cell0 + xcd_remap(blockIdx.x, main_wgs), smem, lane, wave);
 }
 
 template <int NI, int MAXS>
@@ -452,22 +321,50 @@
 }
 
 namespace {
-struct PendingRed { bool on = false; FoldRed r{}; int NI = 0; hipStream_t st = nullptr; bool half = false; hipEvent_t handoff = nullptr; };
+struct PendingSum { bool on = false; FoldRed r{}; int NI = 0; hipStream_t st = nullptr; };
+struct PendingRed { PendingSum own, ride; bool half = false; hipEvent_t handoff = nullptr, ride_ready = nullptr; };
 PendingRed g_pending[64];
 PendingRed& pending_slot() { int dev = 0; (void)hipGetDevice(&dev); return g_pending[(dev >= 0 && dev < 64) ? dev : 0]; }
 constexpr int FOLD_WGS = 40;
 }
 static int tokred_impl(int dtype, int Nout, int Kin, int64_t M, const void* dy, int64_t ldy, const void* x, int64_t ldx, float* out,
                        int accumulate, float* colsum, float* ws, int64_t ws_floats, bool defer, bf_stream_t stream);
-static int flush_pending(PendingRed& p, hipStream_t caller) {
-    if (!p.on) return 0;
-    p.on = false;
-    hipStream_t st = p.st;
-    const FoldRed& r = p.r;
+namespace {
+bool g_fold_off = false, g_ride_off = false;
+bool fold_allowed() { static const bool fold_on = bf_knob("BF_TOKRED_FOLD", 1) != 0; return fold_on && !g_fold_off; }
+struct PPSplit { bool big; int ns, halves_per, tiles_k, ntiles; };
+PPSplit pp_split(int Nout, int Kin, int64_t M) {
+    static const int slices_env = bf_knob("BF_TOKRED_SLICES", 0);
+    static const int tile_env = bf_knob("BF_TOKRED_TILE", 0);
+    static const int wgs_env = bf_knob("BF_TOKRED_WGS", 128);
+    const long halves = M / HR;
+    const int tiles_k = Kin / PTN;
+    const bool big = Nout % 384 == 0 && tile_env == 384;
+    const int tm = big ? 384 : 192;
+    int nslice = slices_env > 0 ? slices_env : std::max(1, wgs_env / ((Nout / tm) * tiles_k));
+    nslice = (int)std::max<long>(1, std::min<long>({(long)nslice, (long)MAX_SLICES, halves / 4}));
+    const int halves_per = bf_cdiv(halves, nslice);
+    return PPSplit{big, bf_cdiv(halves, halves_per), halves_per, tiles_k, (Nout / tm) * tiles_k};
+}
+template <int NI>
+int launch_pp(const Cells& c, int cell0, int main_wgs, const FoldRed& red, const FoldRed& red2, hipStream_t st) {
+    static BfPerDeviceOnce attr_once; bool& attr_done = attr_once.flag();
+    constexpr int lds_bytes = NBUF * PPGeom<NI>::HALFB;
+    if (!attr_done) {
+        hipError_t e_ = hipFuncSetAttribute((const void*)tokred_pp_kernel<NI>, hipFuncAttributeMaxDynamicSharedMemorySize, lds_bytes);
+        if (e_ != hipSuccess) return bf_fail(e_, __FILE__, __LINE__);
+        attr_done = true;
+    }
+    const unsigned extra = (unsigned)(std::max(red.nwg, 0) + std::max(red2.nwg, 0));
+    hipLaunchKernelGGL(tokred_pp_kernel<NI>, dim3((unsigned)main_wgs + extra), dim3(512), lds_bytes, st, c, cell0, main_wgs, red, red2);
+    BF_CHECK_LAUNCH();
+    return 0;
+}
+int launch_sum(const FoldRed& r, int NI, hipStream_t st) {
     const long n = (long)r.Nout * r.Kin;
     const unsigned rblocks = (unsigned)bf_cdiv(std::max<long>(n / 4, r.Nout), 256);
     BfProfScope prof(st, "tokred_reduce_kernel", 0.0, (double)(r.nslice + 1 + (r.accumulate ? 1 : 0)) * n * 4.0);
-    if (p.NI == 6) {
+    if (NI == 6) {
         if (r.nslice <= 8) hipLaunchKernelGGL((tokred_pp_reduce_kernel<6, 8>), dim3(rblocks), dim3(256), 0, st, r.slab, r.cslab, r.nslice, r.ntiles, r.tiles_k, r.Nout, r.Kin, r.out, r.colsum, r.accumulate);
         else hipLaunchKernelGGL((tokred_pp_reduce_kernel<6, MAX_SLICES>), dim3(rblocks), dim3(256), 0, st, r.slab, r.cslab, r.nslice, r.ntiles, r.tiles_k, r.Nout, r.Kin, r.out, r.colsum, r.accumulate);
     } else {
@@ -475,17 +372,33 @@
         else hipLaunchKernelGGL((tokred_pp_reduce_kernel<3, MAX_SLICES>), dim3(rblocks), dim3(256), 0, st, r.slab, r.cslab, r.nslice, r.ntiles, r.tiles_k, r.Nout, r.Kin, r.out, r.colsum, r.accumulate);
     }
     BF_CHECK_LAUNCH();
+    return 0;
+}
+}
+static int flush_one(PendingRed& pr, PendingSum& p, hipStream_t caller) {
+    if (!p.on) return 0;
+    p.on = false;
+    hipStream_t st = p.st;
+    if (const int rc = launch_sum(p.r, p.NI, st)) return rc;
     if (caller == st) return 0;
-    hipError_t e = p.handoff ? hipSuccess : hipEventCreateWithFlags(&p.handoff, hipEventDisableTiming);
-    if (e == hipSuccess) e = hipEventRecord(p.handoff, st);
-    if (e == hipSuccess) e = hipStreamWaitEvent(caller, p.handoff, 0);
+    hipError_t e = pr.handoff ? hipSuccess : hipEventCreateWithFlags(&pr.handoff, hipEventDisableTiming);
+    if (e == hipSuccess) e = hipEventRecord(pr.handoff, st);
+    if (e == hipSuccess) e = hipStreamWaitEvent(caller, pr.handoff, 0);
     return e == hipSuccess ? 0 : bf_fail(e, __FILE__, __LINE__);
 }
+static int flush_pending(PendingRed& p, hipStream_t caller) {
+    if (const int rc = flush_one(p, p.own, caller)) return rc;
+    return flush_one(p, p.ride, caller);
+}
 int bf_gemm_tokred_flush(hipStream_t st) { return flush_pending(pending_slot(), st); }
-namespace { bool g_fold_off = false; }
 extern "C" void bf_debug_tokred_fold(int on) { g_fold_off = on == 0; }
-bool bf_gemm_tokred_pending() { return pending_slot().on; }
-const float* bf_gemm_tokred_pending_out() { const PendingRed& p = pending_slot(); return p.on ? p.r.out : nullptr; }
+extern "C" void bf_debug_wgrad_ride(int on) { g_ride_off = on == 0; }
+bool bf_wgrad_ride_on() { static const bool knob = bf_knob("BF_WGRAD_RIDE", 1) != 0; return knob && !g_ride_off; }
+bool bf_gemm_tokred_pending() { const PendingRed& p = pending_slot(); return p.own.on || p.ride.on; }
+bool bf_gemm_tokred_pending_for(const float* out) {
+    const PendingRed& p = pending_slot();
+    return (p.own.on && p.own.r.out == out) || (p.ride.on && p.ride.r.out == out);
+}
 int bf_gemm_tokred_deferred(int dtype, int Nout, int Kin, int64_t M, const void* dy, int64_t ldy, const void* x, int64_t ldx, float* out,
                             int accumulate, float* colsum, float* ws, int64_t ws_floats, hipStream_t stream) {
     return tokred_impl(dtype, Nout, Kin, M, dy, ldy, x, ldx, out, accumulate, colsum, ws, ws_floats, true, (bf_stream_t)stream);
@@ -509,62 +422,37 @@
     hipStream_t st = (hipStream_t)stream;
     const long n = (long)Nout * Kin;
     static const int slices_env = bf_knob("BF_TOKRED_SLICES", 0);
-    static const int tile_env = bf_knob("BF_TOKRED_TILE", 0);
-    static const int wgs_env = bf_knob("BF_TOKRED_WGS", 128);
     if (pp) {
-        const long halves = M / HR;
-        const int tiles_k0 = Kin / PTN;
-        const bool big = Nout % 384 == 0 && tile_env == 384;
-        const int tm = big ? 384 : 192;
-        int nslice = slices_env > 0 ? slices_env : std::max(1, wgs_env / ((Nout / tm) * tiles_k0));
-        nslice = (int)std::max<long>(1, std::min<long>({(long)nslice, (long)MAX_SLICES, halves / 4}));
-        const int halves_per = bf_cdiv(halves, nslice);
-        const int ns = bf_cdiv(halves, halves_per);
+        const PPSplit sp = pp_split(Nout, Kin, M);
+        const bool big = sp.big;
+        const int ns = sp.ns, ntiles = sp.ntiles;
         BF_REQUIRE(ws_floats >= (int64_t)ns * (n + Nout), "bf_gemm_tokred: workspace too small (bf_gemm_tokred_ws_floats)");
-        const int tiles_k = Kin / PTN, ntiles = (Nout / tm) * tiles_k;
-        static const bool fold_on = bf_knob("BF_TOKRED_FOLD", 1) != 0;
         const int64_t half_floats = (ws_floats / 2) & ~(int64_t)3;
-        const bool fold = defer && fold_on && !g_fold_off && (int64_t)ns * (n + Nout) <= half_floats;
+        const bool fold = defer && fold_allowed() && (int64_t)ns * (n + Nout) <= half_floats;
         PendingRed& pend = pending_slot();
-        if (pend.on && (!fold || pend.NI != (big ? 6 : 3) || pend.st != st)) { const int frc = flush_pending(pend, st); if (frc) return frc; }
+        if (pend.own.on && (!fold || pend.own.NI != (big ? 6 : 3) || pend.own.st != st)) { const int frc = flush_one(pend, pend.own, st); if (frc) return frc; }
+        if (pend.ride.on && (!fold || pend.ride.NI != (big ? 6 : 3))) { const int frc = flush_one(pend, pend.ride, st); if (frc) return frc; }
         float* region = ws;
         if (fold) { region = ws + (pend.half ? half_floats : 0); pend.half = !pend.half; }
         float* slab = region;
         float* cslab = colsum ? region + (size_t)ns * n : nullptr;
-        const unsigned rblocks = (unsigned)bf_cdiv(std::max<long>(n / 4, Nout), 256);
-        FoldRed red{};
+        FoldRed red{}, red2{};
         static const int fold_wgs = bf_knob("BF_TOKRED_FOLD_WGS", FOLD_WGS);
-        if (fold && pend.on) { red = pend.r; red.nwg = fold_wgs; }
-        const unsigned extra = red.nwg > 0 ? (unsigned)red.nwg : 0u;
-#define BF_PP_GO(NIV)                                                                                                                     \
-        do {                                                                                                                              \
-            {                                                                                                                             \
-                BfProfScope prof(st, NIV == 6 ? "tokred_pp_kernel<384x192,h32,ring4>" : "tokred_pp_kernel<192x192,h32,ring4>",           \
-                                 2.0 * Nout * Kin * (double)M, (double)M * (Nout + Kin) * 2.0 + (double)n * 4.0);                         \
-                static BfPerDeviceOnce attr_once; bool& attr_done = attr_once.flag();                                                                                            \
-                constexpr int lds_bytes = NBUF * PPGeom<NIV>::HALFB;                                                                      \
-                if (!attr_done) {                                                                                                         \
-                    hipError_t e_ = hipFuncSetAttribute((const void*)tokred_pp_kernel<NIV>, hipFuncAttributeMaxDynamicSharedMemorySize, lds_bytes); \
-                    if (e_ != hipSuccess) return bf_fail(e_, __FILE__, __LINE__);                                                         \
-                    attr_done = true;                                                                                                     \
-                }                                                                                                                         \
-                hipLaunchKernelGGL(tokred_pp_kernel<NIV>, dim3((unsigned)(ns * ntiles) + extra), dim3(512), lds_bytes, st, (const bf16*)dy, (long)ldy, \
-                                   (const bf16*)x, (long)ldx, slab, cslab, Nout, (int)halves, halves_per, tiles_k, ntiles, ns * ntiles, red); \
-                BF_CHECK_LAUNCH();                                                                                                        \
-            }                                                                                                                             \
-            if (fold) {                                                                                                                   \
-                pend.on = true; pend.NI = NIV; pend.st = st;                                                                              \
-                pend.r = FoldRed{slab, cslab, ns, ntiles, tiles_k, Nout, Kin, out, colsum, accumulate, 0};                                \
-                break;                                                                                                                    \
-            }                                                                                                                             \
-            BfProfScope prof(st, "tokred_reduce_kernel", 0.0, (double)(ns + 1 + (accumulate ? 1 : 0)) * n * 4.0);                         \
-            if (ns <= 8) hipLaunchKernelGGL((tokred_pp_reduce_kernel<NIV, 8>), dim3(rblocks), dim3(256), 0, st, slab, cslab, ns, ntiles, tiles_k, Nout, Kin, out, colsum, accumulate); \
-            else hipLaunchKernelGGL((tokred_pp_reduce_kernel<NIV, MAX_SLICES>), dim3(rblocks), dim3(256), 0, st, slab, cslab, ns, ntiles, tiles_k, Nout, Kin, out, colsum, accumulate); \
-            BF_CHECK_LAUNCH();                                                                                                            \
-        } while (0)
-        if (big) BF_PP_GO(6); else BF_PP_GO(3);
-#undef BF_PP_GO
-        return 0;
+        if (fold && pend.own.on) { red = pend.own.r; red.nwg = fold_wgs; pend.own.on = false; }
+        if (fold && pend.ride.on) {
+            if (pend.ride.st != st) { const hipError_t e_ = hipStreamWaitEvent(st, pend.ride_ready, 0); if (e_ != hipSuccess) return bf_fail(e_, __FILE__, __LINE__); }
+            red2 = pend.ride.r; red2.nwg = fold_wgs; pend.ride.on = false;
+        }
+        const Cells cells{(const bf16*)dy, (long)ldy, (const bf16*)x, (long)ldx, slab, cslab, Nout, (int)(M / HR), sp.halves_per, sp.tiles_k, ntiles};
+        {
+            BfProfScope prof(st, big ? "tokred_pp_kernel<384x192,h32,ring4>" : "tokred_pp_kernel<192x192,h32,ring4>",
+                             2.0 * Nout * Kin * (double)M, (double)M * (Nout + Kin) * 2.0 + (double)n * 4.0);
+            const int lrc = big ? launch_pp<6>(cells, 0, ns * ntiles, red, red2, st) : launch_pp<3>(cells, 0, ns * ntiles, red, red2, st);
+            if (lrc) return lrc;
+        }
+        const FoldRed mine{slab, cslab, ns, ntiles, sp.tiles_k, Nout, Kin, out, colsum, accumulate, 0};
+        if (fold) { pend.own.on = true; pend.own.NI = big ? 6 : 3; pend.own.st = st; pend.own.r = mine; return 0; }
+        return launch_sum(mine, big ? 6 : 3, st);
     }
     { const int frc = flush_pending(pending_slot(), st); if (frc) return frc; }
     const long steps = M / BK;
@@ -595,6 +483,38 @@
         hipLaunchKernelGGL(tokred_reduce_kernel, dim3(blocks), dim3(256), 0, st, slab, cslab, ns, n, Nout, out, colsum, accumulate);
         BF_CHECK_LAUNCH();
     }
+    return 0;
+}
+
+int bf_tokred_ride_plan(int dtype, int Nout, int Kin, int64_t M, const void* dy, int64_t ldy, const void* x, int64_t ldx, float* colsum, float* slabs,
+                        int64_t slab_floats, int max_ride, TokredRidePlan* plan) {
+    if (dtype != BF_DTYPE_BF16 || Nout <= 0 || Kin <= 0 || M <= 0) return 1;
+    if (Nout % 192 || Kin % PTN || M % HR || M < 4 * HR || ldy % 8 || ldx % 8 || ldy < Nout || ldx < Kin) return 1;
+    if (!dy || !x || !slabs || !plan || (((uintptr_t)dy | (uintptr_t)x | (uintptr_t)slabs) & 15)) return 1;
+    const PPSplit sp = pp_split(Nout, Kin, M);
+    const long n = (long)Nout * Kin;
+    if (sp.big || slab_floats < (int64_t)sp.ns * (n + Nout)) return 1;
+    plan->ride.c = Cells{(const bf16*)dy, (long)ldy, (const bf16*)x, (long)ldx, slabs, colsum ? slabs + (size_t)sp.ns * n : nullptr, Nout, (int)(M / HR),
+                         sp.halves_per, sp.tiles_k, sp.ntiles};
+    plan->cells = sp.ns * sp.ntiles; plan->nslice = sp.ns; plan->Nout = Nout; plan->Kin = Kin; plan->colsum = colsum;
+    plan->ride.n = std::max(0, std::min(plan->cells, max_ride));
+    return 0;
+}
+int bf_tokred_ride_commit(const TokredRidePlan& plan, float* out, int accumulate, bool defer, hipStream_t producer) {
+    BF_REQUIRE(out && ((uintptr_t)out & 15) == 0, "bf_tokred_ride_commit: bad output");
+    const Cells& c = plan.ride.c;
+    if (plan.ride.n < plan.cells) {
+        BfProfScope prof(producer, "tokred_pp_kernel<192x192,h32,ring4>", 2.0 * plan.Nout * plan.Kin * (double)c.halves_total * HR * (plan.cells - plan.ride.n) / plan.cells, 0.0);
+        if (const int rc = launch_pp<3>(c, plan.ride.n, plan.cells - plan.ride.n, FoldRed{}, FoldRed{}, producer)) return rc;
+    }
+    const FoldRed mine{c.slab, c.cslab, plan.nslice, c.ntiles, c.tiles_k, plan.Nout, plan.Kin, out, plan.colsum, accumulate, 0};
+    if (!defer || !fold_allowed()) return launch_sum(mine, 3, producer);
+    PendingRed& pend = pending_slot();
+    if (const int rc = flush_one(pend, pend.ride, producer)) return rc;
+    hipError_t e = pend.ride_ready ? hipSuccess : hipEventCreateWithFlags(&pend.ride_ready, hipEventDisableTiming | hipEventDisableSystemFence);
+    if (e == hipSuccess) e = hipEventRecord(pend.ride_ready, producer);
+    if (e != hipSuccess) return bf_fail(e, __FILE__, __LINE__);
+    pend.ride.on = true; pend.ride.NI = 3; pend.ride.st = producer; pend.ride.r = mine;
     return 0;
 }
 
diff --git a/bubbleformer_amd/csrc/model.hip b/bubbleformer_amd/csrc/model.hip
--- a/bubbleformer_amd/csrc/model.hip
+++ b/bubbleformer_amd/csrc/model.hip
@@ -1,9 +1,13 @@
 #include "model_common.h"
+#include "tokred_pp.h"
 
 bool bf_attn_raw_modes(int dtype, int d);
 int bf_gemm_tokred_deferred(int dtype, int Nout, int Kin, int64_t M, const void* dy, int64_t ldy, const void* x, int64_t ldx, float* out,
                             int accumulate, float* colsum, float* ws, int64_t ws_floats, hipStream_t stream);
-const float* bf_gemm_tokred_pending_out();
+bool bf_gemm_tokred_pending_for(const float* out);
+int bf_gemm_inbwd_frames_ride(int dtype, int M, int N, int K, const void* A, int64_t lda, const void* B, int64_t ldb, const void* x,
+                              const void* add, void* out, int S, const float* mean, const float* rstd, const float* w, float* ws,
+                              const float* fscale, int fdiv, const TokredRidePlan& plan, hipStream_t stream);
 int bf_gemm_inbwd_frames_scaled(int dtype, int M, int N, int K, const void* A, int64_t lda, const void* B, int64_t ldb, const void* x,
                                 const void* add, void* out, int S, const float* mean, const float* rstd, const float* w, float* ws,
                                 const float* fscale, int fdiv, void* out_s, const float* f_s, int fdiv_s, hipStream_t stream);
@@ -386,8 +390,25 @@
 int outproj_bwd(const D& d, const Scratch& sc, const void* dout, const void* on, const void* w_s,
                 const float* W, const float* bias, const float* nb, const float* gamma, const float* lo, const float* hi,
                 const float* alpha, const float* mc, float* dW, float* dbias, float* dnb, float* dgamma, float* dlo, float* dhi,
-                void* don, hipStream_t st, Fork& fk, const InFuse* fu = nullptr) {
-    TRY(fk.run([=](hipStream_t ss) -> int {
+                void* don, hipStream_t st, Fork& fk, const InFuse* fu = nullptr, bool may_ride = false) {
+    bool rode = false;
+    if (may_ride && fu && fk.deferred && bf_wgrad_ride_on() && !fu->tail && !fu->scaled_out && d.dtype == BF_DTYPE_BF16 && d.S == 144 && d.N % 288 == 0 &&
+        d.E % 128 == 0) {
+        static BfPerDevice<int> cu_tab;
+        int& cus = cu_tab.get();
+        if (cus == 0) { int dev = 0; (void)hipGetDevice(&dev); if (hipDeviceGetAttribute(&cus, hipDeviceAttributeMultiprocessorCount, dev) != hipSuccess || cus <= 0) cus = -1; }
+        const long host_wgs = (d.N / 288) * (d.E / 128);
+        TokredRidePlan plan;
+        if (cus > host_wgs &&
+            bf_tokred_ride_plan(d.dtype, d.E, d.E, d.N, dout, d.E, on, d.E, sc.csum, sc.gslab, sc.gslab_floats, (int)(cus - host_wgs), &plan) == 0 &&
+            plan.ride.n == plan.cells) {
+            const int rrc = bf_gemm_inbwd_frames_ride(d.dtype, (int)d.N, d.E, d.E, dout, d.E, w_s, d.E, fu->x, fu->add, fu->dx, (int)d.S, fu->mean, fu->rstd,
+                                                      fu->w, fu->ws, fu->fscale, fu->fdiv, plan, st);
+            if (rrc < 0) return rrc;
+            if (rrc == 0) { TRY(bf_tokred_ride_commit(plan, sc.G, 0, true, st)); rode = true; }
+        }
+    }
+    if (!rode) TRY(fk.run([=](hipStream_t ss) -> int {
         const void* dsrc = dout;
         const int trc = bf_gemm_tokred_deferred(d.dtype, d.E, d.E, d.N, dsrc, d.E, on, d.E, sc.G, 0, sc.csum, sc.tokred_ws, sc.tokred_floats, ss);
         if (trc < 0) return trc;
@@ -402,12 +423,13 @@
         return 0;
     }));
     fk.run_late([=](hipStream_t ss) -> int {
-        if (bf_gemm_tokred_pending_out() == sc.G) TRY(bf_gemm_tokred_flush(ss));
+        if (bf_gemm_tokred_pending_for(sc.G)) TRY(bf_gemm_tokred_flush(ss));
         hipLaunchKernelGGL(outproj_finalize_kernel, dim3(d.E + (lo ? bf_cdiv(d.E, 16) : 0)), dim3(256), 0, ss, sc.G, sc.csum, W, bias, nb, gamma, lo, hi, mc,
                            dW, dbias, dnb, dgamma, dlo, dhi, d.E);
         BF_CHECK_LAUNCH();
         return 0;
     });
+    if (rode) return 0;
     if (fu) return dgrad_inbwd(d, dout, d.E, w_s, d.E, don, *fu, st);
     {
         bf_operand A = op_plain(dout, d.E, BF_LAY_KC);
@@ -547,7 +569,7 @@
     L.dbr_ready = TrunkLinks::DbrReady{};
     const InFuse fu2{sv.o, nullptr, dO, sv.mean2, sv.rstd2, p->norm2_w, p->norm2_b, sc.in_ws2};
     TRY(outproj_bwd(d, sc, dbr, sv.on, sv.wout_s, p->output_head_w, p->output_head_b, p->norm2_b, p->gamma, nullptr, nullptr,
-                    sv.alpha, sv.mc, g->output_head_w, g->output_head_b, nullptr, g->gamma, nullptr, nullptr, don, st, fk, &fu2));
+                    sv.alpha, sv.mc, g->output_head_w, g->output_head_b, nullptr, g->gamma, nullptr, nullptr, don, st, fk, &fu2, H.ride));
     ReduceJobs jobs;
     TRY(jobs.push(InReduceJob{sc.in_ws2, (int)d.F, d.E, p->norm2_w, p->norm2_b, nullptr, 1, g->norm2_w, g->norm2_b, nullptr, nullptr, nullptr, nullptr}));
     {
@@ -752,7 +774,7 @@
     TRY(outproj_bwd(d, sc, dbr, sv.on, sv.wout_s, p->output_head_w, p->output_head_b, p->norm2_b, p->gamma_att,
                     d.feat_scale ? p->low_freq_scalar : nullptr, d.feat_scale ? p->high_freq_scalar : nullptr, sv.alpha, sv.mc,
                     g->output_head_w, g->output_head_b, g->norm2_b, g->gamma_att, d.feat_scale ? g->low_freq_scalar : nullptr,
-                    d.feat_scale ? g->high_freq_scalar : nullptr, don, st, fk, &fu2));
+                    d.feat_scale ? g->high_freq_scalar : nullptr, don, st, fk, &fu2, H.ride));
     TRY(jobs.push(InReduceJob{sc.in_ws2, (int)d.F, d.E, p->norm2_w, p->norm2_b, nullptr, 1, g->norm2_w, g->norm2_b, nullptr, nullptr, nullptr, nullptr}));
     void* dqkv = sc.t3;
     {
@@ -843,6 +865,7 @@
         void* gout = i ? gbuf3[rot] : dx;
         rot = (rot + 1) % 3;
         StageHints H;
+        H.ride = true;
         if (kinds[i] == 0) {
             if (i > 0 && kinds[i - 1] == 1) H.tail = NextTail{true, (const bf_spatial_params*)params[i - 1], saved[i - 1], drop_b && drop_b[i - 1]};
             TRY(temporal_bwd(L, H, dims, (const bf_temporal_params*)params[i], (const bf_temporal_params*)grads[i], in, cur, gout, saved[i], scratch,
diff --git a/bubbleformer_amd/csrc/model_common.h b/bubbleformer_amd/csrc/model_common.h
--- a/bubbleformer_amd/csrc/model_common.h
+++ b/bubbleformer_amd/csrc/model_common.h
@@ -80,7 +80,7 @@
 struct NextHead { bool armed = false; const float *w = nullptr, *b = nullptr; float *mean = nullptr, *rstd = nullptr, *sc = nullptr, *sh = nullptr; void* xn = nullptr; const void* saved = nullptr; };
 struct NextTail { bool armed = false; const bf_spatial_params* p = nullptr; const void* saved = nullptr; bool drop = false; };
 struct NextScale { const float* f = nullptr; int fdiv = 1; };
-struct StageHints { bool prepared = false; NextHead head; NextTail tail; NextScale scale; };
+struct StageHints { bool prepared = false; NextHead head; NextTail tail; NextScale scale; bool ride = false; };
 
 struct ReduceJobs {
     static constexpr int IN_CAP = 6, ATTN_CAP = 4;
@@ -199,6 +199,7 @@
 struct Scratch {
     float *G, *csum, *zeros, *ones, *wg, *attn_ws, *attn_ws2, *in_ws, *in_ws2, *in_ws3, *in_ws4, *in_ws5;
     float* tokred_ws; int64_t tokred_floats;
+    float* gslab; int64_t gslab_floats;
     static constexpr long ATTN_WS_FLOATS = 1024L * (4 * 128 + 32 * 16 + 16);
     void *t1, *t3, *t4, *t1b; int64_t t1b_floats;
     void *s1, *e5, *e6, *e7;
@@ -216,6 +217,8 @@
         wg = a.f32(wgn);
         tokred_floats = bf_gemm_tokred_ws_floats(4 * d.E, d.E, d.N);
         tokred_ws = a.f32((size_t)tokred_floats);
+        gslab_floats = bf_gemm_tokred_ws_floats(d.E, d.E, d.N);
+        gslab = a.f32((size_t)gslab_floats);
         attn_ws = a.f32(ATTN_WS_FLOATS);
         attn_ws2 = a.f32(ATTN_WS_FLOATS);
         {
diff --git a/bubbleformer_amd/csrc/tokred_pp.h b/bubbleformer_amd/csrc/tokred_pp.h
--- /dev/null
+++ b/bubbleformer_amd/csrc/tokred_pp.h
@@ -0,0 +1,162 @@
+#pragma once
+#include "gemm_common.h"
+
+namespace bfgemm {
+namespace tokpp {
+
+constexpr int PTN = 192;
+constexpr int HR = 32;
+constexpr int NSB = PTN / 64;
+constexpr int SUBB = HR * 64 * 2;
+constexpr int NBUF = 4;
+template <int NI> struct PPGeom {
+    static constexpr int TM = 64 * NI, HALFB = (NI + NSB) * SUBB, TILES = NI * 6, TILE_FLOATS = TM * PTN;
+};
+
+__device__ __forceinline__ bf16x8 tr_frag(unsigned addr) {
+    return cat(__builtin_amdgcn_ds_read_tr16_b64_v4i16((lds_s16x4)(uintptr_t)addr),
+               __builtin_amdgcn_ds_read_tr16_b64_v4i16((lds_s16x4)(uintptr_t)(addr + 512u)));
+}
+
+template <int NI, int GRP>
+__device__ __forceinline__ void tokred_pp_body(const bf16* __restrict__ A, long lda, const bf16* __restrict__ B, long ldb,
+                                               float* __restrict__ slab_tile, float* __restrict__ cslab_row, int nh, bool do_cs,
+                                               unsigned ring_lds, int lane, int w4) {
+    using Gm = PPGeom<NI>;
+    constexpr int HALFB = Gm::HALFB;
+    constexpr int PG = NI == 6 ? (GRP == 0 ? 5 : 4) : 3;
+    constexpr int NCS = 3;
+    const int wm = w4, wn = GRP;
+    const int dr = 8 * w4 + (lane >> 3);
+    const int dkey = ((dr >> 1) & 1) | (((dr >> 3) & 1) << 1);
+    const int dch = (lane & 7) ^ (dkey << 1);
+    const bf16* pA = A + (long)dr * lda + 8 * dch;
+    const bf16* pB = B + (long)dr * ldb + 8 * dch;
+    const long stepA = (long)HR * lda, stepB = (long)HR * ldb;
+    auto issue = [&](int buf) {
+        const unsigned base = __builtin_amdgcn_readfirstlane(ring_lds + (unsigned)buf * (unsigned)HALFB + (unsigned)w4 * 1024u);
+        if constexpr (NI == 6 && GRP == 0) {
+            glds16_off<0>(pA, base + 0 * SUBB); glds16_off<128>(pA, base + 1 * SUBB); glds16_off<256>(pA, base + 2 * SUBB);
+            glds16_off<384>(pA, base + 3 * SUBB); glds16_off<512>(pA, base + 4 * SUBB);
+            pA += stepA;
+        } else if constexpr (NI == 6) {
+            glds16_off<640>(pA, base + 5 * SUBB);
+            glds16_off<0>(pB, base + 6 * SUBB); glds16_off<128>(pB, base + 7 * SUBB); glds16_off<256>(pB, base + 8 * SUBB);
+            pA += stepA; pB += stepB;
+        } else if constexpr (GRP == 0) {
+            glds16_off<0>(pA, base + 0 * SUBB); glds16_off<128>(pA, base + 1 * SUBB); glds16_off<256>(pA, base + 2 * SUBB);
+            pA += stepA;
+        } else {
+            glds16_off<0>(pB, base + 3 * SUBB); glds16_off<128>(pB, base + 4 * SUBB); glds16_off<256>(pB, base + 5 * SUBB);
+            pB += stepB;
+        }
+    };
+    const int g = lane >> 4, q = (lane >> 2) & 3, p = lane & 3;
+    const int fkey = ((q >> 1) & 1) | ((g & 1) << 1);
+    const unsigned rowb = (unsigned)(8 * g + q) * 128u + (unsigned)(p & 1) * 8u;
+    const unsigned offA = rowb + (unsigned)(((2 * wm + (p >> 1)) ^ (fkey << 1)) * 16);
+    const unsigned offB0 = rowb + (unsigned)(((2 * wn + (p >> 1)) ^ (fkey << 1)) * 16) + (unsigned)(NI * SUBB);
+    const unsigned offB1 = rowb + (unsigned)(((2 * wn + 4 + (p >> 1)) ^ (fkey << 1)) * 16) + (unsigned)(NI * SUBB);
+
+    f32x4 acc[NI][6];
+#pragma unroll
+    for (int i = 0; i < NI; ++i)
+#pragma unroll
+        for (int j = 0; j < 6; ++j) acc[i][j] = f32x4{0.f, 0.f, 0.f, 0.f};
+    f32x4 cs[NCS];
+#pragma unroll
+    for (int c = 0; c < NCS; ++c) cs[c] = f32x4{0.f, 0.f, 0.f, 0.f};
+    bf16x8 ones;
+#pragma unroll
+    for (int c = 0; c < 8; ++c) ones[c] = (bf16)1.0f;
+
+    issue(0);
+    if (nh > 1) issue(1);
+    if (nh > 2) issue(2);
+    if (nh > 2) wait_vm<2 * PG>(); else if (nh > 1) wait_vm<PG>(); else wait_vm<0>();
+    __builtin_amdgcn_s_barrier();
+    if constexpr (GRP == 1) __builtin_amdgcn_s_barrier();
+
+    int buf = 0;
+    for (int h = 0; h < nh; ++h) {
+        const unsigned hb = ring_lds + (unsigned)buf * (unsigned)HALFB;
+        bf16x8 fa[NI], fb[6];
+#pragma unroll
+        for (int i = 0; i < NI; ++i) fa[i] = tr_frag(hb + offA + (unsigned)(i * SUBB));
+#pragma unroll
+        for (int j = 0; j < 6; ++j) fb[j] = tr_frag(hb + ((j & 1) ? offB1 : offB0) + (unsigned)((j >> 1) * SUBB));
+        if (h + 3 < nh) issue((buf + 3) & 3);
+        const int younger = min(h + 3, nh - 1) - (h + 1);
+        if (younger >= 2) wait_vm<2 * PG>(); else if (younger == 1) wait_vm<PG>(); else wait_vm<0>();
+        asm volatile("s_waitcnt lgkmcnt(0)" ::: "memory");
+        __builtin_amdgcn_sched_barrier(0);
+        __builtin_amdgcn_s_barrier();
+#pragma unroll
+        for (int i = 0; i < NI; ++i)
+#pragma unroll
+            for (int j = 0; j < 6; ++j) acc[i][j] = __builtin_amdgcn_mfma_f32_16x16x32_bf16(fb[j], fa[i], acc[i][j], 0, 0, 0);
+        if (do_cs) {
+#pragma unroll
+            for (int c = 0; c < NCS; ++c) {
+                if constexpr (NI == 6) cs[c] = __builtin_amdgcn_mfma_f32_16x16x32_bf16(ones, fa[NCS * GRP + c], cs[c], 0, 0, 0);
+                else if constexpr (GRP == 0) cs[c] = __builtin_amdgcn_mfma_f32_16x16x32_bf16(ones, fa[c], cs[c], 0, 0, 0);
+            }
+        }
+        __builtin_amdgcn_sched_barrier(0);
+        __builtin_amdgcn_s_barrier();
+        buf = (buf + 1) & 3;
+    }
+    if constexpr (GRP == 0) __builtin_amdgcn_s_barrier();
+
+    const int wave = GRP * 4 + w4;
+    float* so = slab_tile + ((size_t)wave * Gm::TILES * 64 + lane) * 4;
+#pragma unroll
+    for (int i = 0; i < NI; ++i)
+#pragma unroll
+        for (int j = 0; j < 6; ++j)
+            *reinterpret_cast<float4*>(so + (size_t)(i * 6 + j) * 256) = make_float4(acc[i][j][0], acc[i][j][1], acc[i][j][2], acc[i][j][3]);
+    if (do_cs && lane < 16) {
+        if constexpr (NI == 6) {
+#pragma unroll
+            for (int c = 0; c < NCS; ++c) cslab_row[16 * (wm + 4 * (NCS * GRP + c)) + lane] = cs[c][0];
+        } else if constexpr (GRP == 0) {
+#pragma unroll
+            for (int c = 0; c < NCS; ++c) cslab_row[16 * (wm + 4 * c) + lane] = cs[c][0];
+        }
+    }
+}
+
+struct Cells {
+    const bf16* A; long lda; const bf16* B; long ldb; float* slab; float* cslab;
+    int Nout, halves_total, halves_per, tiles_k, ntiles;
+};
+template <int NI>
+__device__ __forceinline__ void tokred_pp_cell(const Cells& c, int seq, char* smem, int lane, int wave) {
+    using Gm = PPGeom<NI>;
+    const int slice = seq / c.ntiles, tile = seq - slice * c.ntiles;
+    const int n0 = (tile / c.tiles_k) * Gm::TM, c0 = (tile % c.tiles_k) * PTN;
+    const int h_beg = slice * c.halves_per;
+    const int nh = min(c.halves_per, c.halves_total - h_beg);
+    const bf16* a0 = c.A + (long)h_beg * HR * c.lda + n0;
+    const bf16* b0 = c.B + (long)h_beg * HR * c.ldb + c0;
+    float* slab_tile = c.slab + ((size_t)slice * c.ntiles + tile) * Gm::TILE_FLOATS;
+    const bool do_cs = c.cslab != nullptr && c0 == 0;
+    float* cslab_row = do_cs ? c.cslab + (size_t)slice * c.Nout + n0 : nullptr;
+    const unsigned ring_lds = lds_addr(smem);
+    if (wave < 4) tokred_pp_body<NI, 0>(a0, c.lda, b0, c.ldb, slab_tile, cslab_row, nh, do_cs, ring_lds, lane, wave);
+    else tokred_pp_body<NI, 1>(a0, c.lda, b0, c.ldb, slab_tile, cslab_row, nh, do_cs, ring_lds, lane, wave - 4);
+}
+
+struct Riders { Cells c; int n; };
+constexpr int RIDER_LDS_BYTES = NBUF * PPGeom<3>::HALFB;
+
+}
+}
+
+struct TokredRidePlan {
+    bfgemm::tokpp::Riders ride; int cells, nslice; int Nout, Kin; float* colsum;
+};
+int bf_tokred_ride_plan(int dtype, int Nout, int Kin, int64_t M, const void* dy, int64_t ldy, const void* x, int64_t ldx, float* colsum, float* slabs,
+                        int64_t slab_floats, int max_ride, TokredRidePlan* plan);
+int bf_tokred_ride_commit(const TokredRidePlan& plan, float* out, int accumulate, bool defer, hipStream_t producer);
+bool bf_wgrad_ride_on();
diff --git a/include/bubbleformer_hip.h b/include/bubbleformer_hip.h
--- a/include/bubbleformer_hip.h
+++ b/include/bubbleformer_hip.h
@@ -62,6 +62,10 @@
                                const void* add, void* out, int S, const float* mean, const float* rstd, const float* w, float* ws,
                                const float* fscale, int fdiv, const void* cz, void* cdz, const float* cmean, const float* crstd,
                                const float* cw, const float* cg, int cgdiv, float* cws, bf_stream_t stream);
+int bf_gemm_inbwd_frames_ride_wgrad(int dtype, int M, int N, int K, const void* A, int64_t lda, const void* B, int64_t ldb, const void* x,
+                                    const void* add, void* out, int S, const float* mean, const float* rstd, const float* w, float* ws,
+                                    const float* fscale, int fdiv, int Nout, int Kin, const void* dy, int64_t ldy, const void* tx, int64_t ldtx,
+                                    float* dW, int accumulate, float* colsum, float* tws, int64_t tws_floats, int riders, bf_stream_t stream);
 
 typedef struct bf_frame_norm {
     const float *w, *b;
@@ -120,6 +124,7 @@
 int bf_side_join(bf_stream_t stream);
 void bf_debug_force_generic_attn(int on);
 void bf_debug_tokred_fold(int on);
+void bf_debug_wgrad_ride(int on);
 
 int bf_im2col_nchw(int dtype, const float* x, void* out, int frames, int C, int H, int W, int Kp, bf_stream_t stream);
 int bf_col2im_nchw(int dtype, const void* g, float* dx, int frames, int C, int H, int W, int Kp, bf_stream_t stream);
```
